# BurnhamG/PyTorch-ScalableFHVAE

Measured on AMD Instinct MI355X. Metric: segments/sec + ELBO (nats/frame), (B,20,80) fbank, higher is better.
Workload: dtype bf16; 1 GPU; c3: fhvae.FHVAE 2x256 LSTM enc/dec, z1=z2=32, 28k-seq mu2 table, batch 2048; per-GPU batch 2048, T=20, F=80, full train step (fwd+loss+bwd+Adam), intended objective, mu_idx uniform; global_batch=2048, parallelism=single

## Files before the change

include/fhvae_hip.h:

```cpp
#ifndef FHVAE_HIP_H
#define FHVAE_HIP_H

#include <stdint.h>

#ifdef __cplusplus
extern "C" {
#endif

#define FHVAE_ABI_VERSION 11

enum { FHVAE_F32 = 0, FHVAE_BF16 = 1 };

enum {
  FHVAE_OK = 0,
  FHVAE_ERR_NULL = -1,
  FHVAE_ERR_SHAPE = -2,
  FHVAE_ERR_DTYPE = -3,
  FHVAE_ERR_ALIGN = -4,
  FHVAE_ERR_LIMIT = -5
};

#define FHVAE_MAX_LAYERS 4
#define FHVAE_LSTM_SYNC_BYTES 16384

int fhvae_abi_version(void);
const char* fhvae_strerror(int code);

int fhvae_linear_fwd(const void* x, int64_t ldx, const void* w, int64_t ldw, const float* b,
                     float* y, int64_t ldy, void* y_lp, int64_t M, int64_t K, int64_t N, int relu,
                     int dtype, void* stream);

int fhvae_linear_bwd(const float* x, int64_t ldx, const float* w, int64_t ldw, const float* y,
                     int64_t ldy, const float* dy, int64_t lddy, float* dy_masked, float* dx,
                     int64_t lddx, float* dw, int64_t lddw, float* db, int64_t M, int64_t K,
                     int64_t N, int relu, int dx_accumulate, void* stream);

int fhvae_gauss_head_reparam_fwd(const void* h, int64_t ldh, const void* w_mu, const void* w_lv,
                                 const float* b_mu, const float* b_lv, const float* eps, float* mu,
                                 float* logvar, float* sample, int64_t M, int64_t K, int64_t D,
                                 int dtype, void* stream);
int fhvae_gauss_head_pair_fwd(const void* h_lp, int64_t ldh, const void* w_pair_lp, const float* b_mu, const float* b_lv,
                              float* out, int64_t ldo, int64_t M, int64_t K, int64_t D, void* stream);
int fhvae_head_pair_weights(const float* w_mu, const float* w_lv, void* wl_pair, void* wt_pair, int64_t ldt,
                            int64_t D, int64_t K, void* stream);
int fhvae_gauss_reparam_pair_fwd(const float* out, int64_t ldo, const float* eps, float* sample, float* mu, float* logvar,
                                 int64_t M, int64_t D, void* stream);
int fhvae_gauss_reparam_bwd_pair(const float* d_mu, const float* d_logvar, const float* d_sample, int64_t ld_s, const float* eps,
                                 const float* logvar, int64_t ld_lv, void* g_lp, int64_t ldg, float* db_mu, float* db_lv,
                                 int64_t M, int64_t D, void* stream);
int fhvae_gauss_head_bwd_pair(const void* h_lp, int64_t ldh, const void* wt_pair, int64_t ldt, const void* g_lp, int64_t ldg,
                              const float* col_sum, int64_t col_sum_rows, float* dh, int64_t lddh, float* dw_mu, float* dw_lv, float* db_mu,
                              float* db_lv, int64_t M, int64_t K, int64_t D, void* stream);

int fhvae_gauss_reparam_bwd(const float* d_mu, const float* d_logvar, const float* d_sample,
                            const float* eps, const float* logvar, float* g_mu, float* g_lv,
                            int64_t n, void* stream);
int fhvae_gauss_head_bwd(const float* h, int64_t ldh, const float* w_mu, const float* w_lv,
                         const float* d_mu, const float* d_logvar, const float* d_sample,
                         const float* eps, const float* logvar, float* g_ws, float* dh, int64_t lddh,
                         float* dw_mu, float* dw_lv, float* db_mu, float* db_lv, int64_t M, int64_t K,
                         int64_t D, void* stream);
typedef struct fhvae_lstm_desc {
  int32_t dtype;
  int32_t L;
  int64_t B, T, I, Ic, H;
  const float* x;
  const void* x_lp;
  const float* xc;
  const float* w_ih[FHVAE_MAX_LAYERS];
  const float* w_hh[FHVAE_MAX_LAYERS];
  const float* b_ih[FHVAE_MAX_LAYERS];
  const float* b_hh[FHVAE_MAX_LAYERS];
  void* hs;
  float* cs;
  void* gates;
  float* hn;
  float* hs_top_f32;
  float* pre;
  void* lp;
  void* hn_lp;
  const float* head_w_mu;
  const float* head_w_lv;
  void* head_wl;
  void* head_wt;
  int64_t head_D, head_K, head_ldt;
  int32_t* sticky_status;
} fhvae_lstm_desc;

int64_t fhvae_lstm_lp_bytes(const fhvae_lstm_desc* d);
int64_t fhvae_lstm_pre_elems(const fhvae_lstm_desc* d);
int fhvae_lstm_layout_id(const fhvae_lstm_desc* d);

int64_t fhvae_lstm_ws_below_elems(const fhvae_lstm_desc* d);
int fhvae_lstm_form(const fhvae_lstm_desc* d);
int fhvae_lstm_seq_fwd(const fhvae_lstm_desc* d, void* stream);
int64_t fhvae_lstm_infer_cs_elems(const fhvae_lstm_desc* d);
int fhvae_lstm_seq_infer(const fhvae_lstm_desc* d, void* stream);

typedef struct fhvae_lstm_bwd_desc {
  fhvae_lstm_desc f;
  const float* d_hs_top;
  const float* d_hn;
  void* dgates;
  float* dgsum;
  float* dc;
  float* dw_ih[FHVAE_MAX_LAYERS];
  float* dw_hh[FHVAE_MAX_LAYERS];
  float* db_ih[FHVAE_MAX_LAYERS];
  float* db_hh[FHVAE_MAX_LAYERS];
  float* d_xc;
  int32_t phase;
  float* ws_below;
} fhvae_lstm_bwd_desc;

int fhvae_lstm_seq_bwd(const fhvae_lstm_bwd_desc* d, void* stream);
typedef struct fhvae_wgrad_desc {
  const void* a; int64_t lda;
  int64_t a_col0;
  const void* b; int64_t ldb;
  float* c; int64_t ldc;
  int64_t M, N, K;
} fhvae_wgrad_desc;
int fhvae_wgrad_desc_ok(const fhvae_wgrad_desc* p);
int fhvae_lstm_param_grads_multi(const fhvae_lstm_bwd_desc* const* descs, int n, const fhvae_wgrad_desc* extra, int n_extra,
                                 void* stream);
int fhvae_wgrad_bf16(const void* a, int64_t lda, const void* b, int64_t ldb, float* c, int64_t ldc, int64_t M,
                     int64_t N, int64_t K, void* stream);
int fhvae_wgrad_f32(const float* a, int64_t lda, const float* b, int64_t ldb, float* c, int64_t ldc, int64_t M, int64_t N,
                    int64_t K, void* stream);

int fhvae_proj_bf16(const void* a, int64_t lda, const void* b, int64_t ldb, const float* bias, float* c, int64_t ldc,
                    int64_t M, int64_t N, int64_t K, void* stream);

int fhvae_mu2_gather_fwd(const float* table, const int64_t* idx, int64_t idx_offset, float* mu2,
                         int64_t B, int64_t S, int64_t D, int32_t* oob_flag, void* stream);
int fhvae_mu2_gather_bwd(const float* dmu2, const int64_t* idx, int64_t idx_offset, float* dtable,
                         int64_t B, int64_t S, int64_t D, float scale, void* stream);

typedef struct fhvae_elbo_desc {
  int64_t B, T, F, D1, D2;
  const float* x;    int64_t x_sb, x_st;
  const float* x_mu; const float* x_lv; int64_t xo_sb, xo_st;
  const float* z1_mu; const float* z1_lv;
  const float* z2_mu; const float* z2_lv;
  const float* mu2;
  const int64_t* num_segs; double nsegs_scalar;
  float* lower_bound; float* log_px_z; float* neg_kld_z1; float* neg_kld_z2; float* log_pmu2;
} fhvae_elbo_desc;

int fhvae_elbo_fwd(const fhvae_elbo_desc* d, void* stream);

typedef struct fhvae_elbo_bwd_desc {
  fhvae_elbo_desc f;
  const float* g_lower_bound; const float* g_log_px_z; const float* g_neg_kld_z1;
  const float* g_neg_kld_z2; const float* g_log_pmu2;
  int32_t reference_detach;
  float* d_x_mu; float* d_x_lv;
  float* d_z1_mu; float* d_z1_lv; float* d_z2_mu; float* d_z2_lv; float* d_mu2;
  void* d_x_pair_lp; int64_t ld_pair; float* d_x_colsum;
} fhvae_elbo_bwd_desc;

int fhvae_elbo_bwd(const fhvae_elbo_bwd_desc* d, void* stream);
int64_t fhvae_elbo_colsum_rows(int64_t B);

int64_t fhvae_disc_lse_ws_bytes(int64_t B, int64_t S);
int fhvae_disc_lse_fwd(const float* q, const float* table, const int64_t* idx, int64_t row0,
                       float inv_two_var, float* row_max, float* row_sumexp, float* tgt_logit,
                       float* ce_mean, float ce_scale, void* ws, int64_t B, int64_t S, int64_t D, int dtype, void* stream);
int fhvae_shard_pack(const float* q, const int64_t* idx, float* out, int64_t B, int64_t D, void* stream);
int fhvae_shard_unpack(const float* packed, float* q, int64_t* idx, int64_t N, int64_t D, void* stream);
int fhvae_disc_merge_partials(const float* parts, float* row_max, float* row_sumexp, float* tgt_logit, int64_t W, int64_t N,
                              void* stream);
int fhvae_shard_bwd_pack(const float* dq_all, float dq_scale, const float* dmu2_local, int64_t own0, int64_t n_own, float* out,
                         int64_t N, int64_t D, void* stream);
int fhvae_shard_bwd_unpack(const float* buf, int64_t own0, int64_t n_own, float* dq_local, float* dmu2_all, int64_t N, int64_t D,
                           void* stream);
int fhvae_disc_ce_mean(const float* row_max, const float* row_sumexp, const float* tgt_logit,
                       float* ce_mean, float ce_scale, int64_t B, void* stream);

int64_t fhvae_disc_lse_bwd_ws_bytes(int64_t B, int64_t S, int64_t D);
int fhvae_disc_lse_bwd(const float* q, const float* table, const int64_t* idx, int64_t row0,
                       float inv_two_var, const float* row_max, const float* row_sumexp,
                       const float* g_scale, float g_mul, float* dq, float* dtable, void* ws, int64_t ws_bytes,
                       int64_t B, int64_t S, int64_t D, int dtype, void* stream);

int fhvae_loss_fwd(const float* lower_bound, const float* log_qy, float alpha, float* loss, int64_t B,
                   int32_t* nan_flag, void* stream);
int fhvae_loss_bwd(const float* g_loss, float alpha, float* d_lower_bound, float* d_log_qy, int64_t B,
                   void* stream);

int fhvae_adam_step(float* p, float* g, float* m, float* v, void* p_lp, int64_t n, float lr,
                    float beta1, float beta2, float eps, float grad_scale, int flags, int32_t* step_count,
                    void* stream);
#define FHVAE_ADAM_ZERO_GRAD 1
#define FHVAE_ADAM_ADVANCE 2
#define FHVAE_ADAM_STEP_WORDS (65 * 32)

int fhvae_trace_enable(int on);
int64_t fhvae_trace_collect(float* ms, int32_t* kind, double* flops, int64_t cap);

int fhvae_segment_gather(const float* pool, int64_t pool_frames, const int64_t* start, const float* mean,
                         const float* inv_std, float* out_btf, float* out_tbf, int64_t B, int64_t T,
                         int64_t F, int32_t* oob_flag, void* stream);

int fhvae_mu2_accumulate(const float* z2_mu, const int64_t* idx, float* zsum, float* count, int64_t N,
                         int64_t S, int64_t D, void* stream);
int fhvae_mu2_finalize(const float* zsum, const float* count, float* mu2, int64_t S, int64_t D,
                       float ratio, void* stream);

#define FHVAE_HS_BAD_SEQ 1
#define FHVAE_HS_CAP 2
#define FHVAE_HS_BAD_IDX 4
#define FHVAE_HS_UNSORTED 8
int fhvae_hs_select(const int64_t* seq_ptr, int64_t S, const int64_t* block_seqs, int64_t K, int64_t* seg_ids,
                    int64_t* local_idx, int64_t* n_out, int64_t cap, int32_t* status, void* stream);
int fhvae_mu2_accumulate_sorted(const float* z2_mu, const int64_t* local_idx, float* zsum, float* count, int64_t N,
                                int64_t K, int64_t D, int32_t* status, void* stream);
int fhvae_mu2_load_table(float* zsum, float* count, float* table, float* m_rows, float* v_rows, int64_t K, int64_t D,
                         float ratio, void* stream);
int fhvae_hs_pack_partials(float* zsum, float* count, float* out, int64_t K, int64_t D, void* stream);
int fhvae_mu2_merge_load_shard(const float* parts, int64_t W, int64_t K, int64_t row0, int64_t row1, float* shard,
                               float* m_rows, float* v_rows, int64_t D, float ratio, void* stream);

#define FHVAE_FEATS_FBANK 0
#define FHVAE_FEATS_SPEC 1
#define FHVAE_FEATS_MAX_NFFT 2048
#define FHVAE_FEATS_MAX_NFFT_FBANK 1664
#define FHVAE_FEATS_MAX_NMELS 256
#define FHVAE_FEATS_BAD_PTR 1
int fhvae_feats_tile_rows(int64_t n_fft, int ftype);
int fhvae_feats_fwd(const float* wave, int64_t n_samples, const int64_t* wave_ptr, const int64_t* frame_ptr, int64_t U,
                    int64_t n_frames, const float* dft_basis, const float* mel_basis, int64_t n_fft, int64_t hop, int64_t n_mels,
                    int ftype, float* out, int32_t* status, void* stream);

#define FHVAE_SYNTH_BAD_PTR 1
int fhvae_synth_tile_rows(int64_t n_fft);
int fhvae_synth_istft(const float* spec, int64_t n_frames, const int64_t* wave_ptr, const int64_t* frame_ptr, int64_t U,
                      int64_t n_samples, const float* synth_basis, const float* win_sq, int64_t n_fft, int64_t hop,
                      float* frames_ws, float* wave_out, int32_t* status, void* stream);
int fhvae_synth_project(const float* wave, int64_t n_samples, const int64_t* wave_ptr, const int64_t* frame_ptr, int64_t U,
                        int64_t n_frames, const float* dft_basis, const float* mag, const float* tprev, float coef, int64_t n_fft,
                        int64_t hop, float* rebuilt, float* next, int32_t* status, void* stream);
int fhvae_synth_deemph(const float* wave, const int64_t* wave_ptr, int64_t U, int64_t n_samples, float coef, float* out,
                       int32_t* status, void* stream);

#define FHVAE_RESAMPLE_MAX_L 4096
#define FHVAE_RESAMPLE_MAX_BANK (1 << 24)
#define FHVAE_RESAMPLE_LDS_FLOATS 40128
#define FHVAE_RESAMPLE_BAD_PTR 1
int fhvae_resample_tile_rows(int64_t KP);
int fhvae_resample_fwd(const float* wave_in, int64_t n_in, const int64_t* in_ptr, const int64_t* out_ptr,
                       const int64_t* row_ptr, int64_t U, int64_t n_rows, const float* bank, const int32_t* chunks, int64_t L,
                       int64_t M, int64_t P, int64_t KP, int64_t WL, double ratio, const uint8_t* exc, int64_t n_exc,
                       const float* alt, int64_t alt_taps, int64_t alt_wl, float* wave_out, int64_t n_out, int32_t* status,
                       void* stream);

int fhvae_to_time_major(const float* x_btf, void* x_tbf, float* x_tbf_f32, int64_t B, int64_t T,
                        int64_t F, int dtype, void* stream);
int fhvae_cast_bf16(const float* src, void* dst, void* dst_t, int64_t R, int64_t C, void* stream);

#ifdef __cplusplus
}
#endif
#endif
```

pytorch-scalablefhvae_amd/csrc/disc_mfma.h:

```cpp
#pragma once
#include "common.h"

namespace fh {

struct DiscMfmaArgs {
  const float* X;
  const float* Y;
  int NX, NY;
  float c;
  int x_is_query;
  const int64_t* idx;
  int64_t row0;
  const float* rmax;
  const float* rsum;
  const float* gsc;
  float gmul;
  float2* part;
  float* G;
  float* G2;
  float* WY;
  int chunk;
};

int mfma_chunk(int64_t nx, int64_t ny, int target = 1024);

bool disc_mfma_supported(int64_t B, int64_t S, int64_t D);
int64_t disc_mfma_ws_bytes(int64_t B, int64_t S);
int disc_mfma_fwd(const float* q, const float* table, const int64_t* idx, int64_t row0, float c, float2* part, int* nchunks,
                  int64_t B, int64_t S, int64_t D, int lp, hipStream_t st);
constexpr int64_t kOnePassWsCap = 3LL << 29;
int64_t disc_onepass_ws_bytes(int64_t B, int64_t S, int64_t D);
int disc_mfma_bwd(const float* q, const float* table, const int64_t* idx, int64_t row0, float c, const float* rmax,
                  const float* rsum, const float* gsc, float gmul, float* dq, float* dtable, float* ws, int64_t ws_bytes,
                  int64_t B, int64_t S, int64_t D, int lp, hipStream_t st);
void disc_lp_launch(const DiscMfmaArgs& a, int mode, dim3 grid, hipStream_t st);

}
```

pytorch-scalablefhvae_amd/csrc/disc_mfma.hip:

```cpp
#include <algorithm>

#include "disc_mfma.h"

#include <cstdlib>
#include <type_traits>

namespace fh {


template <int D>
__device__ __forceinline__ int yoff(int row, int ch) {
  constexpr int CHN = D / 4;
  return row * (D * 4) + ((ch ^ (row & (CHN >= 8 ? 7 : CHN - 1))) << 4);
}

template <int D, int MODE>
__global__ __launch_bounds__(256, 2) void disc_mfma_kernel(DiscMfmaArgs a) {
  constexpr int CHN = D / 4;
  constexpr int NJ = D / 16;
  constexpr int YT = 64;
  __shared__ __attribute__((aligned(16))) char ytile[YT * D * 4];
  __shared__ __attribute__((aligned(16))) float yn[YT];
  __shared__ float ymax[YT], yinv[YT];
  __shared__ int ytgt[YT];
  __shared__ int yown[YT / 16];
  constexpr bool BW = MODE >= 1, BOTH = MODE == 2;
  constexpr int kWLd = 68;
  constexpr int kDtLd = D + 4;
  __shared__ __attribute__((aligned(16))) float wimg[BOTH ? 4 : 1][BOTH ? 16 * kWLd : 4];
  __shared__ float wy_lds[BOTH ? 4 : 1][BOTH ? YT : 1];
  constexpr int kRed = !BW ? 1 : (BOTH && 4 * YT * kDtLd > 256 * (D + 1) ? 4 * YT * kDtLd : 256 * (D + 1));
  __shared__ __attribute__((aligned(16))) float red[kRed];
  float (*tr)[D + 1] = (float (*)[D + 1]) red;

  const int tid = threadIdx.x, lane = tid & 63, wave = tid >> 6;
  const int g = lane >> 4, i = lane & 15;
  const int x0 = blockIdx.y * 256 + wave * 64;
  const int y_begin = blockIdx.x * a.chunk;
  const int y_end = min(a.NY, y_begin + a.chunk);
  const float gscale = BW ? (*a.gsc) * a.gmul : 0.f;

  uint4 xf[4][NJ];
  float xn[4], xmax[4], xinv[4];
  int xtgt[4];
#pragma unroll
  for (int t = 0; t < 4; ++t) {
    const int x = x0 + t * 16 + i;
    const bool ok = x < a.NX;
    float nrm = 0.f;
#pragma unroll
    for (int jj = 0; jj < NJ; ++jj) {
      uint4 u = make_uint4(0, 0, 0, 0);
      if (ok) u = *(const uint4*)(a.X + (int64_t)x * D + 4 * g + 16 * jj);
      xf[t][jj] = u;
      const float f0 = __uint_as_float(u.x), f1 = __uint_as_float(u.y), f2 = __uint_as_float(u.z), f3 = __uint_as_float(u.w);
      nrm += f0 * f0 + f1 * f1 + f2 * f2 + f3 * f3;
    }
    nrm += __shfl_xor(nrm, 16, 64);
    nrm += __shfl_xor(nrm, 32, 64);
    xn[t] = nrm;
    xmax[t] = 0.f;
    xinv[t] = 0.f;
    xtgt[t] = -1;
    if (a.x_is_query) {
      if (ok) {
        const int64_t tg = a.idx[x] - a.row0;
        xtgt[t] = (tg >= 0 && tg < a.NY) ? (int)tg : -1;
        if (BW) {
          xmax[t] = a.rmax[x];
          xinv[t] = gscale / a.rsum[x];
        }
      }
    } else {
      xtgt[t] = ok ? x : -2;
    }
  }
  float m[4], ssum[4], wsum[4];
  f32x4 gacc[4][NJ];
#pragma unroll
  for (int t = 0; t < 4; ++t) {
    m[t] = -INFINITY;
    ssum[t] = 0.f;
    wsum[t] = 0.f;
#pragma unroll
    for (int j = 0; j < NJ; ++j) gacc[t][j] = f32x4{0.f, 0.f, 0.f, 0.f};
  }

  constexpr int LOADS = YT * CHN / 256;
  uint4 st[LOADS];
  auto issue = [&](int y0) {
#pragma unroll
    for (int p = 0; p < LOADS; ++p) {
      const int id = tid + p * 256;
      const int row = id / CHN, ch = id % CHN;
      const int y = y0 + row;
      st[p] = (y < y_end) ? *(const uint4*)(a.Y + (int64_t)y * D + ch * 4) : make_uint4(0, 0, 0, 0);
    }
  };
  if (y_begin < y_end) issue(y_begin);
  for (int y0 = y_begin; y0 < y_end; y0 += YT) {
#pragma unroll
    for (int p = 0; p < LOADS; ++p) {
      const int id = tid + p * 256;
      *(uint4*)(ytile + yoff<D>(id / CHN, id % CHN)) = st[p];
    }
    __syncthreads();
    if (y0 + YT < y_end) issue(y0 + YT);
    {
      const int row = tid >> 2, part = tid & 3;
      float nrm = 0.f;
#pragma unroll
      for (int c4 = part; c4 < CHN; c4 += 4) {
        const uint4 u = *(const uint4*)(ytile + yoff<D>(row, c4));
        const float f0 = __uint_as_float(u.x), f1 = __uint_as_float(u.y), f2 = __uint_as_float(u.z), f3 = __uint_as_float(u.w);
        nrm += f0 * f0 + f1 * f1 + f2 * f2 + f3 * f3;
      }
      nrm += __shfl_xor(nrm, 1, 64);
      nrm += __shfl_xor(nrm, 2, 64);
      bool mine = false;
      if (part == 0) {
        yn[row] = nrm;
        const int y = y0 + row;
        if (!a.x_is_query) {
          const bool ok = y < y_end;
          ymax[row] = ok && MODE == 1 ? a.rmax[y] : 0.f;
          yinv[row] = ok && MODE == 1 ? gscale / a.rsum[y] : 0.f;
          int tg = -3;
          if (ok) {
            const int64_t v = a.idx[y] - a.row0;
            tg = (v >= 0 && v < a.NX) ? (int)v : -3;
          }
          ytgt[row] = tg;
          mine = tg >= (int)blockIdx.y * 256 && tg < (int)blockIdx.y * 256 + 256;
        }
      }
      {
        const bool any = __any(mine);
        if (lane == 0) yown[wave] = any ? 1 : 0;
      }
    }
    __syncthreads();

#pragma unroll 1
    for (int yb = 0; yb < YT / 16; ++yb) {
      if (y0 + yb * 16 >= y_end) break;
      uint4 af[NJ];
#pragma unroll
      for (int jj = 0; jj < NJ; ++jj) af[jj] = *(const uint4*)(ytile + yoff<D>(yb * 16 + i, g + 4 * jj));
      const float4 ynv = *(const float4*)(yn + yb * 16 + 4 * g);
      const float ynr[4] = {ynv.x, ynv.y, ynv.z, ynv.w};
      float ymx[4], yiv[4];
      int ytg[4];
      if (MODE == 1 && !a.x_is_query) {
#pragma unroll
        for (int r = 0; r < 4; ++r) {
          ymx[r] = ymax[yb * 16 + 4 * g + r];
          yiv[r] = yinv[yb * 16 + 4 * g + r];
          ytg[r] = ytgt[yb * 16 + 4 * g + r];
        }
      }
      const int ybase = y0 + yb * 16;
      const bool whole = ybase + 16 <= y_end && x0 + 64 <= a.NX;
      const bool own_blk = !a.x_is_query && yown[yb] != 0;
      const float c2 = 2.f * a.c;
      f32x4 oacc[BOTH ? NJ : 1];
      float wyp = 0.f;
      if constexpr (BOTH) {
#pragma unroll
        for (int dj = 0; dj < NJ; ++dj) oacc[dj] = f32x4{0.f, 0.f, 0.f, 0.f};
      }
      auto logits = [&](int t) __attribute__((always_inline)) -> f32x4 {
        f32x4 acc = {0.f, 0.f, 0.f, 0.f};
#pragma unroll
        for (int jj = 0; jj < NJ; ++jj) {
          const uint4 ua = af[jj], ub = xf[t][jj];
          acc = __builtin_amdgcn_mfma_f32_16x16x4f32(__uint_as_float(ua.x), __uint_as_float(ub.x), acc, 0, 0, 0);
          acc = __builtin_amdgcn_mfma_f32_16x16x4f32(__uint_as_float(ua.y), __uint_as_float(ub.y), acc, 0, 0, 0);
          acc = __builtin_amdgcn_mfma_f32_16x16x4f32(__uint_as_float(ua.z), __uint_as_float(ub.z), acc, 0, 0, 0);
          acc = __builtin_amdgcn_mfma_f32_16x16x4f32(__uint_as_float(ua.w), __uint_as_float(ub.w), acc, 0, 0, 0);
        }
        return acc;
      };
      auto tile = [&](int t, auto masked_c, const f32x4& acc) __attribute__((always_inline)) {
        constexpr bool MASKED = decltype(masked_c)::value;
        const bool xok = x0 + t * 16 + i < a.NX;
        const float cxn = a.c * xn[t];
        float lg[4];
#pragma unroll
        for (int r = 0; r < 4; ++r) {
          lg[r] = c2 * acc[r] - (a.c * ynr[r] + cxn);
          if constexpr (MASKED) {
            const int y = ybase + 4 * g + r;
            if (!(xok && y < y_end)) lg[r] = -INFINITY;
            const bool own = (MODE == 1 && !a.x_is_query) ? ytg[r] == xtgt[t] : xtgt[t] == y;
            if (own) lg[r] = -INFINITY;
          }
        }
        if constexpr (MODE == 0) {
          const float gm = fmaxf(fmaxf(lg[0], lg[1]), fmaxf(lg[2], lg[3]));
          if (gm > m[t]) {
            ssum[t] *= __expf(m[t] - gm);
            m[t] = gm;
          }
          if (!MASKED || m[t] > -INFINITY) {
#pragma unroll
            for (int r = 0; r < 4; ++r) ssum[t] += __expf(lg[r] - m[t]);
          }
        } else {
          float w[4];
#pragma unroll
          for (int r = 0; r < 4; ++r) {
            float p;
            if (a.x_is_query)
              p = __expf(lg[r] - xmax[t]) * xinv[t];
            else
              p = __expf(lg[r] - ymx[r]) * yiv[r];
            w[r] = (!MASKED || lg[r] > -INFINITY) ? p : 0.f;
            wsum[t] += w[r];
          }
          float xb[BOTH ? 4 : 1][NJ];
          if constexpr (BOTH) {
#pragma unroll
            for (int q = 0; q < 4; ++q) {
              const int x = min(x0 + 16 * t + 4 * g + q, a.NX - 1);
#pragma unroll
              for (int dj = 0; dj < NJ; ++dj) xb[q][dj] = a.X[(int64_t)x * D + 16 * dj + i];
            }
          }
#pragma unroll
          for (int dj = 0; dj < NJ; ++dj) {
#pragma unroll
            for (int r = 0; r < 4; ++r) {
              const int row = yb * 16 + 4 * g + r, d = dj * 16 + i;
              const float av = *(const float*)(ytile + yoff<D>(row, d >> 2) + (d & 3) * 4);
              gacc[t][dj] = __builtin_amdgcn_mfma_f32_16x16x4f32(av, w[r], gacc[t][dj], 0, 0, 0);
            }
          }
          if constexpr (BOTH) {
            float* wi = wimg[wave];
#pragma unroll
            for (int r = 0; r < 4; ++r) wi[(4 * g + r) * kWLd + 16 * t + i] = w[r];
            asm volatile("" ::: "memory");
            const float4 wt = *(const float4*)(wi + i * kWLd + 16 * t + 4 * g);
            asm volatile("" ::: "memory");
            const float wq[4] = {wt.x, wt.y, wt.z, wt.w};
            wyp += (wq[0] + wq[1]) + (wq[2] + wq[3]);
#pragma unroll
            for (int q = 0; q < 4; ++q)
#pragma unroll
              for (int dj = 0; dj < NJ; ++dj) oacc[dj] = __builtin_amdgcn_mfma_f32_16x16x4f32(wq[q], xb[q][dj], oacc[dj], 0, 0, 0);
          }
        }
      };
      bool any_masked = !whole || own_blk;
      if (a.x_is_query) {
#pragma unroll
        for (int t = 0; t < 4; ++t) any_masked = any_masked || __any((unsigned)(xtgt[t] - ybase) < 16u);
      }
      if (!BOTH && !any_masked) {
        f32x4 nxt = logits(0);
#pragma unroll
        for (int t = 0; t < 4; ++t) {
          const f32x4 cur = nxt;
          if (t + 1 < 4) nxt = logits(t + 1);
          tile(t, std::false_type{}, cur);
        }
      } else {
#pragma unroll
        for (int t = 0; t < 4; ++t) {
          bool masked = !whole || own_blk;
          if (a.x_is_query) masked = masked || __any((unsigned)(xtgt[t] - ybase) < 16u);
          const f32x4 acc = logits(t);
          if (masked)
            tile(t, std::true_type{}, acc);
          else
            tile(t, std::false_type{}, acc);
        }
      }
      if constexpr (BOTH) {
        float* slot = red + wave * (YT * kDtLd);
#pragma unroll
        for (int dj = 0; dj < NJ; ++dj)
#pragma unroll
          for (int r = 0; r < 4; ++r) slot[(yb * 16 + 4 * g + r) * kDtLd + 16 * dj + i] = oacc[dj][r];
        wyp += __shfl_xor(wyp, 16, 64);
        wyp += __shfl_xor(wyp, 32, 64);
        if (g == 0) wy_lds[wave][yb * 16 + i] = wyp;
      }
    }
    __syncthreads();
    if constexpr (BOTH) {
      for (int e = tid; e < YT * D; e += 256) {
        const int row = e / D, d = e % D, o = row * kDtLd + d;
        if (y0 + row < y_end)
          a.G2[((int64_t)blockIdx.y * a.NY + y0 + row) * D + d] =
              (red[o] + red[YT * kDtLd + o]) + (red[2 * YT * kDtLd + o] + red[3 * YT * kDtLd + o]);
      }
      if (tid < YT && y0 + tid < y_end)
        a.WY[(int64_t)blockIdx.y * a.NY + y0 + tid] = (wy_lds[0][tid] + wy_lds[1][tid]) + (wy_lds[2][tid] + wy_lds[3][tid]);
    }
  }

  if constexpr (MODE == 0) {
#pragma unroll
    for (int t = 0; t < 4; ++t) {
      float mm = m[t], ss = ssum[t];
#pragma unroll
      for (int o = 16; o <= 32; o <<= 1) {
        const float om = __shfl_xor(mm, o, 64), os = __shfl_xor(ss, o, 64);
        const float nm = fmaxf(mm, om);
        ss = (nm == -INFINITY) ? 0.f : ss * __expf(mm - nm) + os * __expf(om - nm);
        mm = nm;
      }
      const int x = x0 + t * 16 + i;
      if (g == 0 && x < a.NX) a.part[(int64_t)blockIdx.x * a.NX + x] = make_float2(mm, ss);
    }
  } else {
    if constexpr (BOTH) __syncthreads();
#pragma unroll
    for (int t = 0; t < 4; ++t) {
      float ws = wsum[t];
      ws += __shfl_xor(ws, 16, 64);
      ws += __shfl_xor(ws, 32, 64);
#pragma unroll
      for (int dj = 0; dj < NJ; ++dj) {
        const int x = x0 + t * 16 + i;
        float4 xv = make_float4(0.f, 0.f, 0.f, 0.f);
        if (x < a.NX) xv = *(const float4*)(a.X + (int64_t)x * D + dj * 16 + 4 * g);
        const float xr[4] = {xv.x, xv.y, xv.z, xv.w};
#pragma unroll
        for (int r = 0; r < 4; ++r)
          tr[wave * 64 + t * 16 + i][dj * 16 + 4 * g + r] = 2.f * a.c * (gacc[t][dj][r] - xr[r] * ws);
      }
    }
    __syncthreads();
    for (int e = tid; e < 256 * D; e += 256) {
      const int rr = e / D, d = e % D;
      const int x = blockIdx.y * 256 + rr;
      if (x < a.NX) {
        if constexpr (BOTH)
          a.G[((int64_t)blockIdx.x * a.NX + x) * D + d] = tr[rr][d];
        else
          atomicAdd(a.G + (int64_t)x * D + d, tr[rr][d]);
      }
    }
  }
}

__global__ void disc_dt_finish_kernel(float* __restrict__ dy, const float* __restrict__ y, const float* __restrict__ g2,
                                      const float* __restrict__ wy, int nxt, float c2, int64_t NY, int D) {
  const int64_t i = (int64_t)blockIdx.x * blockDim.x + threadIdx.x;
  if (i >= NY * D) return;
  const int64_t row = i / D;
  float sg = 0.f, sw = 0.f;
  for (int t = 0; t < nxt; ++t) {
    sg += g2[(int64_t)t * NY * D + i];
    sw += wy[(int64_t)t * NY + row];
  }
  dy[i] += c2 * (sg - y[i] * sw);
}
__global__ void disc_dq_reduce_kernel(float* __restrict__ dx, const float* __restrict__ g, int nchunks, int64_t n) {
  const int64_t i = (int64_t)blockIdx.x * blockDim.x + threadIdx.x;
  if (i >= n) return;
  float a0 = 0.f, a1 = 0.f, a2 = 0.f, a3 = 0.f;
  int c = 0;
  for (; c + 4 <= nchunks; c += 4) {
    a0 += g[(int64_t)c * n + i], a1 += g[(int64_t)(c + 1) * n + i], a2 += g[(int64_t)(c + 2) * n + i], a3 += g[(int64_t)(c + 3) * n + i];
  }
  for (; c < nchunks; ++c) a0 += g[(int64_t)c * n + i];
  dx[i] = (a0 + a1) + (a2 + a3);
}

int mfma_chunk(int64_t nx, int64_t ny, int target) {
  const int64_t xt = fh_cdiv(nx, 256);
  int64_t want = fh_cdiv(target, xt);
  int64_t chunk = fh_cdiv(fh_cdiv(ny, want), 64) * 64;
  if (chunk < 64) chunk = 64;
  return (int)chunk;
}

bool disc_mfma_supported(int64_t B, int64_t S, int64_t D) { return (D == 32 || D == 16) && B * S >= (int64_t)1 << 16; }

int64_t disc_mfma_ws_bytes(int64_t B, int64_t S) {
  const int chunk = mfma_chunk(B, S);
  return fh_cdiv(S, chunk) * B * (int64_t)sizeof(float2);
}

static int64_t onepass_group_bytes(int64_t tiles, int64_t B, int64_t S, int64_t D) {
  const int64_t rows = std::min<int64_t>(B, tiles * 256);
  const int64_t nchunks = fh_cdiv(S, mfma_chunk(rows, S, 512));
  return (nchunks * rows * D + tiles * S * (D + 1)) * (int64_t)sizeof(float);
}
static int64_t onepass_group_tiles(int64_t bytes, int64_t B, int64_t S, int64_t D) {
  const int64_t nxt = fh_cdiv(B, 256);
  int64_t lo = 0, hi = nxt;
  while (lo < hi) {
    const int64_t mid = (lo + hi + 1) / 2;
    if (onepass_group_bytes(mid, B, S, D) <= bytes) lo = mid;
    else hi = mid - 1;
  }
  return lo;
}
int64_t disc_onepass_ws_bytes(int64_t B, int64_t S, int64_t D) {
  const int64_t t = onepass_group_tiles(kOnePassWsCap, B, S, D);
  return t > 0 ? onepass_group_bytes(t, B, S, D) : 0;
}

int disc_mfma_fwd(const float* q, const float* table, const int64_t* idx, int64_t row0, float c, float2* part, int* nchunks,
                  int64_t B, int64_t S, int64_t D, int lp, hipStream_t st) {
  DiscMfmaArgs a = {};
  a.X = q;
  a.Y = table;
  a.NX = (int)B;
  a.NY = (int)S;
  a.c = c;
  a.x_is_query = 1;
  a.idx = idx;
  a.row0 = row0;
  a.part = part;
  a.chunk = mfma_chunk(B, S);
  *nchunks = (int)fh_cdiv(S, a.chunk);
  dim3 grid((unsigned)*nchunks, (unsigned)fh_cdiv(B, 256));
  if (lp && D == 32)
    disc_lp_launch(a, 0, grid, st);
  else if (D == 32)
    hipLaunchKernelGGL((disc_mfma_kernel<32, 0>), grid, dim3(256), 0, st, a);
  else
    hipLaunchKernelGGL((disc_mfma_kernel<16, 0>), grid, dim3(256), 0, st, a);
  return fh_launch_status();
}

int disc_mfma_bwd(const float* q, const float* table, const int64_t* idx, int64_t row0, float c, const float* rmax,
                  const float* rsum, const float* gsc, float gmul, float* dq, float* dtable, float* ws, int64_t ws_bytes, int64_t B,
                  int64_t S, int64_t D, int lp, hipStream_t st) {
  DiscMfmaArgs a = {};
  a.c = c;
  a.idx = idx;
  a.row0 = row0;
  a.rmax = rmax;
  a.rsum = rsum;
  a.gsc = gsc;
  a.gmul = gmul;
  const int64_t gtiles = (dq && dtable && ws) ? onepass_group_tiles(ws_bytes, B, S, D) : 0;
  if (gtiles > 0) {
    for (int64_t x0 = 0; x0 < B; x0 += gtiles * 256) {
      const int64_t nb = std::min<int64_t>(B - x0, gtiles * 256), nxt = fh_cdiv(nb, 256);
      a.X = q + x0 * D;
      a.Y = table;
      a.NX = (int)nb;
      a.NY = (int)S;
      a.x_is_query = 1;
      a.idx = idx + x0;
      a.rmax = rmax + x0;
      a.rsum = rsum + x0;
      a.chunk = mfma_chunk(nb, S, 512);
      const int64_t nchunks = fh_cdiv(S, a.chunk);
      a.G = ws;
      a.G2 = a.G + nchunks * nb * D;
      a.WY = a.G2 + nxt * S * D;
      dim3 grid((unsigned)nchunks, (unsigned)nxt);
      if (lp && D == 32)
        disc_lp_launch(a, 2, grid, st);
      else if (D == 32)
        hipLaunchKernelGGL((disc_mfma_kernel<32, 2>), grid, dim3(256), 0, st, a);
      else
        hipLaunchKernelGGL((disc_mfma_kernel<16, 2>), grid, dim3(256), 0, st, a);
      int e = fh_launch_status();
      if (e) return e;
      hipLaunchKernelGGL(disc_dq_reduce_kernel, dim3((unsigned)fh_cdiv(nb * D, 256)), dim3(256), 0, st, dq + x0 * D, a.G, (int)nchunks, nb * D);
      hipLaunchKernelGGL(disc_dt_finish_kernel, dim3((unsigned)fh_cdiv(S * D, 256)), dim3(256), 0, st, dtable, table, a.G2, a.WY, (int)nxt,
                         2.f * c, S, (int)D);
      e = fh_launch_status();
      if (e) return e;
    }
    return FHVAE_OK;
  }
  if (dq) {
    hipError_t he = hipMemsetAsync(dq, 0, (size_t)(B * D) * sizeof(float), st);
    if (he != hipSuccess) return (int)he;
    a.X = q;
    a.Y = table;
    a.NX = (int)B;
    a.NY = (int)S;
    a.x_is_query = 1;
    a.G = dq;
    a.chunk = mfma_chunk(B, S, 512);
    dim3 grid((unsigned)fh_cdiv(S, a.chunk), (unsigned)fh_cdiv(B, 256));
    if (lp && D == 32)
      disc_lp_launch(a, 1, grid, st);
    else if (D == 32)
      hipLaunchKernelGGL((disc_mfma_kernel<32, 1>), grid, dim3(256), 0, st, a);
    else
      hipLaunchKernelGGL((disc_mfma_kernel<16, 1>), grid, dim3(256), 0, st, a);
    int e = fh_launch_status();
    if (e) return e;
  }
  if (dtable) {
    a.X = table;
    a.Y = q;
    a.NX = (int)S;
    a.NY = (int)B;
    a.x_is_query = 0;
    a.G = dtable;
    a.chunk = mfma_chunk(S, B, 512);
    dim3 grid((unsigned)fh_cdiv(B, a.chunk), (unsigned)fh_cdiv(S, 256));
    if (lp && D == 32)
      disc_lp_launch(a, 1, grid, st);
    else if (D == 32)
      hipLaunchKernelGGL((disc_mfma_kernel<32, 1>), grid, dim3(256), 0, st, a);
    else
      hipLaunchKernelGGL((disc_mfma_kernel<16, 1>), grid, dim3(256), 0, st, a);
    int e = fh_launch_status();
    if (e) return e;
  }
  return FHVAE_OK;
}

}
```

pytorch-scalablefhvae_amd/csrc/loss.hip:

```cpp
#include "common.h"
#include "disc_mfma.h"
#include <cstdlib>

namespace fh {

__device__ constexpr float kPz2Logvar = -1.3862943649291992f;
__device__ constexpr float kLog2Pi = 1.8378770664093453f;

template <typename T>
__global__ void to_time_major_kernel(const float* __restrict__ x, T* __restrict__ o, float* __restrict__ of, int64_t B,
                                     int64_t T_, int64_t F) {
  int64_t i = (int64_t)blockIdx.x * blockDim.x + threadIdx.x;
  if (i >= B * T_ * F) return;
  int64_t f = i % F, b = (i / F) % B, t = i / (F * B);
  float v = x[(b * T_ + t) * F + f];
  if constexpr (sizeof(T) == 4)
    o[i] = v;
  else
    o[i] = f2bf(v);
  if (of) of[i] = v;
}

template <typename T>
__global__ void to_time_major4_kernel(const float* __restrict__ x, T* __restrict__ o, float* __restrict__ of, int B, int T_, int F4) {
  const int64_t i = (int64_t)blockIdx.x * blockDim.x + threadIdx.x;
  if (i >= (int64_t)B * T_ * F4) return;
  const int f = (int)(i % F4);
  const int64_t tb = i / F4;
  const int b = (int)(tb % B), t = (int)(tb / B);
  const float4 v = ((const float4*)x)[((int64_t)b * T_ + t) * F4 + f];
  if constexpr (sizeof(T) == 4) {
    ((float4*)o)[i] = v;
  } else {
    ((uint2*)o)[i] = uint2{(uint32_t)f2bf(v.x) | ((uint32_t)f2bf(v.y) << 16), (uint32_t)f2bf(v.z) | ((uint32_t)f2bf(v.w) << 16)};
  }
  if (of) ((float4*)of)[i] = v;
}

__global__ void cast_bf16_kernel(const float* __restrict__ s, u16* __restrict__ d, u16* __restrict__ dt, int64_t R,
                                 int64_t C) {
  int64_t i = (int64_t)blockIdx.x * blockDim.x + threadIdx.x;
  if (i >= R * C) return;
  u16 v = f2bf(s[i]);
  if (d) d[i] = v;
  if (dt) dt[(i % C) * R + i / C] = v;
}

__global__ void gather_fwd_kernel(const float* __restrict__ table, const int64_t* __restrict__ idx, int64_t off,
                                  float* __restrict__ out, int64_t B, int64_t S, int64_t D, int32_t* oob) {
  int64_t i = (int64_t)blockIdx.x * blockDim.x + threadIdx.x;
  if (i >= B * D) return;
  int64_t b = i / D, d = i % D;
  int64_t s = idx[b] - off;
  if (s < 0 || s >= S) {
    out[i] = 0.f;
    if (oob && d == 0) atomicOr(oob, 1);
    return;
  }
  out[i] = table[s * D + d];
}

__global__ void gather_bwd_kernel(const float* __restrict__ dmu2, const int64_t* __restrict__ idx, int64_t off,
                                  float* __restrict__ dtable, int64_t B, int64_t S, int64_t D, float scale) {
  int64_t i = (int64_t)blockIdx.x * blockDim.x + threadIdx.x;
  if (i >= B * D) return;
  int64_t b = i / D, d = i % D;
  int64_t s = idx[b] - off;
  if (s < 0 || s >= S) return;
  atomicAdd(dtable + s * D + d, scale * dmu2[i]);
}


__device__ __forceinline__ float nll_term(float x, float mu, float lv) {
  const float df = x - mu;
  return lv + df * df / expf(lv);
}

__global__ __launch_bounds__(256) void elbo_fwd_kernel(fhvae_elbo_desc d) {
  const int lane = threadIdx.x & 63;
  const int64_t b = (int64_t)blockIdx.x * 4 + (threadIdx.x >> 6);
  if (b >= d.B) return;
  const float* x = d.x + b * d.x_sb;
  const float* xm = d.x_mu + b * d.xo_sb;
  const float* xl = d.x_lv + b * d.xo_sb;
  float s = 0.f;
  const bool vec = (d.F % 4 == 0) && (d.x_sb % 4 == 0) && (d.x_st % 4 == 0) && (d.xo_sb % 4 == 0) &&
                   (d.xo_st % 4 == 0) && ((((uintptr_t)d.x | (uintptr_t)d.x_mu | (uintptr_t)d.x_lv) & 15) == 0);
  if (vec) {
    const int F4 = (int)(d.F / 4);
    const int n4 = (int)d.T * F4;
    for (int i = lane; i < n4; i += 64) {
      const int t = i / F4, f = (i % F4) * 4;
      const float4 a = *(const float4*)(x + t * d.x_st + f);
      const float4 m = *(const float4*)(xm + t * d.xo_st + f);
      const float4 l = *(const float4*)(xl + t * d.xo_st + f);
      s += nll_term(a.x, m.x, l.x) + nll_term(a.y, m.y, l.y) + nll_term(a.z, m.z, l.z) + nll_term(a.w, m.w, l.w);
    }
  } else {
    const int n = (int)(d.T * d.F);
    for (int i = lane; i < n; i += 64) {
      const int t = i / (int)d.F, f = i % (int)d.F;
      s += nll_term(x[t * d.x_st + f], xm[t * d.xo_st + f], xl[t * d.xo_st + f]);
    }
  }
  s = wave_sum(s);
  const float log_px_z = -0.5f * ((float)(d.T * d.F) * kLog2Pi + s);

  const float v2 = expf(kPz2Logvar);
  float k1 = 0.f, k2 = 0.f, pm = 0.f;
  for (int j = lane; j < d.D1; j += 64) {
    const float mu = d.z1_mu[b * d.D1 + j], lv = d.z1_lv[b * d.D1 + j];
    k1 += 1.f + lv - 0.f - (mu * mu + expf(lv)) / 1.f;
  }
  for (int j = lane; j < d.D2; j += 64) {
    const float mu = d.z2_mu[b * d.D2 + j], lv = d.z2_lv[b * d.D2 + j], m2 = d.mu2[b * d.D2 + j];
    const float df = mu - m2;
    k2 += 1.f + lv - kPz2Logvar - (df * df + expf(lv)) / v2;
    pm += kLog2Pi + m2 * m2;
  }
  k1 = 0.5f * wave_sum(k1);
  k2 = 0.5f * wave_sum(k2);
  pm = -0.5f * wave_sum(pm);
  if (lane == 0) {
    const float ns = d.num_segs ? (float)d.num_segs[b] : (float)d.nsegs_scalar;
    d.log_px_z[b] = log_px_z;
    d.neg_kld_z1[b] = k1;
    d.neg_kld_z2[b] = k2;
    d.log_pmu2[b] = pm;
    d.lower_bound[b] = log_px_z + k1 + k2 + pm / ns;
  }
}

__device__ __forceinline__ void elbo_dx4(const float4& a, const float4& mu, const float4& lv, float gpx, float4& gm, float4& gl) {
  const float av[4] = {a.x, a.y, a.z, a.w}, mv[4] = {mu.x, mu.y, mu.z, mu.w}, lvv[4] = {lv.x, lv.y, lv.z, lv.w};
  float m[4], l[4];
#pragma unroll
  for (int k = 0; k < 4; ++k) {
    const float df = av[k] - mv[k], iv = 1.f / expf(lvv[k]);
    m[k] = gpx * df * iv;
    l[k] = gpx * -0.5f * (1.f - df * df * iv);
  }
  gm = make_float4(m[0], m[1], m[2], m[3]);
  gl = make_float4(l[0], l[1], l[2], l[3]);
}

struct ElboG {
  float gpx, gk1, gk2, gpm;
};
__device__ __forceinline__ ElboG elbo_upstream(const fhvae_elbo_bwd_desc& bd, int64_t b) {
  const fhvae_elbo_desc& d = bd.f;
  const float glb = bd.g_lower_bound ? bd.g_lower_bound[b] : 0.f;
  ElboG g;
  g.gpx = glb + (bd.g_log_px_z ? bd.g_log_px_z[b] : 0.f);
  g.gk1 = glb + (bd.g_neg_kld_z1 ? bd.g_neg_kld_z1[b] : 0.f);
  g.gk2 = glb + (bd.g_neg_kld_z2 ? bd.g_neg_kld_z2[b] : 0.f);
  const float ns = d.num_segs ? (float)d.num_segs[b] : (float)d.nsegs_scalar;
  g.gpm = glb / ns + (bd.g_log_pmu2 ? bd.g_log_pmu2[b] : 0.f);
  return g;
}
__device__ __forceinline__ void elbo_dz(const fhvae_elbo_bwd_desc& bd, int64_t b, int lane, const ElboG& g) {
  const fhvae_elbo_desc& d = bd.f;
  const float v2 = expf(kPz2Logvar);
  for (int j = lane; j < d.D1; j += 64) {
    const int64_t o = b * d.D1 + j;
    const float mu = d.z1_mu[o], lv = d.z1_lv[o];
    bd.d_z1_mu[o] = -mu * g.gk1;
    bd.d_z1_lv[o] = 0.5f * (1.f - expf(lv)) * g.gk1;
  }
  for (int j = lane; j < d.D2; j += 64) {
    const int64_t o = b * d.D2 + j;
    const float mu = d.z2_mu[o], lv = d.z2_lv[o], m2 = d.mu2[o];
    const float df = (mu - m2) / v2;
    bd.d_z2_mu[o] = -df * g.gk2;
    bd.d_z2_lv[o] = 0.5f * (1.f - expf(lv) / v2) * g.gk2;
    bd.d_mu2[o] = df * g.gk2 + (bd.reference_detach ? 0.f : -m2 * g.gpm);
  }
}

__global__ __launch_bounds__(256) void elbo_bwd_kernel(fhvae_elbo_bwd_desc bd) {
  const fhvae_elbo_desc& d = bd.f;
  const int lane = threadIdx.x & 63;
  const int64_t b = (int64_t)blockIdx.x * 4 + (threadIdx.x >> 6);
  if (b >= d.B) return;
  const ElboG g = elbo_upstream(bd, b);
  if (bd.d_x_mu && bd.d_x_lv && !bd.reference_detach) {
    const float* x = d.x + b * d.x_sb;
    const float* xm = d.x_mu + b * d.xo_sb;
    const float* xl = d.x_lv + b * d.xo_sb;
    float* dm = bd.d_x_mu + b * d.xo_sb;
    float* dl = bd.d_x_lv + b * d.xo_sb;
    const bool vec = (d.F % 4 == 0) && (d.x_sb % 4 == 0) && (d.x_st % 4 == 0) && (d.xo_sb % 4 == 0) && (d.xo_st % 4 == 0) &&
                     ((((uintptr_t)d.x | (uintptr_t)d.x_mu | (uintptr_t)d.x_lv | (uintptr_t)bd.d_x_mu | (uintptr_t)bd.d_x_lv) & 15) == 0);
    if (vec) {
      const int F4 = (int)(d.F / 4), n4 = (int)d.T * F4;
      for (int i = lane; i < n4; i += 64) {
        const int t = i / F4, f = (i % F4) * 4;
        const int64_t o = t * d.xo_st + f;
        float4 gm, gl;
        elbo_dx4(*(const float4*)(x + t * d.x_st + f), *(const float4*)(xm + o), *(const float4*)(xl + o), g.gpx, gm, gl);
        *(float4*)(dm + o) = gm;
        *(float4*)(dl + o) = gl;
      }
    } else {
      const int n = (int)(d.T * d.F);
      for (int i = lane; i < n; i += 64) {
        const int t = i / (int)d.F, f = i % (int)d.F;
        const int64_t o = t * d.xo_st + f;
        const float df = x[t * d.x_st + f] - xm[o];
        const float iv = 1.f / expf(xl[o]);
        dm[o] = g.gpx * df * iv;
        dl[o] = g.gpx * -0.5f * (1.f - df * df * iv);
      }
    }
  }
  elbo_dz(bd, b, lane, g);
}

__global__ __launch_bounds__(256) void elbo_bwd_pair_kernel(fhvae_elbo_bwd_desc bd) {
  const fhvae_elbo_desc& d = bd.f;
  __shared__ float cs[4][512];
  const int lane = threadIdx.x & 63, wave = threadIdx.x >> 6;
  const int64_t b = (int64_t)blockIdx.x * 2 + (wave >> 1);
  const int half = wave & 1;
  const int F = (int)d.F, F4 = F / 4, RP = 64 / F4, T = (int)d.T;
  const int rsub = lane / F4, f = (lane % F4) * 4;
  const bool act = lane < RP * F4 && b < d.B;
  float4 sm = make_float4(0.f, 0.f, 0.f, 0.f), sl = sm;
  if (b < d.B) {
    const ElboG g = elbo_upstream(bd, b);
    const float* x = d.x + b * d.x_sb;
    const float* xm = d.x_mu + b * d.xo_sb;
    const float* xl = d.x_lv + b * d.xo_sb;
    float* dm = bd.d_x_mu + b * d.xo_sb;
    float* dl = bd.d_x_lv + b * d.xo_sb;
    u16* gp = (u16*)bd.d_x_pair_lp;
    const int npass = (T + RP - 1) / RP;
    for (int p0 = half; p0 < npass; p0 += 8) {
      float4 a[4], mu[4], lv[4];
#pragma unroll
      for (int k = 0; k < 4; ++k) {
        const int t = (p0 + 2 * k) * RP + rsub;
        if (act && t < T) {
          const int64_t o = t * d.xo_st + f;
          a[k] = *(const float4*)(x + t * d.x_st + f);
          mu[k] = *(const float4*)(xm + o);
          lv[k] = *(const float4*)(xl + o);
        }
      }
#pragma unroll
      for (int k = 0; k < 4; ++k) {
        const int t = (p0 + 2 * k) * RP + rsub;
        if (act && t < T) {
          const int64_t o = t * d.xo_st + f;
          float4 gm, gl;
          elbo_dx4(a[k], mu[k], lv[k], g.gpx, gm, gl);
          *(float4*)(dm + o) = gm;
          *(float4*)(dl + o) = gl;
          u16* row = gp + ((int64_t)t * d.B + b) * bd.ld_pair;
          *(uint2*)(row + f) = uint2{(uint32_t)f2bf(gm.x) | ((uint32_t)f2bf(gm.y) << 16), (uint32_t)f2bf(gm.z) | ((uint32_t)f2bf(gm.w) << 16)};
          *(uint2*)(row + F + f) = uint2{(uint32_t)f2bf(gl.x) | ((uint32_t)f2bf(gl.y) << 16), (uint32_t)f2bf(gl.z) | ((uint32_t)f2bf(gl.w) << 16)};
          sm.x += gm.x, sm.y += gm.y, sm.z += gm.z, sm.w += gm.w;
          sl.x += gl.x, sl.y += gl.y, sl.z += gl.z, sl.w += gl.w;
        }
      }
    }
    const int padc = (int)(bd.ld_pair - 2 * F) / 8;
    for (int i = lane + 64 * half; i < T * padc; i += 128) {
      const int t = i / padc, c = i % padc;
      *(uint4*)(gp + ((int64_t)t * d.B + b) * bd.ld_pair + 2 * F + c * 8) = make_uint4(0u, 0u, 0u, 0u);
    }
    if (half == 0) elbo_dz(bd, b, lane, g);
  }
  for (int j = lane; j < 2 * F; j += 64) cs[wave][j] = 0.f;
  __syncthreads();
  if (lane < RP * F4) {
    atomicAdd(&cs[wave][f + 0], sm.x), atomicAdd(&cs[wave][f + 1], sm.y), atomicAdd(&cs[wave][f + 2], sm.z), atomicAdd(&cs[wave][f + 3], sm.w);
    atomicAdd(&cs[wave][F + f + 0], sl.x), atomicAdd(&cs[wave][F + f + 1], sl.y), atomicAdd(&cs[wave][F + f + 2], sl.z),
        atomicAdd(&cs[wave][F + f + 3], sl.w);
  }
  __syncthreads();
  for (int j = threadIdx.x; j < 2 * F; j += 256)
    bd.d_x_colsum[(int64_t)blockIdx.x * 2 * F + j] = (cs[0][j] + cs[1][j]) + (cs[2][j] + cs[3][j]);
}

struct DiscPlan {
  int chunk;
  int nchunks;
  int btiles;
};
static inline DiscPlan disc_plan(int64_t B, int64_t S) {
  DiscPlan p;
  p.btiles = (int)fh_cdiv(B, 256);
  int64_t want = fh_cdiv(1024, p.btiles);
  int64_t chunk = fh_cdiv(S, want);
  chunk = fh_cdiv(chunk, 8) * 8;
  if (chunk < 8) chunk = 8;
  p.chunk = (int)chunk;
  p.nchunks = (int)fh_cdiv(S, chunk);
  return p;
}

template <int D>
__device__ __forceinline__ float sqdist(const float (&q)[D], const float* __restrict__ trow) {
  float a0 = 0.f, a1 = 0.f;
#pragma unroll
  for (int d = 0; d < D; d += 2) {
    const float d0 = q[d] - trow[d], d1 = q[d + 1] - trow[d + 1];
    a0 = fmaf(d0, d0, a0);
    a1 = fmaf(d1, d1, a1);
  }
  return a0 + a1;
}

template <int D>
__global__ __launch_bounds__(256) void disc_fwd_kernel(const float* __restrict__ q, const float* __restrict__ table,
                                                       float c, float2* __restrict__ part, int B, int S, int chunk) {
  const int b = blockIdx.x * 256 + threadIdx.x;
  const int bb = b < B ? b : B - 1;
  float qr[D];
#pragma unroll
  for (int d = 0; d < D; ++d) qr[d] = q[(int64_t)bb * D + d];
  const int s0 = blockIdx.y * chunk;
  const int s1 = min(S, s0 + chunk);
  float m = -INFINITY, sum = 0.f;
  for (int s = s0; s < s1; s += 8) {
    float l[8];
    float gm = -INFINITY;
#pragma unroll
    for (int u = 0; u < 8; ++u) {
      const int su = s + u;
      const float* trow = table + (int64_t)(su < s1 ? su : s1 - 1) * D;
      l[u] = su < s1 ? -c * sqdist<D>(qr, trow) : -INFINITY;
      gm = fmaxf(gm, l[u]);
    }
    if (gm > m) {
      sum *= __expf(m - gm);
      m = gm;
    }
#pragma unroll
    for (int u = 0; u < 8; ++u) sum += __expf(l[u] - m);
  }
  if (b < B) part[(int64_t)blockIdx.y * B + b] = make_float2(m, sum);
}

template <int D>
__global__ __launch_bounds__(256) void disc_combine_kernel(const float* __restrict__ q, const float* __restrict__ table,
                                                           const int64_t* __restrict__ idx, int64_t row0, float c,
                                                           const float2* __restrict__ part, int nchunks,
                                                           float* __restrict__ row_max, float* __restrict__ row_sum,
                                                           float* __restrict__ tgt, int B, int S, int own_excluded) {
  const int lane = threadIdx.x & 63;
  const int b = blockIdx.x * 4 + (threadIdx.x >> 6);
  if (b >= B) return;
  float m = -INFINITY, sum = 0.f;
  for (int k = lane; k < nchunks; k += 64) {
    const float2 p = part[(int64_t)k * B + b];
    if (p.x > m) {
      sum = sum * __expf(m - p.x) + p.y;
      m = p.x;
    } else {
      sum += p.y * __expf(p.x - m);
    }
  }
  const float gm = wave_max(m);
  sum = m == -INFINITY ? 0.f : sum * __expf(m - gm);
  sum = wave_sum(sum);
  const int64_t s = idx[b] - row0;
  if (lane == 0) {
    float t = 0.f;
    if (s >= 0 && s < S) {
      float qr[D];
#pragma unroll
      for (int d = 0; d < D; ++d) qr[d] = q[(int64_t)b * D + d];
      t = -c * sqdist<D>(qr, table + s * D);
      if (own_excluded) {
        const float nm = fmaxf(gm, t);
        sum = (gm == -INFINITY ? 0.f : sum * __expf(gm - nm)) + __expf(t - nm);
        row_max[b] = nm;
        row_sum[b] = sum;
        tgt[b] = t;
        return;
      }
    }
    row_max[b] = gm;
    row_sum[b] = sum;
    tgt[b] = t;
  }
}

template <int D>
__global__ __launch_bounds__(256) void disc_own_bwd_kernel(const float* __restrict__ q, const float* __restrict__ table,
                                                           const int64_t* __restrict__ idx, int64_t row0, float c,
                                                           const float* __restrict__ rmax, const float* __restrict__ rsum,
                                                           const float* __restrict__ gsc, float gmul, float* __restrict__ dq,
                                                           float* __restrict__ dtable, int B, int S) {
  constexpr int PER = D / 4;
  const int tid = blockIdx.x * 256 + threadIdx.x;
  const int b = tid / PER, part = tid % PER;
  if (b >= B) return;
  const int64_t s = idx[b] - row0;
  if (s < 0 || s >= S) return;
  float qr[D];
#pragma unroll
  for (int d = 0; d < D; ++d) qr[d] = q[(int64_t)b * D + d];
  const float t = -c * sqdist<D>(qr, table + s * D);
  const float w = (*gsc) * gmul * (__expf(t - rmax[b]) / rsum[b] - 1.f);
#pragma unroll
  for (int k = 0; k < 4; ++k) {
    const int d = part * 4 + k;
    const float diff = qr[d] - table[s * D + d];
    if (dq) atomicAdd(dq + (int64_t)b * D + d, -2.f * c * w * diff);
    if (dtable) atomicAdd(dtable + s * D + d, 2.f * c * w * diff);
  }
}

__global__ __launch_bounds__(256) void ce_mean_kernel(const float* __restrict__ row_max, const float* __restrict__ row_sum,
                                                      const float* __restrict__ tgt, float* __restrict__ out, int B, float scale) {
  __shared__ float red[4];
  float s = 0.f;
  for (int b = threadIdx.x; b < B; b += 256) s += (row_max[b] - tgt[b]) + logf(row_sum[b]);
  s = wave_sum(s);
  if ((threadIdx.x & 63) == 0) red[threadIdx.x >> 6] = s;
  __syncthreads();
  if (threadIdx.x == 0) *out = scale * ((red[0] + red[1] + red[2] + red[3]) / (float)B);
}

__global__ __launch_bounds__(256) void loss_fwd_kernel(const float* __restrict__ lb, const float* __restrict__ log_qy, float alpha,
                                                       float* __restrict__ out, int B, int* __restrict__ nan_flag) {
  __shared__ float red[4];
  float s = 0.f;
  for (int b = threadIdx.x; b < B; b += 256) s += lb[b];
  s = wave_sum(s);
  if ((threadIdx.x & 63) == 0) red[threadIdx.x >> 6] = s;
  __syncthreads();
  if (threadIdx.x == 0) {
    const float mean_lb = (red[0] + red[1] + red[2] + red[3]) / (float)B;
    *out = -(mean_lb + alpha * log_qy[0]);
    if (nan_flag && mean_lb != mean_lb) atomicOr(nan_flag, 1);
  }
}
__global__ void loss_bwd_kernel(const float* __restrict__ g, float alpha, float* __restrict__ d_lb, float* __restrict__ d_qy,
                                int64_t B) {
  const int64_t i = (int64_t)blockIdx.x * blockDim.x + threadIdx.x;
  const float gv = g ? g[0] : 1.f;
  if (i < B) d_lb[i] = -gv / (float)B;
  if (i == 0 && d_qy) d_qy[0] = -alpha * gv;
}

__global__ void shard_pack_kernel(const float* __restrict__ q, const int64_t* __restrict__ idx, float* __restrict__ out, int64_t B, int D) {
  const int64_t i = (int64_t)blockIdx.x * blockDim.x + threadIdx.x;
  if (i >= B * (D + 1)) return;
  const int64_t b = i / (D + 1);
  const int d = (int)(i - b * (D + 1));
  out[i] = d < D ? q[b * D + d] : __int_as_float((int)idx[b]);
}
__global__ void shard_unpack_kernel(const float* __restrict__ pk, float* __restrict__ q, int64_t* __restrict__ idx, int64_t N, int D) {
  const int64_t i = (int64_t)blockIdx.x * blockDim.x + threadIdx.x;
  if (i >= N * (D + 1)) return;
  const int64_t b = i / (D + 1);
  const int d = (int)(i - b * (D + 1));
  if (d < D)
    q[b * D + d] = pk[i];
  else
    idx[b] = (int64_t)__float_as_int(pk[i]);
}
__global__ void disc_merge_kernel(const float* __restrict__ parts, float* __restrict__ m, float* __restrict__ s, float* __restrict__ t,
                                  int W, int64_t N) {
  const int64_t i = (int64_t)blockIdx.x * blockDim.x + threadIdx.x;
  if (i >= N) return;
  float mx = -INFINITY;
  for (int w = 0; w < W; ++w) mx = fmaxf(mx, parts[((int64_t)w * 3 + 0) * N + i]);
  float ss = 0.f, tt = 0.f;
  for (int w = 0; w < W; ++w) {
    const float rm = parts[((int64_t)w * 3 + 0) * N + i], rs = parts[((int64_t)w * 3 + 1) * N + i];
    ss += rs > 0.f ? rs * __expf(rm - mx) : 0.f;
    tt += parts[((int64_t)w * 3 + 2) * N + i];
  }
  m[i] = mx, s[i] = ss, t[i] = tt;
}
__global__ void shard_bwd_pack_kernel(const float* __restrict__ dq, float scale, const float* __restrict__ dmu2, int64_t own0, int64_t nown,
                                      float* __restrict__ out, int64_t N, int D) {
  const int64_t i = (int64_t)blockIdx.x * blockDim.x + threadIdx.x;
  if (i >= N * 2 * D) return;
  const int64_t b = i / (2 * D);
  const int d = (int)(i - b * 2 * D);
  float v = 0.f;
  if (d < D) {
    if (dq) v = dq[b * D + d] * scale;
  } else if (dmu2 && b >= own0 && b < own0 + nown) {
    v = dmu2[(b - own0) * D + (d - D)];
  }
  out[i] = v;
}
__global__ void shard_bwd_unpack_kernel(const float* __restrict__ buf, int64_t own0, int64_t nown, float* __restrict__ dq_local,
                                        float* __restrict__ dmu2_all, int64_t N, int D) {
  const int64_t i = (int64_t)blockIdx.x * blockDim.x + threadIdx.x;
  if (i >= N * 2 * D) return;
  const int64_t b = i / (2 * D);
  const int d = (int)(i - b * 2 * D);
  if (d < D) {
    if (dq_local && b >= own0 && b < own0 + nown) dq_local[(b - own0) * D + d] = buf[i];
  } else if (dmu2_all) {
    dmu2_all[b * D + (d - D)] = buf[i];
  }
}

template <int D>
__global__ __launch_bounds__(256) void disc_bwd_dq_kernel(const float* __restrict__ q, const float* __restrict__ table,
                                                          const int64_t* __restrict__ idx, int64_t row0, float c,
                                                          const float* __restrict__ rmax, const float* __restrict__ rsum,
                                                          const float* __restrict__ gsc, float gmul,
                                                          float* __restrict__ dq, int B, int S, int chunk) {
  __shared__ float tr[256][D + 1];
  const int b = blockIdx.x * 256 + threadIdx.x;
  const int bb = b < B ? b : B - 1;
  float qr[D], V[D];
#pragma unroll
  for (int d = 0; d < D; ++d) {
    qr[d] = q[(int64_t)bb * D + d];
    V[d] = 0.f;
  }
  const float g = *gsc * gmul;
  const float mb = rmax[bb], inv_s = 1.f / rsum[bb];
  const int64_t tg = idx[bb] - row0;
  const int s0 = blockIdx.y * chunk, s1 = min(S, s0 + chunk);
  for (int s = s0; s < s1; ++s) {
    const float* trow = table + (int64_t)s * D;
    float df[D];
    float a0 = 0.f, a1 = 0.f;
#pragma unroll
    for (int d = 0; d < D; d += 2) {
      df[d] = qr[d] - trow[d];
      df[d + 1] = qr[d + 1] - trow[d + 1];
      a0 = fmaf(df[d], df[d], a0);
      a1 = fmaf(df[d + 1], df[d + 1], a1);
    }
    const float lg = -c * (a0 + a1);
    const float w = g * (__expf(lg - mb) * inv_s - (s == tg ? 1.f : 0.f));
#pragma unroll
    for (int d = 0; d < D; ++d) V[d] = fmaf(w, df[d], V[d]);
  }
#pragma unroll
  for (int d = 0; d < D; ++d) tr[threadIdx.x][d] = -2.f * c * V[d];
  __syncthreads();
  for (int i = threadIdx.x; i < 256 * D; i += 256) {
    const int r = i / D, d = i % D;
    const int br = blockIdx.x * 256 + r;
    if (br < B) atomicAdd(dq + (int64_t)br * D + d, tr[r][d]);
  }
}

template <int D>
__global__ __launch_bounds__(256) void disc_bwd_dt_kernel(const float* __restrict__ q, const float* __restrict__ table,
                                                          const int64_t* __restrict__ idx, int64_t row0, float c,
                                                          const float* __restrict__ rmax, const float* __restrict__ rsum,
                                                          const float* __restrict__ gsc, float gmul,
                                                          float* __restrict__ dtable, int B, int S, int bchunk) {
  __shared__ float tr[256][D + 1];
  const int s = blockIdx.x * 256 + threadIdx.x;
  const int ss = s < S ? s : S - 1;
  float t[D], U[D];
#pragma unroll
  for (int d = 0; d < D; ++d) {
    t[d] = table[(int64_t)ss * D + d];
    U[d] = 0.f;
  }
  const float g = *gsc * gmul;
  const int b0 = blockIdx.y * bchunk, b1 = min(B, b0 + bchunk);
  for (int b = b0; b < b1; ++b) {
    const float* qrow = q + (int64_t)b * D;
    float df[D];
    float a0 = 0.f, a1 = 0.f;
#pragma unroll
    for (int d = 0; d < D; d += 2) {
      df[d] = qrow[d] - t[d];
      df[d + 1] = qrow[d + 1] - t[d + 1];
      a0 = fmaf(df[d], df[d], a0);
      a1 = fmaf(df[d + 1], df[d + 1], a1);
    }
    const float lg = -c * (a0 + a1);
    const float w = g * (__expf(lg - rmax[b]) / rsum[b] - ((int64_t)s == idx[b] - row0 ? 1.f : 0.f));
#pragma unroll
    for (int d = 0; d < D; ++d) U[d] = fmaf(w, df[d], U[d]);
  }
#pragma unroll
  for (int d = 0; d < D; ++d) tr[threadIdx.x][d] = 2.f * c * U[d];
  __syncthreads();
  for (int i = threadIdx.x; i < 256 * D; i += 256) {
    const int r = i / D, d = i % D;
    const int sr = blockIdx.x * 256 + r;
    if (sr < S) atomicAdd(dtable + (int64_t)sr * D + d, tr[r][d]);
  }
}

__device__ __forceinline__ float adam_one(float& p, float g, float& m, float& v, float lr_bc1, float rs_bc2, float b1,
                                          float b2, float eps, float gscale) {
  const float gi = g * gscale;
  m = b1 * m + (1.f - b1) * gi;
  v = b2 * v + (1.f - b2) * gi * gi;
  const float denom = sqrtf(v) * rs_bc2 + eps;
  p = p - lr_bc1 * (m / denom);
  return p;
}

__global__ void adam_kernel(float* __restrict__ p, float* __restrict__ g, float* __restrict__ m,
                            float* __restrict__ v, u16* __restrict__ plp, int64_t n, float lr, float b1, float b2,
                            float eps, float gscale, int flags, int32_t* __restrict__ step) {
  const int t_i = *(volatile int32_t*)step + ((flags & FHVAE_ADAM_ADVANCE) ? 1 : 0);
  const float t = (float)t_i;
  const bool zg = (flags & FHVAE_ADAM_ZERO_GRAD) != 0;
  const float lr_bc1 = lr / (1.f - powf(b1, t)), rs_bc2 = 1.f / sqrtf(1.f - powf(b2, t));
  const int64_t n4 = n / 4;
  const bool vec = ((((uintptr_t)p | (uintptr_t)g | (uintptr_t)m | (uintptr_t)v) & 15) == 0);
  const int64_t stride = (int64_t)gridDim.x * blockDim.x;
  int64_t i = (int64_t)blockIdx.x * blockDim.x + threadIdx.x;
  if (vec) {
    for (int64_t k = i; k < n4; k += stride) {
      float4 pp = ((float4*)p)[k], mm = ((float4*)m)[k], vv = ((float4*)v)[k];
      const float4 gg = ((const float4*)g)[k];
      adam_one(pp.x, gg.x, mm.x, vv.x, lr_bc1, rs_bc2, b1, b2, eps, gscale);
      adam_one(pp.y, gg.y, mm.y, vv.y, lr_bc1, rs_bc2, b1, b2, eps, gscale);
      adam_one(pp.z, gg.z, mm.z, vv.z, lr_bc1, rs_bc2, b1, b2, eps, gscale);
      adam_one(pp.w, gg.w, mm.w, vv.w, lr_bc1, rs_bc2, b1, b2, eps, gscale);
      ((float4*)p)[k] = pp;
      ((float4*)m)[k] = mm;
      ((float4*)v)[k] = vv;
      if (zg) ((float4*)g)[k] = make_float4(0.f, 0.f, 0.f, 0.f);
      if (plp) {
        plp[4 * k] = f2bf(pp.x);
        plp[4 * k + 1] = f2bf(pp.y);
        plp[4 * k + 2] = f2bf(pp.z);
        plp[4 * k + 3] = f2bf(pp.w);
      }
    }
    i += n4 * 4;
    for (int64_t k = i; k < n; k += stride) {
      const float r = adam_one(p[k], g[k], m[k], v[k], lr_bc1, rs_bc2, b1, b2, eps, gscale);
      if (zg) g[k] = 0.f;
      if (plp) plp[k] = f2bf(r);
    }
  } else {
    for (int64_t k = i; k < n; k += stride) {
      const float r = adam_one(p[k], g[k], m[k], v[k], lr_bc1, rs_bc2, b1, b2, eps, gscale);
      if (zg) g[k] = 0.f;
      if (plp) plp[k] = f2bf(r);
    }
  }
  if (flags & FHVAE_ADAM_ADVANCE) {
    __syncthreads();
    if (threadIdx.x == 0) {
      const unsigned grp = blockIdx.x & 63u, ngrp = gridDim.x < 64u ? gridDim.x : 64u;
      const unsigned members = (gridDim.x - grp + 63u) / 64u;
      if (atomicAdd((unsigned*)(step + 32 * (1 + grp)), 1u) == members - 1) {
        step[32 * (1 + grp)] = 0;
        if (atomicAdd((unsigned*)(step + 1), 1u) == ngrp - 1) {
          step[1] = 0;
          step[0] = t_i;
        }
      }
    }
  }
}

}

using namespace fh;

extern "C" int fhvae_abi_version(void) { return FHVAE_ABI_VERSION; }

extern "C" const char* fhvae_strerror(int code) {
  switch (code) {
    case FHVAE_OK: return "ok";
    case FHVAE_ERR_NULL: return "required pointer is NULL";
    case FHVAE_ERR_SHAPE: return "bad or inconsistent dimension";
    case FHVAE_ERR_DTYPE: return "unsupported dtype for this entry point";
    case FHVAE_ERR_ALIGN: return "pointer or leading dimension not aligned";
    case FHVAE_ERR_LIMIT: return "dimension exceeds kernel index range";
    default: return code > 0 ? hipGetErrorString((hipError_t)code) : "unknown error";
  }
}

extern "C" int fhvae_to_time_major(const float* x_btf, void* x_tbf, float* x_tbf_f32, int64_t B, int64_t T, int64_t F,
                                   int dtype, void* stream) {
  FH_CHECK_PTR(x_btf);
  FH_CHECK_PTR(x_tbf);
  FH_CHECK_POS(B);
  FH_CHECK_POS(T);
  FH_CHECK_POS(F);
  const int64_t n = B * T * F;
  if (dtype != FHVAE_F32 && dtype != FHVAE_BF16) return FHVAE_ERR_DTYPE;
  if (F % 4 == 0 && B <= INT32_MAX && T <= INT32_MAX && ((((uintptr_t)x_btf) | ((uintptr_t)x_tbf) | ((uintptr_t)x_tbf_f32)) & 15) == 0) {
    dim3 grid4((unsigned)fh_cdiv(n / 4, 256));
    if (dtype == FHVAE_F32)
      hipLaunchKernelGGL((to_time_major4_kernel<float>), grid4, dim3(256), 0, (hipStream_t)stream, x_btf, (float*)x_tbf, x_tbf_f32, (int)B,
                         (int)T, (int)(F / 4));
    else
      hipLaunchKernelGGL((to_time_major4_kernel<u16>), grid4, dim3(256), 0, (hipStream_t)stream, x_btf, (u16*)x_tbf, x_tbf_f32, (int)B, (int)T,
                         (int)(F / 4));
    return fh_launch_status();
  }
  dim3 grid((unsigned)fh_cdiv(n, 256));
  if (dtype == FHVAE_F32)
    hipLaunchKernelGGL((to_time_major_kernel<float>), grid, dim3(256), 0, (hipStream_t)stream, x_btf, (float*)x_tbf,
                       x_tbf_f32, B, T, F);
  else if (dtype == FHVAE_BF16)
    hipLaunchKernelGGL((to_time_major_kernel<u16>), grid, dim3(256), 0, (hipStream_t)stream, x_btf, (u16*)x_tbf, x_tbf_f32,
                       B, T, F);
  else
    return FHVAE_ERR_DTYPE;
  return fh_launch_status();
}

extern "C" int fhvae_cast_bf16(const float* src, void* dst, void* dst_t, int64_t R, int64_t C, void* stream) {
  FH_CHECK_PTR(src);
  if (!dst && !dst_t) return FHVAE_ERR_NULL;
  FH_CHECK_POS(R);
  FH_CHECK_POS(C);
  hipLaunchKernelGGL(cast_bf16_kernel, dim3((unsigned)fh_cdiv(R * C, 256)), dim3(256), 0, (hipStream_t)stream, src,
                     (u16*)dst, (u16*)dst_t, R, C);
  return fh_launch_status();
}

extern "C" int fhvae_mu2_gather_fwd(const float* table, const int64_t* idx, int64_t idx_offset, float* mu2, int64_t B,
                                    int64_t S, int64_t D, int32_t* oob_flag, void* stream) {
  FH_CHECK_PTR(table);
  FH_CHECK_PTR(idx);
  FH_CHECK_PTR(mu2);
  FH_CHECK_POS(B);
  FH_CHECK_POS(S);
  FH_CHECK_POS(D);
  hipLaunchKernelGGL(gather_fwd_kernel, dim3((unsigned)fh_cdiv(B * D, 256)), dim3(256), 0, (hipStream_t)stream, table, idx,
                     idx_offset, mu2, B, S, D, oob_flag);
  return fh_launch_status();
}

extern "C" int fhvae_mu2_gather_bwd(const float* dmu2, const int64_t* idx, int64_t idx_offset, float* dtable, int64_t B,
                                    int64_t S, int64_t D, float scale, void* stream) {
  FH_CHECK_PTR(dmu2);
  FH_CHECK_PTR(idx);
  FH_CHECK_PTR(dtable);
  FH_CHECK_POS(B);
  FH_CHECK_POS(S);
  FH_CHECK_POS(D);
  hipLaunchKernelGGL(gather_bwd_kernel, dim3((unsigned)fh_cdiv(B * D, 256)), dim3(256), 0, (hipStream_t)stream, dmu2, idx,
                     idx_offset, dtable, B, S, D, scale);
  return fh_launch_status();
}

static int check_elbo(const fhvae_elbo_desc* d) {
  FH_CHECK_PTR(d);
  FH_CHECK_POS(d->B);
  FH_CHECK_POS(d->T);
  FH_CHECK_POS(d->F);
  FH_CHECK_POS(d->D1);
  FH_CHECK_POS(d->D2);
  FH_CHECK_I32(d->T * d->F);
  FH_CHECK_PTR(d->x);
  FH_CHECK_PTR(d->x_mu);
  FH_CHECK_PTR(d->x_lv);
  FH_CHECK_PTR(d->z1_mu);
  FH_CHECK_PTR(d->z1_lv);
  FH_CHECK_PTR(d->z2_mu);
  FH_CHECK_PTR(d->z2_lv);
  FH_CHECK_PTR(d->mu2);
  if (!d->num_segs && !(d->nsegs_scalar > 0)) return FHVAE_ERR_SHAPE;
  return FHVAE_OK;
}

extern "C" int fhvae_elbo_fwd(const fhvae_elbo_desc* d, void* stream) {
  int e = check_elbo(d);
  if (e) return e;
  FH_CHECK_PTR(d->lower_bound);
  FH_CHECK_PTR(d->log_px_z);
  FH_CHECK_PTR(d->neg_kld_z1);
  FH_CHECK_PTR(d->neg_kld_z2);
  FH_CHECK_PTR(d->log_pmu2);
  hipLaunchKernelGGL(elbo_fwd_kernel, dim3((unsigned)fh_cdiv(d->B, 4)), dim3(256), 0, (hipStream_t)stream, *d);
  return fh_launch_status();
}

extern "C" int fhvae_elbo_bwd(const fhvae_elbo_bwd_desc* d, void* stream) {
  FH_CHECK_PTR(d);
  int e = check_elbo(&d->f);
  if (e) return e;
  FH_CHECK_PTR(d->d_z1_mu);
  FH_CHECK_PTR(d->d_z1_lv);
  FH_CHECK_PTR(d->d_z2_mu);
  FH_CHECK_PTR(d->d_z2_lv);
  FH_CHECK_PTR(d->d_mu2);
  if (!d->reference_detach && (!d->d_x_mu || !d->d_x_lv)) return FHVAE_ERR_NULL;
  if (d->d_x_pair_lp) {
    const fhvae_elbo_desc& f = d->f;
    FH_CHECK_PTR(d->d_x_colsum);
    if (d->reference_detach || !d->d_x_mu) return FHVAE_ERR_NULL;
    if (f.F % 4 || f.F > 256 || d->ld_pair < 2 * f.F || (d->ld_pair - 2 * f.F) % 8 || d->ld_pair % 8) return FHVAE_ERR_SHAPE;
    if ((f.x_sb % 4) || (f.x_st % 4) || (f.xo_sb % 4) || (f.xo_st % 4)) return FHVAE_ERR_ALIGN;
    if ((((uintptr_t)f.x | (uintptr_t)f.x_mu | (uintptr_t)f.x_lv | (uintptr_t)d->d_x_mu | (uintptr_t)d->d_x_lv | (uintptr_t)d->d_x_pair_lp) & 15))
      return FHVAE_ERR_ALIGN;
  }
  if (d->d_x_pair_lp)
    hipLaunchKernelGGL(elbo_bwd_pair_kernel, dim3((unsigned)fh_cdiv(d->f.B, 2)), dim3(256), 0, (hipStream_t)stream, *d);
  else
    hipLaunchKernelGGL(elbo_bwd_kernel, dim3((unsigned)fh_cdiv(d->f.B, 4)), dim3(256), 0, (hipStream_t)stream, *d);
  return fh_launch_status();
}


extern "C" int64_t fhvae_disc_lse_bwd_ws_bytes(int64_t B, int64_t S, int64_t D) {
  return (B > 0 && S > 0 && D > 0 && disc_mfma_supported(B, S, D)) ? disc_onepass_ws_bytes(B, S, D) : 0;
}

extern "C" int64_t fhvae_elbo_colsum_rows(int64_t B) { return B > 0 ? fh_cdiv(B, 2) : 0; }

extern "C" int64_t fhvae_disc_lse_ws_bytes(int64_t B, int64_t S) {
  if (B <= 0 || S <= 0) return 0;
  DiscPlan p = disc_plan(B, S);
  const int64_t a = (int64_t)p.nchunks * B * (int64_t)sizeof(float2), b = disc_mfma_ws_bytes(B, S);
  return a > b ? a : b;
}

#define DISC_DISPATCH(D_, CALL) \
  switch (D_) {                 \
    case 4: { constexpr int DD = 4; CALL; } break;   \
    case 8: { constexpr int DD = 8; CALL; } break;   \
    case 16: { constexpr int DD = 16; CALL; } break; \
    case 32: { constexpr int DD = 32; CALL; } break; \
    case 64: { constexpr int DD = 64; CALL; } break; \
    default: return FHVAE_ERR_SHAPE;                 \
  }

extern "C" int fhvae_disc_lse_fwd(const float* q, const float* table, const int64_t* idx, int64_t row0, float inv_two_var,
                                  float* row_max, float* row_sumexp, float* tgt_logit, float* ce_mean, float ce_scale, void* ws,
                                  int64_t B, int64_t S, int64_t D, int dtype, void* stream) {
  if (dtype != FHVAE_F32 && dtype != FHVAE_BF16) return FHVAE_ERR_DTYPE;
  FH_CHECK_PTR(q);
  FH_CHECK_PTR(table);
  FH_CHECK_PTR(idx);
  FH_CHECK_PTR(row_max);
  FH_CHECK_PTR(row_sumexp);
  FH_CHECK_PTR(tgt_logit);
  FH_CHECK_PTR(ws);
  FH_CHECK_POS(B);
  FH_CHECK_POS(S);
  FH_CHECK_I32(B);
  FH_CHECK_I32(S);
  hipStream_t st = (hipStream_t)stream;
  DiscPlan p = disc_plan(B, S);
  float2* part = (float2*)ws;
  int e, own_excluded = 0;
  if (disc_mfma_supported(B, S, D) && !getenv("FHVAE_DISC_VALU")) {
    e = disc_mfma_fwd(q, table, idx, row0, inv_two_var, part, &p.nchunks, B, S, D, dtype == FHVAE_BF16, st);
    own_excluded = 1;
  } else {
    dim3 grid((unsigned)p.btiles, (unsigned)p.nchunks);
    DISC_DISPATCH(D, hipLaunchKernelGGL((disc_fwd_kernel<DD>), grid, dim3(256), 0, st, q, table, inv_two_var, part, (int)B,
                                        (int)S, p.chunk));
    e = fh_launch_status();
  }
  if (e) return e;
  DISC_DISPATCH(D, hipLaunchKernelGGL((disc_combine_kernel<DD>), dim3((unsigned)fh_cdiv(B, 4)), dim3(256), 0, st, q, table, idx,
                                      row0, inv_two_var, part, p.nchunks, row_max, row_sumexp, tgt_logit, (int)B, (int)S,
                                      own_excluded));
  e = fh_launch_status();
  if (e) return e;
  if (ce_mean) {
    hipLaunchKernelGGL(ce_mean_kernel, dim3(1), dim3(256), 0, st, row_max, row_sumexp, tgt_logit, ce_mean, (int)B, ce_scale);
    e = fh_launch_status();
  }
  return e;
}

extern "C" int fhvae_shard_pack(const float* q, const int64_t* idx, float* out, int64_t B, int64_t D, void* stream) {
  FH_CHECK_PTR(q);
  FH_CHECK_PTR(idx);
  FH_CHECK_PTR(out);
  FH_CHECK_POS(B);
  FH_CHECK_POS(D);
  hipLaunchKernelGGL(shard_pack_kernel, dim3((unsigned)fh_cdiv(B * (D + 1), 256)), dim3(256), 0, (hipStream_t)stream, q, idx, out, B, (int)D);
  return fh_launch_status();
}
extern "C" int fhvae_shard_unpack(const float* packed, float* q, int64_t* idx, int64_t N, int64_t D, void* stream) {
  FH_CHECK_PTR(packed);
  FH_CHECK_PTR(q);
  FH_CHECK_PTR(idx);
  FH_CHECK_POS(N);
  FH_CHECK_POS(D);
  hipLaunchKernelGGL(shard_unpack_kernel, dim3((unsigned)fh_cdiv(N * (D + 1), 256)), dim3(256), 0, (hipStream_t)stream, packed, q, idx, N, (int)D);
  return fh_launch_status();
}
extern "C" int fhvae_disc_merge_partials(const float* parts, float* row_max, float* row_sumexp, float* tgt_logit, int64_t W, int64_t N,
                                         void* stream) {
  FH_CHECK_PTR(parts);
  FH_CHECK_PTR(row_max);
  FH_CHECK_PTR(row_sumexp);
  FH_CHECK_PTR(tgt_logit);
  FH_CHECK_POS(W);
  FH_CHECK_POS(N);
  FH_CHECK_I32(W);
  hipLaunchKernelGGL(disc_merge_kernel, dim3((unsigned)fh_cdiv(N, 256)), dim3(256), 0, (hipStream_t)stream, parts, row_max, row_sumexp,
                     tgt_logit, (int)W, N);
  return fh_launch_status();
}
extern "C" int fhvae_shard_bwd_pack(const float* dq_all, float dq_scale, const float* dmu2_local, int64_t own0, int64_t n_own, float* out,
                                    int64_t N, int64_t D, void* stream) {
  FH_CHECK_PTR(out);
  FH_CHECK_POS(N);
  FH_CHECK_POS(D);
  hipLaunchKernelGGL(shard_bwd_pack_kernel, dim3((unsigned)fh_cdiv(N * 2 * D, 256)), dim3(256), 0, (hipStream_t)stream, dq_all, dq_scale,
                     dmu2_local, own0, n_own, out, N, (int)D);
  return fh_launch_status();
}
extern "C" int fhvae_shard_bwd_unpack(const float* buf, int64_t own0, int64_t n_own, float* dq_local, float* dmu2_all, int64_t N, int64_t D,
                                      void* stream) {
  FH_CHECK_PTR(buf);
  FH_CHECK_POS(N);
  FH_CHECK_POS(D);
  hipLaunchKernelGGL(shard_bwd_unpack_kernel, dim3((unsigned)fh_cdiv(N * 2 * D, 256)), dim3(256), 0, (hipStream_t)stream, buf, own0, n_own,
                     dq_local, dmu2_all, N, (int)D);
  return fh_launch_status();
}

extern "C" int fhvae_disc_ce_mean(const float* row_max, const float* row_sumexp, const float* tgt_logit, float* ce_mean,
                                  float ce_scale, int64_t B, void* stream) {
  FH_CHECK_PTR(row_max);
  FH_CHECK_PTR(row_sumexp);
  FH_CHECK_PTR(tgt_logit);
  FH_CHECK_PTR(ce_mean);
  FH_CHECK_POS(B);
  FH_CHECK_I32(B);
  hipLaunchKernelGGL(ce_mean_kernel, dim3(1), dim3(256), 0, (hipStream_t)stream, row_max, row_sumexp, tgt_logit, ce_mean,
                     (int)B, ce_scale);
  return fh_launch_status();
}

extern "C" int fhvae_disc_lse_bwd(const float* q, const float* table, const int64_t* idx, int64_t row0, float inv_two_var,
                                  const float* row_max, const float* row_sumexp, const float* g_scale, float g_mul,
                                  float* dq, float* dtable, void* ws, int64_t ws_bytes, int64_t B, int64_t S, int64_t D, int dtype,
                                  void* stream) {
  if (dtype != FHVAE_F32 && dtype != FHVAE_BF16) return FHVAE_ERR_DTYPE;
  FH_CHECK_PTR(q);
  FH_CHECK_PTR(table);
  FH_CHECK_PTR(idx);
  FH_CHECK_PTR(row_max);
  FH_CHECK_PTR(row_sumexp);
  FH_CHECK_PTR(g_scale);
  FH_CHECK_POS(B);
  FH_CHECK_POS(S);
  FH_CHECK_I32(B);
  FH_CHECK_I32(S);
  hipStream_t st = (hipStream_t)stream;
  if (disc_mfma_supported(B, S, D) && !getenv("FHVAE_DISC_VALU")) {
    if (ws && (((uintptr_t)ws) & 15)) return FHVAE_ERR_ALIGN;
    int e = disc_mfma_bwd(q, table, idx, row0, inv_two_var, row_max, row_sumexp, g_scale, g_mul, dq, dtable, (float*)ws,
                          ws ? ws_bytes : 0, B, S, D, dtype == FHVAE_BF16, st);
    if (e) return e;
    if (dq || dtable) {
      DISC_DISPATCH(D, hipLaunchKernelGGL((disc_own_bwd_kernel<DD>), dim3((unsigned)fh_cdiv(B * (DD / 4), 256)), dim3(256), 0, st, q,
                                          table, idx, row0, inv_two_var, row_max, row_sumexp, g_scale, g_mul, dq, dtable, (int)B,
                                          (int)S));
      e = fh_launch_status();
    }
    return e;
  }
  if (dq) {
    hipError_t he = hipMemsetAsync(dq, 0, (size_t)(B * D) * sizeof(float), st);
    if (he != hipSuccess) return (int)he;
    DiscPlan p = disc_plan(B, S);
    dim3 grid((unsigned)p.btiles, (unsigned)p.nchunks);
    DISC_DISPATCH(D, hipLaunchKernelGGL((disc_bwd_dq_kernel<DD>), grid, dim3(256), 0, st, q, table, idx, row0, inv_two_var,
                                        row_max, row_sumexp, g_scale, g_mul, dq, (int)B, (int)S, p.chunk));
    int e = fh_launch_status();
    if (e) return e;
  }
  if (dtable) {
    DiscPlan p = disc_plan(S, B);
    dim3 grid((unsigned)p.btiles, (unsigned)p.nchunks);
    DISC_DISPATCH(D, hipLaunchKernelGGL((disc_bwd_dt_kernel<DD>), grid, dim3(256), 0, st, q, table, idx, row0, inv_two_var,
                                        row_max, row_sumexp, g_scale, g_mul, dtable, (int)B, (int)S, p.chunk));
    int e = fh_launch_status();
    if (e) return e;
  }
  return FHVAE_OK;
}

extern "C" int fhvae_adam_step(float* p, float* g, float* m, float* v, void* p_lp, int64_t n, float lr, float beta1,
                               float beta2, float eps, float grad_scale, int flags, int32_t* step_count, void* stream) {
  if (flags & ~(FHVAE_ADAM_ZERO_GRAD | FHVAE_ADAM_ADVANCE)) return FHVAE_ERR_SHAPE;
  FH_CHECK_PTR(p);
  FH_CHECK_PTR(g);
  FH_CHECK_PTR(m);
  FH_CHECK_PTR(v);
  FH_CHECK_PTR(step_count);
  FH_CHECK_POS(n);
  int64_t blocks = fh_cdiv(fh_cdiv(n, 4), 256);
  if (blocks > 8192) blocks = 8192;
  if (blocks < 1) blocks = 1;
  hipLaunchKernelGGL(adam_kernel, dim3((unsigned)blocks), dim3(256), 0, (hipStream_t)stream, p, g, m, v, (u16*)p_lp, n, lr,
                     beta1, beta2, eps, grad_scale, flags, step_count);
  return fh_launch_status();
}

extern "C" int fhvae_loss_fwd(const float* lower_bound, const float* log_qy, float alpha, float* loss, int64_t B, int32_t* nan_flag,
                              void* stream) {
  FH_CHECK_PTR(lower_bound);
  FH_CHECK_PTR(log_qy);
  FH_CHECK_PTR(loss);
  FH_CHECK_POS(B);
  FH_CHECK_I32(B);
  hipLaunchKernelGGL(loss_fwd_kernel, dim3(1), dim3(256), 0, (hipStream_t)stream, lower_bound, log_qy, alpha, loss, (int)B, nan_flag);
  return fh_launch_status();
}

extern "C" int fhvae_loss_bwd(const float* g_loss, float alpha, float* d_lower_bound, float* d_log_qy, int64_t B, void* stream) {
  FH_CHECK_PTR(d_lower_bound);
  FH_CHECK_POS(B);
  hipLaunchKernelGGL(loss_bwd_kernel, dim3((unsigned)fh_cdiv(B, 256)), dim3(256), 0, (hipStream_t)stream, g_loss, alpha, d_lower_bound,
                     d_log_qy, B);
  return fh_launch_status();
}
```

pytorch-scalablefhvae_amd/fhvae.py:

```python
from __future__ import annotations

import math

import torch
import torch.nn as nn

import hip_binding as hb
from fhvae_core import FHVAEBase
from simple_fhvae import GaussianLayer


class LSTMParams(nn.Module):

    def __init__(self, input_size: int, hidden_size: int, num_layers: int):
        super().__init__()
        self.input_size, self.hidden_size, self.num_layers = input_size, hidden_size, num_layers
        k = 1.0 / math.sqrt(hidden_size)
        for l in range(num_layers):
            i = input_size if l == 0 else hidden_size
            for name, shape in (("weight_ih", (4 * hidden_size, i)), ("weight_hh", (4 * hidden_size, hidden_size)),
                                ("bias_ih", (4 * hidden_size,)), ("bias_hh", (4 * hidden_size,))):
                self.register_parameter("%s_l%d" % (name, l), nn.Parameter(torch.empty(shape).uniform_(-k, k)))

    def flat(self):
        out = []
        for l in range(self.num_layers):
            out += [getattr(self, "%s_l%d" % (n, l)) for n in ("weight_ih", "weight_hh", "bias_ih", "bias_hh")]
        return out


class LSTMNet(nn.Module):
    def __init__(self, input_size: int, hus):
        super().__init__()
        if len(set(hus)) != 1:
            raise ValueError("all layers of one LSTM net must share the hidden size (got %s)" % (hus,))
        self.lstm = LSTMParams(input_size, hus[0], len(hus))

    def forward(self, x_tm, xc, T, dtype=hb.F32, top=2, head=None):
        return hb.lstm_seq(x_tm, xc, T, self.lstm.flat(), dtype, top, head.head_weights() if (head is not None and dtype == hb.BF16) else None)


class FHVAE(FHVAEBase):
    def __init__(self, input_size: int, z1_hus: list, z2_hus: list, z1_dim: int, z2_dim: int, x_hus: list, *,
                 seg_len: int = 20, num_seqs=None, reference_compat=True, compute_dtype: str = "f32"):
        super().__init__()
        self.model = "fhvae"
        self._init_common(z1_hus, z2_hus, z1_dim, z2_dim, x_hus, num_seqs, reference_compat)
        input_size = int(input_size)
        if input_size % seg_len:
            raise ValueError("input_size=%d is not a multiple of seg_len=%d" % (input_size, seg_len))
        if compute_dtype not in ("f32", "bf16"):
            raise ValueError("compute_dtype must be 'f32' (exact-f32 MFMA, parity mode) or 'bf16'")
        self.compute_dtype = compute_dtype
        self.seg_len = int(seg_len)
        self.n_feat = input_size // seg_len
        F_ = self.n_feat
        self.z1_pre_encoder = LSTMNet(F_ + self.z2_dim, self.z1_hus)
        self.z2_pre_encoder = LSTMNet(F_, self.z2_hus)
        self.z1_gauss_layer = GaussianLayer(sum(self.z1_hus), self.z1_dim)
        self.z2_gauss_layer = GaussianLayer(sum(self.z2_hus), self.z2_dim)
        self.pre_decoder = LSTMNet(self.z1_dim + self.z2_dim, self.x_hus)
        self.dec_gauss_layer = GaussianLayer(self.x_hus[-1], F_)
        self._maybe_create_table()

    def mu2_lookup(self, mu_idx: torch.Tensor, z2_dim: int, num_seqs: int, init_std: float = 1.0, mu2_table=None):
        return self.table_ops.lookup(mu_idx, num_seqs, mu2_table)

    @torch.no_grad()
    def encode(self, x: torch.Tensor):
        x, _, _ = self._prep_inputs(x, torch.zeros(x.shape[0], dtype=torch.int64), 1)
        T = x.shape[1]
        dt = self._dt()
        x_tm = hb.to_time_major(x, with_bf16=dt == hb.BF16)
        _, hn2 = hb.lstm_seq_eval(x_tm, None, T, self.z2_pre_encoder.lstm.flat(), dt, top=0)
        z2_mu, z2_logvar, _ = self.z2_gauss_layer(hn2, sample=False)
        _, hn1 = hb.lstm_seq_eval(x_tm, z2_mu, T, self.z1_pre_encoder.lstm.flat(), dt, top=0)
        z1_mu, z1_logvar, _ = self.z1_gauss_layer(hn1, sample=False)
        self.qz2_x = [z2_mu, z2_logvar]
        return z1_mu, z2_mu

    @torch.no_grad()
    def encode_z2(self, x: torch.Tensor):
        x, _, _ = self._prep_inputs(x, torch.zeros(x.shape[0], dtype=torch.int64), 1)
        T = x.shape[1]
        dt = self._dt()
        x_tm = hb.to_time_major(x, with_bf16=dt == hb.BF16)
        _, hn2 = hb.lstm_seq_eval(x_tm, None, T, self.z2_pre_encoder.lstm.flat(), dt, top=0)
        z2_mu, z2_logvar, _ = self.z2_gauss_layer(hn2, sample=False)
        self.qz2_x = [z2_mu, z2_logvar]
        return z2_mu

    def _dt(self):
        return hb.BF16 if self.compute_dtype == "bf16" else hb.F32

    @torch.no_grad()
    def decode(self, z1: torch.Tensor, z2: torch.Tensor):
        z1, z2 = self._prep_latents(z1, z2)
        B, T, F_ = z1.shape[0], self.seg_len, self.n_feat
        dt = self._dt()
        lp_head = dt == hb.BF16 and self.x_hus[-1] % 8 == 0 and F_ % 8 == 0
        head = self.dec_gauss_layer.head_weights() if dt == hb.BF16 else None
        hs_top, _ = hb.lstm_seq_eval(None, torch.cat([z1, z2], dim=-1), T, self.pre_decoder.lstm.flat(), dt,
                                     top=1 if lp_head else 2, head=head)
        H = hs_top.shape[-1]
        hs_lp = getattr(hs_top, "_fh_lp", None) if lp_head else None
        x_mu, x_logvar, _ = self.dec_gauss_layer(hs_top.reshape(T * B, H), sample=False,
                                                 input_lp=hs_lp.reshape(T * B, H) if hs_lp is not None else None,
                                                 shadows=getattr(hs_top, "_fh_head", None))
        return (x_mu.reshape(T, B, F_).transpose(0, 1).contiguous(), x_logvar.reshape(T, B, F_).transpose(0, 1).contiguous())

    def forward(self, x: torch.Tensor, mu_idx: torch.Tensor, num_seqs: int, num_segs, *, mu2_table=None, eps=None):
        self._check_idx(mu_idx, num_seqs)
        x, mu_idx, num_segs = self._prep_inputs(x, mu_idx, num_segs)
        B, T, F_ = x.shape
        if F_ != self.n_feat:
            raise ValueError("x has %d features per frame, model was built for %d" % (F_, self.n_feat))
        mu2_table, mu2 = self.mu2_lookup(mu_idx, self.z2_dim, num_seqs, mu2_table=mu2_table)
        e2, e1 = self._draw(eps, B, x.device)

        dt = hb.BF16 if self.compute_dtype == "bf16" else hb.F32
        x_tm = hb.to_time_major(x, with_bf16=dt == hb.BF16)
        lp = (lambda h, dim: (getattr(h, "_fh_lp", None) if getattr(h, "_fh_lp", None) is not None else hb.cast_bf16(h))
              if (dt == hb.BF16 and h.shape[1] % 8 == 0 and dim % 8 == 0) else None)
        _, hn2 = self.z2_pre_encoder(x_tm, None, T, dt, top=0, head=self.z2_gauss_layer)
        z2_mu, z2_logvar, z2_sample = self.z2_gauss_layer(hn2, e2, input_lp=lp(hn2, self.z2_dim), shadows=getattr(hn2, "_fh_head", None))
        _, hn1 = self.z1_pre_encoder(x_tm, z2_sample, T, dt, top=0, head=self.z1_gauss_layer)
        z1_mu, z1_logvar, z1_sample = self.z1_gauss_layer(hn1, e1, input_lp=lp(hn1, self.z1_dim), shadows=getattr(hn1, "_fh_head", None))
        lp_head = dt == hb.BF16 and self.x_hus[-1] % 8 == 0 and F_ % 8 == 0
        hs_top, _ = self.pre_decoder(None, torch.cat([z1_sample, z2_sample], dim=-1), T, dt, top=1 if lp_head else 2,
                                     head=self.dec_gauss_layer)
        H = hs_top.shape[-1]
        hs_lp = getattr(hs_top, "_fh_lp", None)
        x_mu, x_logvar, _ = self.dec_gauss_layer(hs_top.reshape(T * B, H), sample=False,
                                                 input_lp=hs_lp.reshape(T * B, H) if hs_lp is not None else None,
                                                 shadows=getattr(hs_top, "_fh_head", None))

        layout = (B, T, F_, (F_, B * F_), (F_, B * F_))
        return self._tail(x_tm, layout, x_mu, x_logvar, (z1_mu, z1_logvar), (z2_mu, z2_logvar), mu2, mu2_table, mu_idx,
                          num_segs)
```

pytorch-scalablefhvae_amd/fhvae_core.py:

```python
from __future__ import annotations

import warnings
from typing import Optional, Tuple

import numpy as np
import torch
import torch.nn as nn

import hip_binding as hb

PZ1_LOGVAR = np.log(1.0 ** 2).astype(np.float32)
PMU2_LOGVAR = np.log(1.0 ** 2).astype(np.float32)
PZ2_LOGVAR = np.log(0.5 ** 2).astype(np.float32)


class LocalTableOps:

    def __init__(self, model):
        self.model = model

    def lookup(self, mu_idx, num_seqs, mu2_table=None):
        table = mu2_table if mu2_table is not None else self.model._table(num_seqs, mu_idx.device)
        return table, hb.mu2_gather(table, mu_idx)

    def disc(self, z2_mu, table, mu_idx, sign=1.0):
        return hb.disc_lse(z2_mu, table, mu_idx, lp=getattr(self.model, "compute_dtype", "f32") == "bf16", sign=sign)

    def resolve(self, z2_mu, table, mu_idx, mu2, sign=1.0):
        return mu2, self.disc(z2_mu, table, mu_idx, sign)


class FHVAEBase(nn.Module):

    def _init_common(self, z1_hus, z2_hus, z1_dim, z2_dim, x_hus, num_seqs, reference_compat):
        self.z1_hus = [int(h) for h in z1_hus]
        self.z2_hus = [int(h) for h in z2_hus]
        self.x_hus = [int(h) for h in x_hus]
        self.z1_dim = int(z1_dim)
        self.z2_dim = int(z2_dim)
        self.pz1 = [0.0, PZ1_LOGVAR]
        self.pmu2 = [0.0, PMU2_LOGVAR]
        self.pz2 = [None, PZ2_LOGVAR]
        self.reference_compat = bool(reference_compat)
        self._init_num_seqs = num_seqs
        self.table_ops = LocalTableOps(self)

    def _maybe_create_table(self):
        if self._init_num_seqs is not None:
            self.mu2_table = nn.Parameter(torch.empty(int(self._init_num_seqs), self.z2_dim).normal_(0.0, 1.0))
        else:
            self.register_parameter("mu2_table", None)

    def _table(self, num_seqs: int, device) -> torch.Tensor:
        if self.mu2_table is None:
            warnings.warn(
                "mu2_table created lazily at the first forward; optimizers built before this call do not "
                "contain it (pass num_seqs= to the constructor)")
            self.mu2_table = nn.Parameter(torch.empty(int(num_seqs), self.z2_dim, device=device).normal_(0.0, 1.0))
        if self.mu2_table.shape[0] != int(num_seqs):
            raise ValueError("num_seqs=%d does not match the mu2 table (%d rows)" % (num_seqs, self.mu2_table.shape[0]))
        return self.mu2_table

    @staticmethod
    def _check_idx(mu_idx, num_seqs):
        t = torch.as_tensor(mu_idx)
        if not t.is_cuda and t.numel() > 0:
            lo, hi = int(t.min()), int(t.max())
            if lo < 0 or hi >= int(num_seqs):
                raise IndexError("mu_idx out of range: [%d, %d] for a mu2 table of %d rows" % (lo, hi, num_seqs))

    @staticmethod
    def _prep_inputs(x, mu_idx, num_segs):
        if not x.is_cuda:
            raise RuntimeError("FHVAE (HIP path) needs the model and inputs on a MI355X device; no CPU fallback")
        if x.dtype != torch.float32:
            raise RuntimeError("the HIP path computes in float32/bf16; got input dtype %s "
                               "(the reference's model.double() at train_model.py:438 is not supported)" % x.dtype)
        dev = x.device
        mu_idx = torch.as_tensor(mu_idx).to(device=dev, dtype=torch.int64).contiguous()
        if isinstance(num_segs, torch.Tensor):
            num_segs = num_segs.to(device=dev, dtype=torch.int64).contiguous()
        return x.contiguous(), mu_idx, num_segs

    def _prep_latents(self, z1, z2):
        if not z1.is_cuda or not z2.is_cuda:
            raise RuntimeError("decode (HIP path) needs the latents on a MI355X device; no CPU fallback")
        if z1.dtype != torch.float32 or z2.dtype != torch.float32:
            raise RuntimeError("decode takes float32 latents; got %s / %s" % (z1.dtype, z2.dtype))
        if z1.dim() != 2 or z1.shape[1] != self.z1_dim:
            raise ValueError("z1 must be (B, %d); got %s" % (self.z1_dim, tuple(z1.shape)))
        if z2.dim() == 1:
            z2 = z2.unsqueeze(0).expand(z1.shape[0], -1)
        if z2.dim() != 2 or z2.shape[1] != self.z2_dim or z2.shape[0] != z1.shape[0]:
            raise ValueError("z2 must be (%d, %d) or (%d,); got %s" % (z1.shape[0], self.z2_dim, self.z2_dim, tuple(z2.shape)))
        return z1.contiguous(), z2.contiguous()

    @torch.no_grad()
    def reconstruct(self, x: torch.Tensor):
        x_mu, x_lv = self.decode(*self.encode(x))
        return x_mu.reshape(x.shape), x_lv.reshape(x.shape)

    @torch.no_grad()
    def convert(self, x: torch.Tensor, z2: torch.Tensor):
        z1, _ = self.encode(x)
        x_mu, x_lv = self.decode(z1, z2)
        return x_mu.reshape(x.shape), x_lv.reshape(x.shape)

    def _draw(self, eps, B, device):
        if eps is not None:
            return eps[0].to(device), eps[1].to(device)
        if self.z1_dim == self.z2_dim:
            e = torch.randn(2, B, self.z2_dim, device=device)
            return e[0], e[1]
        e2 = torch.randn(B, self.z2_dim, device=device)
        e1 = torch.randn(B, self.z1_dim, device=device)
        return e2, e1

    def _tail(self, x_like, layout, x_mu, x_lv, z1, z2, mu2, table, mu_idx, num_segs):
        rc = self.reference_compat
        mu2, log_qy = self.table_ops.resolve(z2[0], table, mu_idx, mu2, 1.0 if rc else -1.0)
        lb, lpx, nk1, nk2, lpm = hb.elbo(x_like, x_mu, x_lv, z1[0], z1[1], z2[0], z2[1], mu2, num_segs, layout, rc)
        self.qz2_x = [z2[0], z2[1]]
        self.pz2 = [mu2, PZ2_LOGVAR]
        return lb, log_qy, lpx, nk1, nk2, lpm
```

pytorch-scalablefhvae_amd/hip_binding.py:

```python
from __future__ import annotations

import ctypes as C
import os
from typing import List, Optional, Sequence

import numpy as np
import torch

_HERE = os.path.dirname(os.path.abspath(__file__))
LIB_PATH = os.path.join(_HERE, "libfhvae_hip.so")

F32, BF16 = 0, 1
MAX_LAYERS = 4
ABI_VERSION = 11
PZ2_LOGVAR = np.log(0.5 ** 2).astype(np.float32)
INV_TWO_VAR = float(np.float32(1.0) / (np.float32(2.0) * np.exp(PZ2_LOGVAR)))

_vp, _i64, _i32, _f32, _f64 = C.c_void_p, C.c_int64, C.c_int32, C.c_float, C.c_double


class LstmDesc(C.Structure):
    _fields_ = [
        ("dtype", _i32), ("L", _i32),
        ("B", _i64), ("T", _i64), ("I", _i64), ("Ic", _i64), ("H", _i64),
        ("x", _vp), ("x_lp", _vp), ("xc", _vp),
        ("w_ih", _vp * MAX_LAYERS), ("w_hh", _vp * MAX_LAYERS),
        ("b_ih", _vp * MAX_LAYERS), ("b_hh", _vp * MAX_LAYERS),
        ("hs", _vp), ("cs", _vp), ("gates", _vp), ("hn", _vp), ("hs_top_f32", _vp), ("pre", _vp), ("lp", _vp),
        ("hn_lp", _vp),
        ("head_w_mu", _vp), ("head_w_lv", _vp), ("head_wl", _vp), ("head_wt", _vp), ("head_D", _i64), ("head_K", _i64), ("head_ldt", _i64),
        ("sticky_status", _vp),
    ]


class LstmBwdDesc(C.Structure):
    _fields_ = [
        ("f", LstmDesc),
        ("d_hs_top", _vp), ("d_hn", _vp),
        ("dgates", _vp), ("dgsum", _vp), ("dc", _vp),
        ("dw_ih", _vp * MAX_LAYERS), ("dw_hh", _vp * MAX_LAYERS),
        ("db_ih", _vp * MAX_LAYERS), ("db_hh", _vp * MAX_LAYERS),
        ("d_xc", _vp), ("phase", _i32), ("ws_below", _vp),
    ]


class ElboDesc(C.Structure):
    _fields_ = [
        ("B", _i64), ("T", _i64), ("F", _i64), ("D1", _i64), ("D2", _i64),
        ("x", _vp), ("x_sb", _i64), ("x_st", _i64),
        ("x_mu", _vp), ("x_lv", _vp), ("xo_sb", _i64), ("xo_st", _i64),
        ("z1_mu", _vp), ("z1_lv", _vp), ("z2_mu", _vp), ("z2_lv", _vp), ("mu2", _vp),
        ("num_segs", _vp), ("nsegs_scalar", _f64),
        ("lower_bound", _vp), ("log_px_z", _vp), ("neg_kld_z1", _vp), ("neg_kld_z2", _vp), ("log_pmu2", _vp),
    ]


class ElboBwdDesc(C.Structure):
    _fields_ = [
        ("f", ElboDesc),
        ("g_lower_bound", _vp), ("g_log_px_z", _vp), ("g_neg_kld_z1", _vp), ("g_neg_kld_z2", _vp), ("g_log_pmu2", _vp),
        ("reference_detach", _i32),
        ("d_x_mu", _vp), ("d_x_lv", _vp), ("d_z1_mu", _vp), ("d_z1_lv", _vp), ("d_z2_mu", _vp), ("d_z2_lv", _vp),
        ("d_mu2", _vp),
        ("d_x_pair_lp", _vp), ("ld_pair", _i64), ("d_x_colsum", _vp),
    ]


class WgradDesc(C.Structure):
    _fields_ = [("a", _vp), ("lda", _i64), ("a_col0", _i64), ("b", _vp), ("ldb", _i64), ("c", _vp), ("ldc", _i64),
                ("M", _i64), ("N", _i64), ("K", _i64)]


SIGNATURES = {
    "fhvae_abi_version": (C.c_int, []),
    "fhvae_strerror": (C.c_char_p, [C.c_int]),
    "fhvae_linear_fwd": (C.c_int, [_vp, _i64, _vp, _i64, _vp, _vp, _i64, _vp, _i64, _i64, _i64, C.c_int, C.c_int, _vp]),
    "fhvae_linear_bwd": (C.c_int, [_vp, _i64, _vp, _i64, _vp, _i64, _vp, _i64, _vp, _vp, _i64, _vp, _i64, _vp, _i64, _i64,
                                   _i64, C.c_int, C.c_int, _vp]),
    "fhvae_gauss_head_reparam_fwd": (C.c_int, [_vp, _i64, _vp, _vp, _vp, _vp, _vp, _vp, _vp, _vp, _i64, _i64, _i64, C.c_int,
                                               _vp]),
    "fhvae_gauss_head_pair_fwd": (C.c_int, [_vp, _i64, _vp, _vp, _vp, _vp, _i64, _i64, _i64, _i64, _vp]),
    "fhvae_gauss_reparam_bwd": (C.c_int, [_vp, _vp, _vp, _vp, _vp, _vp, _vp, _i64, _vp]),
    "fhvae_gauss_head_bwd": (C.c_int, [_vp, _i64, _vp, _vp, _vp, _vp, _vp, _vp, _vp, _vp, _vp, _i64, _vp, _vp, _vp, _vp, _i64, _i64, _i64, _vp]),
    "fhvae_head_pair_weights": (C.c_int, [_vp, _vp, _vp, _vp, _i64, _i64, _i64, _vp]),
    "fhvae_gauss_reparam_pair_fwd": (C.c_int, [_vp, _i64, _vp, _vp, _vp, _vp, _i64, _i64, _vp]),
    "fhvae_gauss_reparam_bwd_pair": (C.c_int, [_vp, _vp, _vp, _i64, _vp, _vp, _i64, _vp, _i64, _vp, _vp, _i64, _i64, _vp]),
    "fhvae_elbo_colsum_rows": (_i64, [_i64]),
    "fhvae_gauss_head_bwd_pair": (C.c_int, [_vp, _i64, _vp, _i64, _vp, _i64, _vp, _i64, _vp, _i64, _vp, _vp, _vp, _vp, _i64, _i64, _i64, _vp]),
    "fhvae_loss_fwd": (C.c_int, [_vp, _vp, _f32, _vp, _i64, _vp, _vp]),
    "fhvae_loss_bwd": (C.c_int, [_vp, _f32, _vp, _vp, _i64, _vp]),
    "fhvae_lstm_lp_bytes": (_i64, [C.POINTER(LstmDesc)]),
    "fhvae_lstm_form": (C.c_int, [C.POINTER(LstmDesc)]),
    "fhvae_lstm_layout_id": (C.c_int, [C.POINTER(LstmDesc)]),
    "fhvae_lstm_pre_elems": (_i64, [C.POINTER(LstmDesc)]),
    "fhvae_lstm_ws_below_elems": (_i64, [C.POINTER(LstmDesc)]),
    "fhvae_lstm_seq_fwd": (C.c_int, [C.POINTER(LstmDesc), _vp]),
    "fhvae_lstm_infer_cs_elems": (_i64, [C.POINTER(LstmDesc)]),
    "fhvae_lstm_seq_infer": (C.c_int, [C.POINTER(LstmDesc), _vp]),
    "fhvae_lstm_seq_bwd": (C.c_int, [C.POINTER(LstmBwdDesc), _vp]),
    "fhvae_lstm_param_grads_multi": (C.c_int, [_vp, C.c_int, _vp, C.c_int, _vp]),
    "fhvae_wgrad_desc_ok": (C.c_int, [_vp]),
    "fhvae_wgrad_bf16": (C.c_int, [_vp, _i64, _vp, _i64, _vp, _i64, _i64, _i64, _i64, _vp]),
    "fhvae_wgrad_f32": (C.c_int, [_vp, _i64, _vp, _i64, _vp, _i64, _i64, _i64, _i64, _vp]),
    "fhvae_proj_bf16": (C.c_int, [_vp, _i64, _vp, _i64, _vp, _vp, _i64, _i64, _i64, _i64, _vp]),
    "fhvae_mu2_gather_fwd": (C.c_int, [_vp, _vp, _i64, _vp, _i64, _i64, _i64, _vp, _vp]),
    "fhvae_mu2_gather_bwd": (C.c_int, [_vp, _vp, _i64, _vp, _i64, _i64, _i64, _f32, _vp]),
    "fhvae_shard_pack": (C.c_int, [_vp, _vp, _vp, _i64, _i64, _vp]),
    "fhvae_shard_unpack": (C.c_int, [_vp, _vp, _vp, _i64, _i64, _vp]),
    "fhvae_disc_merge_partials": (C.c_int, [_vp, _vp, _vp, _vp, _i64, _i64, _vp]),
    "fhvae_shard_bwd_pack": (C.c_int, [_vp, _f32, _vp, _i64, _i64, _vp, _i64, _i64, _vp]),
    "fhvae_shard_bwd_unpack": (C.c_int, [_vp, _i64, _i64, _vp, _vp, _i64, _i64, _vp]),
    "fhvae_disc_ce_mean": (C.c_int, [_vp, _vp, _vp, _vp, _f32, _i64, _vp]),
    "fhvae_elbo_fwd": (C.c_int, [C.POINTER(ElboDesc), _vp]),
    "fhvae_elbo_bwd": (C.c_int, [C.POINTER(ElboBwdDesc), _vp]),
    "fhvae_disc_lse_ws_bytes": (_i64, [_i64, _i64]),
    "fhvae_disc_lse_bwd_ws_bytes": (_i64, [_i64, _i64, _i64]),
    "fhvae_disc_lse_fwd": (C.c_int, [_vp, _vp, _vp, _i64, _f32, _vp, _vp, _vp, _vp, _f32, _vp, _i64, _i64, _i64, C.c_int, _vp]),
    "fhvae_disc_lse_bwd": (C.c_int, [_vp, _vp, _vp, _i64, _f32, _vp, _vp, _vp, _f32, _vp, _vp, _vp, _i64, _i64, _i64, _i64, C.c_int, _vp]),
    "fhvae_adam_step": (C.c_int, [_vp, _vp, _vp, _vp, _vp, _i64, _f32, _f32, _f32, _f32, _f32, C.c_int, _vp, _vp]),
    "fhvae_segment_gather": (C.c_int, [_vp, _i64, _vp, _vp, _vp, _vp, _vp, _i64, _i64, _i64, _vp, _vp]),
    "fhvae_mu2_accumulate": (C.c_int, [_vp, _vp, _vp, _vp, _i64, _i64, _i64, _vp]),
    "fhvae_mu2_finalize": (C.c_int, [_vp, _vp, _vp, _i64, _i64, _f32, _vp]),
    "fhvae_hs_select": (C.c_int, [_vp, _i64, _vp, _i64, _vp, _vp, _vp, _i64, _vp, _vp]),
    "fhvae_mu2_accumulate_sorted": (C.c_int, [_vp, _vp, _vp, _vp, _i64, _i64, _i64, _vp, _vp]),
    "fhvae_mu2_load_table": (C.c_int, [_vp, _vp, _vp, _vp, _vp, _i64, _i64, _f32, _vp]),
    "fhvae_hs_pack_partials": (C.c_int, [_vp, _vp, _vp, _i64, _i64, _vp]),
    "fhvae_mu2_merge_load_shard": (C.c_int, [_vp, _i64, _i64, _i64, _i64, _vp, _vp, _vp, _i64, _f32, _vp]),
    "fhvae_feats_tile_rows": (C.c_int, [_i64, C.c_int]),
    "fhvae_feats_fwd": (C.c_int, [_vp, _i64, _vp, _vp, _i64, _i64, _vp, _vp, _i64, _i64, _i64, C.c_int, _vp, _vp, _vp]),
    "fhvae_synth_tile_rows": (C.c_int, [_i64]),
    "fhvae_synth_istft": (C.c_int, [_vp, _i64, _vp, _vp, _i64, _i64, _vp, _vp, _i64, _i64, _vp, _vp, _vp, _vp]),
    "fhvae_synth_project": (C.c_int, [_vp, _i64, _vp, _vp, _i64, _i64, _vp, _vp, _vp, C.c_float, _i64, _i64, _vp, _vp, _vp, _vp]),
    "fhvae_synth_deemph": (C.c_int, [_vp, _vp, _i64, _i64, C.c_float, _vp, _vp, _vp]),
    "fhvae_resample_tile_rows": (C.c_int, [_i64]),
    "fhvae_resample_fwd": (C.c_int, [_vp, _i64, _vp, _vp, _vp, _i64, _i64, _vp, _vp, _i64, _i64, _i64, _i64, _i64, C.c_double, _vp, _i64, _vp,
                                     _i64, _i64, _vp, _i64, _vp, _vp]),
    "fhvae_trace_enable": (C.c_int, [C.c_int]),
    "fhvae_trace_collect": (_i64, [_vp, _vp, _vp, _i64]),
    "fhvae_to_time_major": (C.c_int, [_vp, _vp, _vp, _i64, _i64, _i64, C.c_int, _vp]),
    "fhvae_cast_bf16": (C.c_int, [_vp, _vp, _vp, _i64, _i64, _vp]),
}

_lib = None


def load_library(path: str = LIB_PATH):
    global _lib
    if _lib is not None:
        return _lib
    if not os.path.exists(path):
        raise RuntimeError(
            "libfhvae_hip.so is not built (%s). Run `python pytorch-scalablefhvae_amd/build_ext.py` "
            "(or __graft_entry__.build()). There is no CPU fallback." % path
        )
    lib = C.CDLL(path)
    for name, (res, args) in SIGNATURES.items():
        fn = getattr(lib, name)
        fn.restype = res
        fn.argtypes = args
    if lib.fhvae_abi_version() != ABI_VERSION:
        raise RuntimeError("libfhvae_hip.so ABI version mismatch")
    _lib = lib
    return lib


_SIDE = {"stream": None, "pending": False, "keep": [], "enabled": False}


LSTM_BWD_REC_HOOK = {"fn": None}


_DEFER = {"enabled": not os.environ.get("FHVAE_NO_DEFER"), "pending": [], "extra": []}


def flush_param_grads():
    pend, extra = _DEFER["pending"], _DEFER["extra"]
    if not pend and not extra:
        return
    lib = load_library()
    n, nx = len(pend), len(extra)
    arr = (C.POINTER(LstmBwdDesc) * n)(*[C.pointer(bd) for bd, _ in pend]) if n else None
    xs = (WgradDesc * nx)(*[x for x, _ in extra]) if nx else None
    with _Timed("fhvae_lstm_param_grads_multi"):
        _check(lib.fhvae_lstm_param_grads_multi(arr, n, xs, nx, _stream()), "fhvae_lstm_param_grads_multi")
    pend.clear()
    extra.clear()


def flush_param_grads_except_last():
    pend = _DEFER["pending"]
    if len(pend) <= 1:
        return
    last = pend.pop()
    flush_param_grads()
    pend.append(last)


def set_defer_param_grads(on: bool):
    flush_param_grads()
    _DEFER["enabled"] = bool(on)


def side_stream():
    if _SIDE["stream"] is None:
        _SIDE["stream"] = torch.cuda.Stream()
    return _SIDE["stream"]


def join_side_stream():
    if _SIDE["pending"]:
        torch.cuda.current_stream().wait_stream(_SIDE["stream"])
        _SIDE["pending"] = False
        _SIDE["keep"].clear()


def set_side_stream_enabled(on: bool):
    join_side_stream()
    _SIDE["enabled"] = bool(on)


class _OpTimer:

    def __init__(self):
        self.on = False
        self.pairs = []

    def enable(self):
        self.on, self.pairs = True, []

    def disable(self):
        self.on = False

    def start(self):
        e = torch.cuda.Event(enable_timing=True)
        e.record()
        return e

    def stop(self, name, e0):
        e1 = torch.cuda.Event(enable_timing=True)
        e1.record()
        self.pairs.append((name, e0, e1))

    def summary(self):
        torch.cuda.synchronize()
        out = {}
        for name, e0, e1 in self.pairs:
            n, t = out.get(name, (0, 0.0))
            out[name] = (n + 1, t + e0.elapsed_time(e1))
        return out


OP_TIMER = _OpTimer()


def cell_trace(enable: bool):
    _check(load_library().fhvae_trace_enable(int(enable)), "fhvae_trace_enable")


def cell_trace_collect(cap: int = 65536):
    lib = load_library()
    ms = (C.c_float * cap)()
    kind = (C.c_int32 * cap)()
    fl = (C.c_double * cap)()
    n = int(lib.fhvae_trace_collect(ms, kind, fl, cap))
    out = {}
    for i in range(n):
        c, t, f = out.get(kind[i], (0, 0.0, 0.0))
        out[kind[i]] = (c + 1, t + ms[i], f + fl[i])
    return out


class _Timed:

    def __init__(self, name):
        self.name = name

    def __enter__(self):
        self.e0 = OP_TIMER.start() if OP_TIMER.on else None

    def __exit__(self, *exc):
        if self.e0 is not None:
            OP_TIMER.stop(self.name, self.e0)


def _check(code: int, what: str):
    if code != 0:
        msg = load_library().fhvae_strerror(code).decode()
        raise RuntimeError("%s failed: %s (code %d)" % (what, msg, code))


def _p(t: Optional[torch.Tensor]):
    if t is None:
        return None
    return t.data_ptr()


def _stream():
    return torch.cuda.current_stream().cuda_stream


def _need_gpu(*ts):
    for t in ts:
        if t is not None and not t.is_cuda:
            raise RuntimeError(
                "fhvae HIP op called with a CPU tensor: the hot path has no CPU fallback "
                "(move the model and inputs to a MI355X device)"
            )


def _sink(t):
    return getattr(t, "_fh_grad", None) if t is not None else None


def _f32c(t: torch.Tensor) -> torch.Tensor:
    if t.dtype != torch.float32:
        raise RuntimeError("fhvae HIP ops take float32 tensors (got %s)" % t.dtype)
    return t if t.is_contiguous() else t.contiguous()


def raw_linear_fwd(x, w, b, relu=False):
    lib = load_library()
    M, K = x.shape
    N = w.shape[0]
    y = torch.empty(M, N, device=x.device, dtype=torch.float32)
    with _Timed("fhvae_linear_fwd"):
        _check(lib.fhvae_linear_fwd(_p(x), x.stride(0), _p(w), w.stride(0), _p(b), _p(y), N, None, M, K, N, int(relu), F32,
                                    _stream()), "fhvae_linear_fwd")
    return y


def raw_linear_bwd(x, w, y, dy, relu, need_dx=True, need_dw=True, need_db=True, dx_out=None, dw_sink=None, db_sink=None):
    lib = load_library()
    M, K = x.shape
    N = w.shape[0]
    dev = x.device
    masked = torch.empty(M, N, device=dev, dtype=torch.float32) if relu else None
    acc = dx_out is not None
    dx = dx_out if acc else (torch.empty(M, K, device=dev, dtype=torch.float32) if need_dx else None)
    dw = dw_sink if dw_sink is not None else (torch.zeros(N, K, device=dev, dtype=torch.float32) if need_dw else None)
    db = db_sink if db_sink is not None else (torch.zeros(N, device=dev, dtype=torch.float32) if need_db else None)
    with _Timed("fhvae_linear_bwd"):
        _check(lib.fhvae_linear_bwd(_p(x), x.stride(0), _p(w), w.stride(0), _p(y), N if y is not None else 0, _p(dy),
                                    dy.stride(0), _p(masked), _p(dx), K, _p(dw), K, _p(db), M, K, N, int(relu), int(acc),
                                    _stream()), "fhvae_linear_bwd")
    return dx, dw, db


class _Linear(torch.autograd.Function):

    @staticmethod
    def forward(ctx, x, w, b, relu):
        _need_gpu(x, w, b)
        ctx.sinks = (_sink(w), _sink(b))
        x, w, b = _f32c(x), _f32c(w), _f32c(b)
        y = raw_linear_fwd(x, w, b, relu)
        ctx.relu = relu
        ctx.save_for_backward(x, w, y if relu else None)
        return y

    @staticmethod
    def backward(ctx, dy):
        x, w, y = ctx.saved_tensors
        dy = _f32c(dy)
        dx, dw, db = raw_linear_bwd(x, w, y, dy, ctx.relu, need_dx=ctx.needs_input_grad[0],
                                    need_dw=ctx.needs_input_grad[1], need_db=ctx.needs_input_grad[2],
                                    dw_sink=ctx.sinks[0], db_sink=ctx.sinks[1])
        return dx, (None if ctx.sinks[0] is not None else dw), (None if ctx.sinks[1] is not None else db), None


def linear(x, w, b, relu=False):
    return _Linear.apply(x, w, b, bool(relu))


class _GaussHead(torch.autograd.Function):

    @staticmethod
    def forward(ctx, h, w_mu, b_mu, w_lv, b_lv, eps):
        _need_gpu(h, w_mu, b_mu, w_lv, b_lv, eps)
        ctx.set_materialize_grads(False)
        lib = load_library()
        ctx.sinks = tuple(_sink(t) for t in (w_mu, b_mu, w_lv, b_lv))
        h, w_mu, b_mu, w_lv, b_lv = _f32c(h), _f32c(w_mu), _f32c(b_mu), _f32c(w_lv), _f32c(b_lv)
        M, K = h.shape
        D = w_mu.shape[0]
        mu = torch.empty(M, D, device=h.device, dtype=torch.float32)
        lv = torch.empty_like(mu)
        if eps is not None:
            eps = _f32c(eps)
            smp = torch.empty_like(mu)
        else:
            smp = None
        with _Timed("fhvae_gauss_head_reparam_fwd"):
            _check(lib.fhvae_gauss_head_reparam_fwd(_p(h), h.stride(0), _p(w_mu), _p(w_lv), _p(b_mu), _p(b_lv), _p(eps), _p(mu),
                                                    _p(lv), _p(smp), M, K, D, F32, _stream()), "fhvae_gauss_head_reparam_fwd")
        ctx.save_for_backward(h, w_mu, w_lv, eps, lv)
        if smp is None:
            smp = mu.new_empty(())
            ctx.mark_non_differentiable(smp)
        return mu, lv, smp

    @staticmethod
    def backward(ctx, d_mu, d_lv, d_s):
        lib = load_library()
        h, w_mu, w_lv, eps, lv = ctx.saved_tensors
        if eps is None:
            d_s = None
        M, D = lv.shape
        K = h.shape[1]
        d_mu = _f32c(d_mu) if d_mu is not None else None
        d_lv = _f32c(d_lv) if d_lv is not None else None
        d_s = _f32c(d_s) if d_s is not None else None
        need_dh = ctx.needs_input_grad[0]
        sk = ctx.sinks
        outs = [k if k is not None else torch.zeros(shape, device=h.device, dtype=torch.float32)
                for k, shape in zip(sk, ((D, K), (D,), (D, K), (D,)))]
        dw_mu, db_mu, dw_lv, db_lv = outs
        g_ws = torch.empty(M, 2 * D, device=h.device, dtype=torch.float32)
        dh = torch.empty(M, K, device=h.device, dtype=torch.float32) if need_dh else None
        with _Timed("fhvae_gauss_head_bwd"):
            _check(lib.fhvae_gauss_head_bwd(_p(h), h.stride(0), _p(w_mu), _p(w_lv), _p(d_mu), _p(d_lv), _p(d_s), _p(eps), _p(lv),
                                            _p(g_ws), _p(dh), K, _p(dw_mu), _p(dw_lv), _p(db_mu), _p(db_lv), M, K, D, _stream()),
                   "fhvae_gauss_head_bwd")
        dw_mu, db_mu, dw_lv, db_lv = (None if k is not None else o for k, o in zip(sk, outs))
        return dh, dw_mu, db_mu, dw_lv, db_lv, None


_PAIR_GRAD: dict = {}
PAIR_SIDE = {"enabled": True, "used": 0}


def _pair_ld(D: int) -> int:
    return (2 * D + 63) // 64 * 64


class _GaussHeadLp(torch.autograd.Function):

    @staticmethod
    def forward(ctx, h, h_lp, w_mu, b_mu, w_lv, b_lv, eps, shadows=None):
        _need_gpu(h, h_lp, w_mu, b_mu, w_lv, b_lv, eps)
        lib = load_library()
        ctx.set_materialize_grads(False)
        ctx.sinks = tuple(_sink(t) for t in (w_mu, b_mu, w_lv, b_lv))
        w_mu, b_mu, w_lv, b_lv = _f32c(w_mu), _f32c(b_mu), _f32c(w_lv), _f32c(b_lv)
        M, K = h_lp.shape
        D = w_mu.shape[0]
        assert h_lp.dtype == torch.bfloat16 and h_lp.is_contiguous() and h.shape == h_lp.shape
        dev = h_lp.device
        ldg = _pair_ld(D)
        if shadows is not None and tuple(shadows[0].shape) == (2 * D, K) and tuple(shadows[1].shape) == (K, ldg):
            wl, wt = shadows
        else:
            wl = torch.empty(2 * D, K, device=dev, dtype=torch.bfloat16)
            wt = torch.empty(K, ldg, device=dev, dtype=torch.bfloat16)
            _check(lib.fhvae_head_pair_weights(_p(w_mu), _p(w_lv), _p(wl), _p(wt), ldg, D, K, _stream()), "fhvae_head_pair_weights")
        out = torch.empty(M, 2 * D, device=dev, dtype=torch.float32)
        with _Timed("fhvae_gauss_head_reparam_fwd"):
            _check(lib.fhvae_gauss_head_pair_fwd(_p(h_lp), K, _p(wl), _p(b_mu), _p(b_lv), _p(out), 2 * D, M, K, D, _stream()),
                   "fhvae_gauss_head_pair_fwd")
            if eps is not None:
                eps = _f32c(eps)
                mu, lv, smp = (torch.empty(M, D, device=dev, dtype=torch.float32) for _ in range(3))
                _check(lib.fhvae_gauss_reparam_pair_fwd(_p(out), 2 * D, _p(eps), _p(smp), _p(mu), _p(lv), M, D, _stream()),
                       "fhvae_gauss_reparam_pair_fwd")
            else:
                mu, lv = out[:, :D], out[:, D:]
                smp = mu.new_empty(())
                ctx.mark_non_differentiable(smp)
        ctx.save_for_backward(h_lp, wt, eps, lv)
        return mu, lv, smp

    @staticmethod
    def backward(ctx, d_mu, d_lv, d_s):
        lib = load_library()
        h_lp, wt, eps, lv = ctx.saved_tensors
        if eps is None:
            d_s = None
        M, D = lv.shape
        K = h_lp.shape[1]
        ldg = wt.shape[1]
        need_dh = ctx.needs_input_grad[0]
        sk = ctx.sinks
        dev = h_lp.device
        outs = [k if k is not None else torch.zeros(shape, device=dev, dtype=torch.float32)
                for k, shape in zip(sk, ((D, K), (D,), (D, K), (D,)))]
        dh = torch.empty(M, K, device=dev, dtype=torch.float32) if need_dh else None
        g_lp = colsum = None
        db_done = False
        ready = _PAIR_GRAD.get("latest")
        if (ready is not None and d_s is None and d_mu is not None and d_lv is not None and ready[0].data_ptr() == d_mu.data_ptr()
                and d_mu._base is ready[0] and d_lv._base is ready[0] and ready[0]._version == ready[3]
                and d_lv.data_ptr() == d_mu.data_ptr() + 4 * D and d_mu.shape == (M, D) and d_lv.shape == (M, D)
                and d_mu.stride() == (2 * D, 1) and d_lv.stride() == (2 * D, 1) and ready[1].shape == (M, ldg)):
            g_lp, colsum = ready[1], ready[2]
            _PAIR_GRAD.clear()
            PAIR_SIDE["used"] += 1
        with _Timed("fhvae_gauss_head_bwd"):
            if g_lp is None:
                d_mu = _f32c(d_mu) if d_mu is not None else None
                d_lv = _f32c(d_lv) if d_lv is not None else None
                if d_s is not None and not (d_s.dtype == torch.float32 and d_s.dim() == 2 and d_s.stride(1) == 1 and d_s.stride(0) >= D):
                    d_s = _f32c(d_s)
                g_lp = torch.empty(M, ldg, device=dev, dtype=torch.bfloat16)
                _check(lib.fhvae_gauss_reparam_bwd_pair(_p(d_mu), _p(d_lv), _p(d_s), d_s.stride(0) if d_s is not None else D, _p(eps), _p(lv), lv.stride(0), _p(g_lp), ldg,
                                                        _p(outs[1]), _p(outs[3]), M, D, _stream()), "fhvae_gauss_reparam_bwd_pair")
                db_done = True
            xs = None
            if _DEFER["enabled"] and not _SIDE["enabled"] and all(k is not None for k in sk):
                xs = [WgradDesc(_p(g_lp) + 2 * i * D, ldg, i * D, _p(h_lp), K, _p(outs[2 * i]), K, D, K, M) for i in range(2)]
                if not all(lib.fhvae_wgrad_desc_ok(C.byref(x)) for x in xs):
                    xs = None
            dws = (None, None) if xs is not None else (outs[0], outs[2])
            _check(lib.fhvae_gauss_head_bwd_pair(_p(h_lp), K, _p(wt), ldg, _p(g_lp), ldg, _p(colsum), colsum.shape[0] if colsum is not None else 0, _p(dh), K,
                                                 _p(dws[0]), _p(dws[1]),
                                                 None if db_done else _p(outs[1]), None if db_done else _p(outs[3]), M, K, D, _stream()),
                   "fhvae_gauss_head_bwd_pair")
            if xs is not None:
                _DEFER["extra"].extend((x, (g_lp, h_lp, outs[0], outs[2])) for x in xs)
        dw_mu, db_mu, dw_lv, db_lv = (None if k is not None else o for k, o in zip(sk, outs))
        return dh, None, dw_mu, db_mu, dw_lv, db_lv, None, None


def head_shadow_shapes(w_mu):
    D, K = w_mu.shape
    if K % 8 or D % 8:
        return None
    return (2 * D, K), (K, _pair_ld(D))


def gauss_head(h, w_mu, b_mu, w_lv, b_lv, eps, h_lp=None, shadows=None):
    if h_lp is not None and h.shape[1] % 8 == 0 and w_mu.shape[0] % 8 == 0:
        mu, lv, smp = _GaussHeadLp.apply(h, h_lp, w_mu, b_mu, w_lv, b_lv, eps, shadows)
    else:
        mu, lv, smp = _GaussHead.apply(h, w_mu, b_mu, w_lv, b_lv, eps)
    return mu, lv, (smp if eps is not None else None)


def cast_bf16(t: torch.Tensor) -> torch.Tensor:
    _need_gpu(t)
    t = _f32c(t.detach())
    out = torch.empty(t.shape, device=t.device, dtype=torch.bfloat16)
    R = t.shape[0]
    _check(load_library().fhvae_cast_bf16(_p(t), _p(out), None, R, t.numel() // R, _stream()), "fhvae_cast_bf16")
    return out


def to_time_major(x: torch.Tensor, with_bf16: bool = False):
    _need_gpu(x)
    lib = load_library()
    x = _f32c(x.detach())
    B, T, F_ = x.shape
    out = torch.empty(T, B, F_, device=x.device, dtype=torch.float32)
    if with_bf16:
        lp = torch.empty(T, B, F_, device=x.device, dtype=torch.bfloat16)
        with _Timed("fhvae_to_time_major"):
            _check(lib.fhvae_to_time_major(_p(x), _p(lp), _p(out), B, T, F_, BF16, _stream()), "fhvae_to_time_major")
        out._fh_lp = lp
        return out
    with _Timed("fhvae_to_time_major"):
        _check(lib.fhvae_to_time_major(_p(x), _p(out), None, B, T, F_, F32, _stream()), "fhvae_to_time_major")
    return out


def _fill_lstm_desc(d, dtype, dims, x_tm, xc, params, x_lp=None):
    L, B, T, I, Ic, H = dims
    d.dtype, d.L, d.B, d.T, d.I, d.Ic, d.H = dtype, L, B, T, I, Ic, H
    d.x, d.xc = _p(x_tm), _p(xc)
    d.x_lp = _p(x_lp) if dtype == BF16 else None
    for l in range(L):
        d.w_ih[l], d.w_hh[l], d.b_ih[l], d.b_hh[l] = (_p(params[4 * l + k]) for k in range(4))
    d.sticky_status = _p(_device_words(params[0].device)) if dtype == BF16 else None


_DEVICE_WORDS: dict = {}


def _device_words(device) -> torch.Tensor:
    key = torch.device(device).index if torch.device(device).index is not None else torch.cuda.current_device()
    w = _DEVICE_WORDS.get(key)
    if w is None:
        w = _DEVICE_WORDS[key] = torch.zeros(4, device=torch.device("cuda", key), dtype=torch.int32)
    return w


def diverged(device=None) -> bool:
    w = _device_words(device if device is not None else torch.cuda.current_device())
    return bool(w[1].item() != 0)


def reset_device_words(device=None):
    _device_words(device if device is not None else torch.cuda.current_device()).zero_()


LSTM_WORKSPACES: list = []


LSTM_FORMS = {0: "one launch per wavefront step", 1: "persistent cluster kernel (waves split rows)",
              2: "persistent cluster kernel (waves split the contraction)"}
LAST_LSTM_FORM = {"form": 0, "layout": 0}


def lstm_kernel_names(form: int, H: int) -> dict:
    kn = {0: "lstm_%s_step_kernel", 1: "lstm_%s_cluster_kernel", 2: "lstm_%s_ksplit_kernel"}[form]
    names = {0: kn % "fwd", 1: kn % "bwd"}
    if form == 1:
        names[1] = "lstm_bwd_layer_rs_kernel" if H == 256 and not os.environ.get("FHVAE_NO_RS") else "lstm_bwd_layer_kernel"
        if H == 256 and not os.environ.get("FHVAE_NO_RS") and not os.environ.get("FHVAE_NO_FWD_WR"):
            names[0] = "lstm_fwd_wr_kernel"
    return names


def lstm_sync_status() -> int:
    st = 0
    for w in _DEVICE_WORDS.values():
        st |= int(w[0].item())
    for lp in LSTM_WORKSPACES:
        st |= int(lp[:4].view(torch.int32).item())
    return st


class _LstmSeq(torch.autograd.Function):

    @staticmethod
    def forward(ctx, x_tm, xc, T, dtype, top, head, *params):
        lib = load_library()
        ctx.set_materialize_grads(False)
        _need_gpu(x_tm, xc, *params)
        L = len(params) // 4
        assert len(params) == 4 * L and 1 <= L <= MAX_LAYERS
        ctx.sinks = [_sink(p) for p in params]
        params = [_f32c(p) for p in params]
        H = params[1].shape[1]
        x_lp = getattr(x_tm, "_fh_lp", None) if x_tm is not None else None
        x_tm = _f32c(x_tm) if x_tm is not None else None
        xc = _f32c(xc) if xc is not None else None
        I = x_tm.shape[2] if x_tm is not None else 0
        Ic = xc.shape[1] if xc is not None else 0
        B = x_tm.shape[1] if x_tm is not None else xc.shape[0]
        if x_tm is not None:
            assert x_tm.shape[0] == T
        assert params[0].shape == (4 * H, I + Ic), (params[0].shape, H, I, Ic)
        dev = params[0].device
        f32 = dict(device=dev, dtype=torch.float32)
        bf = dtype == BF16
        hs = torch.empty(L, T, B, H, device=dev, dtype=torch.bfloat16 if bf else torch.float32)
        cs = torch.empty(L, T, B, H, **f32)
        gates = torch.empty(L, T, B, 4 * H, device=dev, dtype=hs.dtype)
        hn = torch.empty(B, L * H, **f32)
        hn_lp = torch.empty(B, L * H, device=dev, dtype=torch.bfloat16) if (bf and top == 0) else None
        if not bf:
            top = 2
        hs_top = torch.empty(T, B, H, **f32) if (bf and top != 0) else None
        d = LstmDesc()
        dims = (L, B, T, I, Ic, H)
        _fill_lstm_desc(d, dtype, dims, x_tm, xc, params, x_lp)
        lp = torch.empty(int(lib.fhvae_lstm_lp_bytes(C.byref(d))), device=dev, dtype=torch.uint8)
        if bf:
            LSTM_WORKSPACES.append(lp)
            del LSTM_WORKSPACES[:-16]
        d.lp = _p(lp)
        d.hs, d.cs, d.gates, d.hn, d.hs_top_f32, d.lp = _p(hs), _p(cs), _p(gates), _p(hn), _p(hs_top if top == 2 else None), _p(lp)
        d.hn_lp = _p(hn_lp)
        shadows = None
        if bf and head is not None and head_shadow_shapes(head[0]) is not None:
            hw_mu, hw_lv = _f32c(head[0].detach()), _f32c(head[1].detach())
            (sl, st_) = head_shadow_shapes(hw_mu)
            shadows = (torch.empty(sl, device=dev, dtype=torch.bfloat16), torch.empty(st_, device=dev, dtype=torch.bfloat16))
            d.head_w_mu, d.head_w_lv, d.head_wl, d.head_wt = _p(hw_mu), _p(hw_lv), _p(shadows[0]), _p(shadows[1])
            d.head_D, d.head_K, d.head_ldt = hw_mu.shape[0], hw_mu.shape[1], st_[1]
        pre = torch.empty(max(1, int(lib.fhvae_lstm_pre_elems(C.byref(d)))), **f32)
        d.pre = _p(pre)
        LAST_LSTM_FORM["form"] = int(lib.fhvae_lstm_form(C.byref(d)))
        with _Timed("fhvae_lstm_seq_fwd"):
            _check(lib.fhvae_lstm_seq_fwd(C.byref(d), _stream()), "fhvae_lstm_seq_fwd")
        ctx.dims, ctx.dtype = dims, dtype
        ctx.x_lp = x_lp
        ctx.layout_id = int(lib.fhvae_lstm_layout_id(C.byref(d)))
        LAST_LSTM_FORM["layout"] = ctx.layout_id
        ctx.save_for_backward(x_tm, xc, hs, cs, gates, lp, *params)
        if hn_lp is not None:
            hn._fh_lp = hn_lp
        hn._fh_head = shadows
        if top == 0:
            out = hn.new_empty(())
            ctx.mark_non_differentiable(out)
            return out, hn
        out = hs_top if bf else hs[L - 1]
        if bf:
            out._fh_lp = hs[L - 1]
        out._fh_head = shadows
        return out, hn

    @staticmethod
    def backward(ctx, d_hs_top, d_hn):
        lib = load_library()
        L, B, T, I, Ic, H = ctx.dims
        x_tm, xc, hs, cs, gates, lp = ctx.saved_tensors[:6]
        params = ctx.saved_tensors[6:]
        dev = hs.device
        f32 = dict(device=dev, dtype=torch.float32)
        if d_hs_top is None and d_hn is None:
            return (None,) * (6 + 4 * L)
        d_hs_top = _f32c(d_hs_top) if d_hs_top is not None else None
        d_hn = _f32c(d_hn) if d_hn is not None else None
        bd = LstmBwdDesc()
        d = bd.f
        _fill_lstm_desc(d, ctx.dtype, ctx.dims, x_tm, xc, params, ctx.x_lp)
        pre = torch.empty(1, **f32)
        d.hs, d.cs, d.gates, d.hn, d.hs_top_f32, d.pre, d.lp = _p(hs), _p(cs), _p(gates), None, None, _p(pre), _p(lp)
        dgates = torch.empty(L, T, B, 4 * H, device=dev, dtype=hs.dtype)
        dgsum = torch.empty(B, 4 * H, **f32) if Ic > 0 else None
        dc = torch.empty(L, B, H, **f32)
        grads = [sk if sk is not None else torch.zeros_like(p) for p, sk in zip(params, ctx.sinks)]
        d_xc = torch.empty(B, Ic, **f32) if (Ic > 0 and ctx.needs_input_grad[1]) else None
        bd.d_hs_top, bd.d_hn = _p(d_hs_top), _p(d_hn)
        bd.dgates, bd.dgsum, bd.dc = _p(dgates), _p(dgsum), _p(dc)
        for l in range(L):
            bd.dw_ih[l], bd.dw_hh[l], bd.db_ih[l], bd.db_hh[l] = (_p(grads[4 * l + k]) for k in range(4))
        bd.d_xc = _p(d_xc)
        if int(lib.fhvae_lstm_layout_id(C.byref(d))) != ctx.layout_id:
            raise RuntimeError("the LSTM schedule changed between this net's forward and its backward (an FHVAE_* switch was flipped "
                               "in between?): the saved gates / workspaces are in the forward's layout")
        n_below = int(lib.fhvae_lstm_ws_below_elems(C.byref(d)))
        ws_below = torch.empty(n_below, **f32) if n_below > 0 else None
        bd.ws_below = _p(ws_below)
        if (_DEFER["enabled"] and not _SIDE["enabled"] and all(sk is not None for sk in ctx.sinks)):
            bd.phase = 1
            with _Timed("fhvae_lstm_seq_bwd"):
                _check(lib.fhvae_lstm_seq_bwd(C.byref(bd), _stream()), "fhvae_lstm_seq_bwd")
            _DEFER["pending"].append((bd, (x_tm, xc, hs, cs, gates, lp, pre, dgates, dgsum, dc, d_hs_top, d_hn, params, ctx.x_lp)))
            if LSTM_BWD_REC_HOOK["fn"] is not None:
                LSTM_BWD_REC_HOOK["fn"](ctx.sinks)
            return (None, d_xc, None, None, None, None, *[None] * len(params))
        if _SIDE["enabled"] and all(sk is not None for sk in ctx.sinks):
            bd.phase = 1
            with _Timed("fhvae_lstm_seq_bwd"):
                _check(lib.fhvae_lstm_seq_bwd(C.byref(bd), _stream()), "fhvae_lstm_seq_bwd")
            main, side = torch.cuda.current_stream(), side_stream()
            side.wait_stream(main)
            bd.phase = 2
            with torch.cuda.stream(side):
                with _Timed("fhvae_lstm_seq_bwd(param grads, side stream)"):
                    _check(lib.fhvae_lstm_seq_bwd(C.byref(bd), _stream()), "fhvae_lstm_seq_bwd")
            _SIDE["pending"] = True
            _SIDE["keep"].append((x_tm, xc, hs, cs, gates, lp, dgates, dgsum, dc, d_hs_top, d_hn, params))
        elif LSTM_BWD_REC_HOOK["fn"] is not None:
            bd.phase = 1
            with _Timed("fhvae_lstm_seq_bwd"):
                _check(lib.fhvae_lstm_seq_bwd(C.byref(bd), _stream()), "fhvae_lstm_seq_bwd")
            LSTM_BWD_REC_HOOK["fn"](ctx.sinks)
            bd.phase = 2
            with _Timed("fhvae_lstm_seq_bwd(param grads)"):
                _check(lib.fhvae_lstm_seq_bwd(C.byref(bd), _stream()), "fhvae_lstm_seq_bwd")
        else:
            bd.phase = 0
            with _Timed("fhvae_lstm_seq_bwd"):
                _check(lib.fhvae_lstm_seq_bwd(C.byref(bd), _stream()), "fhvae_lstm_seq_bwd")
        return (None, d_xc, None, None, None, None, *[None if sk is not None else g for g, sk in zip(grads, ctx.sinks)])


def lstm_seq(x_tm, xc, T, params: Sequence[torch.Tensor], dtype: int = F32, top: int = 2, head=None):
    return _LstmSeq.apply(x_tm, xc, int(T), int(dtype), int(top), head, *params)


def lstm_seq_infer(x_tm, xc, T, params: Sequence[torch.Tensor], dtype: int = F32, top: int = 2, head=None):
    lib = load_library()
    _need_gpu(x_tm, xc, *params)
    L = len(params) // 4
    assert len(params) == 4 * L and 1 <= L <= MAX_LAYERS
    T, dtype, top = int(T), int(dtype), int(top)
    params = [_f32c(p.detach()) for p in params]
    H = params[1].shape[1]
    x_lp = getattr(x_tm, "_fh_lp", None) if x_tm is not None else None
    x_tm = _f32c(x_tm.detach()) if x_tm is not None else None
    xc = _f32c(xc.detach()) if xc is not None else None
    I = x_tm.shape[2] if x_tm is not None else 0
    Ic = xc.shape[1] if xc is not None else 0
    B = x_tm.shape[1] if x_tm is not None else xc.shape[0]
    if x_tm is not None:
        assert x_tm.shape[0] == T
    assert params[0].shape == (4 * H, I + Ic), (params[0].shape, H, I, Ic)
    dev = params[0].device
    f32 = dict(device=dev, dtype=torch.float32)
    bf = dtype == BF16
    hs = torch.empty(L, T, B, H, device=dev, dtype=torch.bfloat16 if bf else torch.float32)
    hn = torch.empty(B, L * H, **f32)
    hn_lp = torch.empty(B, L * H, device=dev, dtype=torch.bfloat16) if (bf and top == 0) else None
    if not bf:
        top = 2
    hs_top = torch.empty(T, B, H, **f32) if (bf and top == 2) else None
    d = LstmDesc()
    dims = (L, B, T, I, Ic, H)
    _fill_lstm_desc(d, dtype, dims, x_tm, xc, params, x_lp)
    lp = None
    if bf:
        lp = torch.empty(int(lib.fhvae_lstm_lp_bytes(C.byref(d))), device=dev, dtype=torch.uint8)
        LSTM_WORKSPACES.append(lp)
        del LSTM_WORKSPACES[:-16]
    d.lp = _p(lp)
    d.hs, d.gates, d.hn, d.hs_top_f32, d.hn_lp = _p(hs), None, _p(hn), _p(hs_top), _p(hn_lp)
    shadows = None
    if bf and head is not None and head_shadow_shapes(head[0]) is not None:
        hw_mu, hw_lv = _f32c(head[0].detach()), _f32c(head[1].detach())
        (sl, st_) = head_shadow_shapes(hw_mu)
        shadows = (torch.empty(sl, device=dev, dtype=torch.bfloat16), torch.empty(st_, device=dev, dtype=torch.bfloat16))
        d.head_w_mu, d.head_w_lv, d.head_wl, d.head_wt = _p(hw_mu), _p(hw_lv), _p(shadows[0]), _p(shadows[1])
        d.head_D, d.head_K, d.head_ldt = hw_mu.shape[0], hw_mu.shape[1], st_[1]
    pre = torch.empty(max(1, int(lib.fhvae_lstm_pre_elems(C.byref(d)))), **f32)
    d.pre = _p(pre)
    n_cs = int(lib.fhvae_lstm_infer_cs_elems(C.byref(d)))
    cs = torch.empty(n_cs, **f32) if n_cs > 0 else None
    d.cs = _p(cs)
    LAST_LSTM_FORM["form"] = int(lib.fhvae_lstm_form(C.byref(d)))
    with _Timed("fhvae_lstm_seq_infer"):
        _check(lib.fhvae_lstm_seq_infer(C.byref(d), _stream()), "fhvae_lstm_seq_infer")
    LAST_LSTM_FORM["layout"] = int(lib.fhvae_lstm_layout_id(C.byref(d)))
    if hn_lp is not None:
        hn._fh_lp = hn_lp
    hn._fh_head = shadows
    if top == 0:
        return None, hn
    out = hs_top if (bf and top == 2) else hs[L - 1]
    if bf:
        out._fh_lp = hs[L - 1]
    out._fh_head = shadows
    return out, hn


def infer_enabled() -> bool:
    return not os.environ.get("FHVAE_NO_INFER")


def lstm_seq_eval(x_tm, xc, T, params, dtype=F32, top=2, head=None):
    if infer_enabled():
        return lstm_seq_infer(x_tm, xc, T, params, dtype, top, head)
    out, hn = lstm_seq(x_tm, xc, T, params, dtype, top, head)
    return (None if (top == 0 and dtype == BF16) else out), hn


def raw_gather_rows(table, idx, idx_offset=0):
    lib = load_library()
    S, D = table.shape
    B = idx.shape[0]
    out = torch.empty(B, D, device=table.device, dtype=torch.float32)
    with _Timed("fhvae_mu2_gather_fwd"):
        _check(lib.fhvae_mu2_gather_fwd(_p(table), _p(idx), idx_offset, _p(out), B, S, D, None, _stream()),
               "fhvae_mu2_gather_fwd")
    return out


def raw_scatter_rows_(dtable, drows, idx, idx_offset=0, scale=1.0):
    lib = load_library()
    S, D = dtable.shape
    with _Timed("fhvae_mu2_gather_bwd"):
        _check(lib.fhvae_mu2_gather_bwd(_p(drows), _p(idx), idx_offset, _p(dtable), idx.shape[0], S, D, float(scale),
                                        _stream()), "fhvae_mu2_gather_bwd")


class _Mu2Gather(torch.autograd.Function):

    @staticmethod
    def forward(ctx, table, idx):
        _need_gpu(table, idx)
        ctx.sink = _sink(table)
        table = _f32c(table)
        out = raw_gather_rows(table, idx)
        ctx.save_for_backward(idx)
        ctx.shape = tuple(table.shape)
        return out

    @staticmethod
    def backward(ctx, dmu2):
        (idx,) = ctx.saved_tensors
        dmu2 = _f32c(dmu2)
        dt = ctx.sink if ctx.sink is not None else torch.zeros(ctx.shape, device=dmu2.device, dtype=torch.float32)
        raw_scatter_rows_(dt, dmu2, idx)
        return (None if ctx.sink is not None else dt), None


def mu2_gather(table, idx):
    return _Mu2Gather.apply(table, idx)


def _fill_elbo_desc(d: ElboDesc, x, x_strides, x_mu, x_lv, xo_strides, z1_mu, z1_lv, z2_mu, z2_lv, mu2, num_segs, B, T, F_):
    d.B, d.T, d.F, d.D1, d.D2 = B, T, F_, z1_mu.shape[1], z2_mu.shape[1]
    d.x, (d.x_sb, d.x_st) = _p(x), x_strides
    d.x_mu, d.x_lv, (d.xo_sb, d.xo_st) = _p(x_mu), _p(x_lv), xo_strides
    d.z1_mu, d.z1_lv, d.z2_mu, d.z2_lv, d.mu2 = _p(z1_mu), _p(z1_lv), _p(z2_mu), _p(z2_lv), _p(mu2)
    if isinstance(num_segs, torch.Tensor):
        d.num_segs, d.nsegs_scalar = _p(num_segs), 0.0
    else:
        d.num_segs, d.nsegs_scalar = None, float(num_segs)


class _Elbo(torch.autograd.Function):

    @staticmethod
    def forward(ctx, x, x_mu, x_lv, z1_mu, z1_lv, z2_mu, z2_lv, mu2, num_segs, layout, reference_detach):
        _need_gpu(x, x_mu, x_lv, z1_mu, z1_lv, z2_mu, z2_lv, mu2)
        ctx.set_materialize_grads(False)
        lib = load_library()
        B, T, F_, xs, xos = layout
        pair = (x_mu.dim() == 2 and x_lv.dim() == 2 and x_mu.dtype == torch.float32 and x_lv.dtype == torch.float32
                and x_mu.stride(1) == 1 and x_lv.stride(1) == 1 and x_mu.stride(0) == 2 * F_ and x_lv.stride(0) == 2 * F_
                and x_lv.data_ptr() - x_mu.data_ptr() == 4 * F_ and xos == (F_, B * F_))
        if pair:
            xos = (2 * F_, B * 2 * F_)
            layout = (B, T, F_, xs, xos)
        ts = [t if (pair and i in (1, 2)) else _f32c(t) for i, t in enumerate((x, x_mu, x_lv, z1_mu, z1_lv, z2_mu, z2_lv, mu2))]
        ctx.pair = pair
        if isinstance(num_segs, torch.Tensor):
            num_segs = num_segs.to(device=ts[0].device, dtype=torch.int64).contiguous()
        outs = [torch.empty(B, device=ts[0].device, dtype=torch.float32) for _ in range(5)]
        d = ElboDesc()
        _fill_elbo_desc(d, ts[0], xs, ts[1], ts[2], xos, *ts[3:], num_segs, B, T, F_)
        d.lower_bound, d.log_px_z, d.neg_kld_z1, d.neg_kld_z2, d.log_pmu2 = (_p(o) for o in outs)
        with _Timed("fhvae_elbo_fwd"):
            _check(lib.fhvae_elbo_fwd(C.byref(d), _stream()), "fhvae_elbo_fwd")
        ctx.layout, ctx.detach = layout, bool(reference_detach)
        ctx.nsegs = num_segs
        ctx.save_for_backward(*ts)
        if reference_detach:
            ctx.mark_non_differentiable(outs[1], outs[4])
        return tuple(outs)

    @staticmethod
    def backward(ctx, g_lb, g_px, g_k1, g_k2, g_pm):
        lib = load_library()
        ts = ctx.saved_tensors
        B, T, F_, xs, xos = ctx.layout
        _PAIR_GRAD.clear()
        bd = ElboBwdDesc()
        _fill_elbo_desc(bd.f, ts[0], xs, ts[1], ts[2], xos, *ts[3:], ctx.nsegs, B, T, F_)
        gs = [_f32c(g) if g is not None else None for g in (g_lb, g_px, g_k1, g_k2, g_pm)]
        if ctx.detach:
            gs[1] = gs[4] = None
        bd.g_lower_bound, bd.g_log_px_z, bd.g_neg_kld_z1, bd.g_neg_kld_z2, bd.g_log_pmu2 = (_p(g) for g in gs)
        bd.reference_detach = int(ctx.detach)
        need_x = not ctx.detach
        side = None
        if need_x and ctx.pair:
            dbuf = torch.empty(ts[1].shape[0], 2 * F_, device=ts[1].device, dtype=torch.float32)
            d_xmu, d_xlv = dbuf[:, :F_], dbuf[:, F_:]
            if PAIR_SIDE["enabled"] and xs == (F_, B * F_) and F_ % 4 == 0 and F_ <= 256 and ts[0].data_ptr() % 16 == 0 and ts[1].data_ptr() % 16 == 0:
                ldg = _pair_ld(F_)
                side = (dbuf, torch.empty(T * B, ldg, device=dbuf.device, dtype=torch.bfloat16),
                        torch.empty(int(lib.fhvae_elbo_colsum_rows(B)), 2 * F_, device=dbuf.device, dtype=torch.float32))
                bd.d_x_pair_lp, bd.ld_pair, bd.d_x_colsum = _p(side[1]), ldg, _p(side[2])
        else:
            d_xmu = torch.empty_like(ts[1]) if need_x else None
            d_xlv = torch.empty_like(ts[2]) if need_x else None
        dz = [torch.empty_like(t) for t in ts[3:8]]
        bd.d_x_mu, bd.d_x_lv = _p(d_xmu), _p(d_xlv)
        bd.d_z1_mu, bd.d_z1_lv, bd.d_z2_mu, bd.d_z2_lv, bd.d_mu2 = (_p(t) for t in dz)
        with _Timed("fhvae_elbo_bwd"):
            _check(lib.fhvae_elbo_bwd(C.byref(bd), _stream()), "fhvae_elbo_bwd")
        if side is not None:
            _PAIR_GRAD["latest"] = side + (dbuf._version,)
        return (None, d_xmu, d_xlv, *dz, None, None, None)


def elbo(x, x_mu, x_lv, z1_mu, z1_lv, z2_mu, z2_lv, mu2, num_segs, layout, reference_detach):
    if reference_detach:
        x_mu, x_lv = x_mu.detach(), x_lv.detach()
    return _Elbo.apply(x, x_mu, x_lv, z1_mu, z1_lv, z2_mu, z2_lv, mu2, num_segs, layout, bool(reference_detach))


class _FusedLoss(torch.autograd.Function):

    @staticmethod
    def forward(ctx, lower_bound, log_qy, alpha):
        _need_gpu(lower_bound, log_qy)
        lib = load_library()
        lb, qy = _f32c(lower_bound), _f32c(log_qy)
        out = torch.empty((), device=lb.device, dtype=torch.float32)
        with _Timed("fhvae_loss_fwd"):
            _check(lib.fhvae_loss_fwd(_p(lb), _p(qy), float(alpha), _p(out), lb.numel(), _device_words(lb.device)[1:].data_ptr(),
                                      _stream()), "fhvae_loss_fwd")
        ctx.alpha, ctx.B = float(alpha), lb.numel()
        return out

    @staticmethod
    def backward(ctx, g):
        lib = load_library()
        g = _f32c(g)
        d_lb = torch.empty(ctx.B, device=g.device, dtype=torch.float32)
        d_qy = torch.empty((), device=g.device, dtype=torch.float32) if ctx.needs_input_grad[1] else None
        with _Timed("fhvae_loss_bwd"):
            _check(lib.fhvae_loss_bwd(_p(g), ctx.alpha, _p(d_lb), _p(d_qy), ctx.B, _stream()), "fhvae_loss_bwd")
        return d_lb, d_qy, None


def fused_loss(lower_bound, log_qy, alpha):
    return _FusedLoss.apply(lower_bound, log_qy, float(alpha))


def raw_disc_fwd(q, table, idx, row0=0, want_ce=True, lp=False, out3=None, ce_scale=1.0):
    lib = load_library()
    B, D = q.shape
    S = table.shape[0]
    dev = q.device
    ws = torch.empty(max(int(lib.fhvae_disc_lse_ws_bytes(B, S)), 8), device=dev, dtype=torch.uint8)
    rmax, rsum, tgt = (out3[0], out3[1], out3[2]) if out3 is not None else (torch.empty(B, device=dev, dtype=torch.float32) for _ in range(3))
    ce = torch.empty((), device=dev, dtype=torch.float32) if want_ce else None
    with _Timed("fhvae_disc_lse_fwd"):
        _check(lib.fhvae_disc_lse_fwd(_p(q), _p(table), _p(idx), row0, INV_TWO_VAR, _p(rmax), _p(rsum), _p(tgt), _p(ce), float(ce_scale),
                                      _p(ws), B, S, D, BF16 if lp else F32, _stream()), "fhvae_disc_lse_fwd")
    return rmax, rsum, tgt, ce


DISC_BWD_WS = {"bytes": None}


def raw_disc_bwd(q, table, idx, rmax, rsum, g_scale, g_mul, row0=0, need_dq=True, need_dt=True, dt_sink=None, lp=False, ws_bytes=None):
    lib = load_library()
    B, D = q.shape
    S = table.shape[0]
    dq = torch.empty(B, D, device=q.device, dtype=torch.float32) if need_dq else None
    dt = dt_sink if dt_sink is not None else (torch.zeros(S, D, device=q.device, dtype=torch.float32) if need_dt else None)
    if ws_bytes is None:
        ws_bytes = DISC_BWD_WS["bytes"]
    nws = int(lib.fhvae_disc_lse_bwd_ws_bytes(B, S, D)) if ws_bytes is None else int(ws_bytes)
    ws = torch.empty(nws, device=q.device, dtype=torch.uint8) if (need_dq and dt is not None and nws > 0) else None
    with _Timed("fhvae_disc_lse_bwd"):
        _check(lib.fhvae_disc_lse_bwd(_p(q), _p(table), _p(idx), row0, INV_TWO_VAR, _p(rmax), _p(rsum), _p(g_scale), float(g_mul),
                                      _p(dq), _p(dt), _p(ws), nws if ws is not None else 0, B, S, D, BF16 if lp else F32, _stream()),
               "fhvae_disc_lse_bwd")
    return dq, (None if dt_sink is not None else dt)


def shard_pack(q, idx):
    lib = load_library()
    B, D = q.shape
    out = torch.empty(B, D + 1, device=q.device, dtype=torch.float32)
    _check(lib.fhvae_shard_pack(_p(q), _p(idx), _p(out), B, D, _stream()), "fhvae_shard_pack")
    return out


def shard_unpack(pk):
    lib = load_library()
    N, D = pk.shape[0], pk.shape[1] - 1
    q = torch.empty(N, D, device=pk.device, dtype=torch.float32)
    idx = torch.empty(N, device=pk.device, dtype=torch.int64)
    _check(lib.fhvae_shard_unpack(_p(pk), _p(q), _p(idx), N, D, _stream()), "fhvae_shard_unpack")
    return q, idx


def disc_merge_partials(parts):
    lib = load_library()
    W, _, N = parts.shape
    m, s, t = (torch.empty(N, device=parts.device, dtype=torch.float32) for _ in range(3))
    _check(lib.fhvae_disc_merge_partials(_p(parts), _p(m), _p(s), _p(t), W, N, _stream()), "fhvae_disc_merge_partials")
    return m, s, t


def shard_bwd_pack(dq_all, dq_scale, dmu2_local, own0, n_all, D):
    lib = load_library()
    ref = dq_all if dq_all is not None else dmu2_local
    out = torch.empty(n_all, 2 * D, device=ref.device, dtype=torch.float32)
    n_own = dmu2_local.shape[0] if dmu2_local is not None else 0
    _check(lib.fhvae_shard_bwd_pack(_p(dq_all), float(dq_scale), _p(dmu2_local), own0, n_own, _p(out), n_all, D, _stream()),
           "fhvae_shard_bwd_pack")
    return out


def shard_bwd_unpack(buf, own0, n_own, want_dq=True, want_dmu2=True):
    lib = load_library()
    N, D = buf.shape[0], buf.shape[1] // 2
    dq = torch.empty(n_own, D, device=buf.device, dtype=torch.float32) if want_dq else None
    dm = torch.empty(N, D, device=buf.device, dtype=torch.float32) if want_dmu2 else None
    _check(lib.fhvae_shard_bwd_unpack(_p(buf), own0, n_own, _p(dq), _p(dm), N, D, _stream()), "fhvae_shard_bwd_unpack")
    return dq, dm


def raw_disc_ce_mean(m, s, tgt, scale=1.0):
    lib = load_library()
    ce = torch.empty((), device=m.device, dtype=torch.float32)
    with _Timed("fhvae_disc_ce_mean"):
        _check(lib.fhvae_disc_ce_mean(_p(m), _p(s), _p(tgt), _p(ce), float(scale), m.numel(), _stream()), "fhvae_disc_ce_mean")
    return ce


class _DiscLse(torch.autograd.Function):

    @staticmethod
    def forward(ctx, q, table, idx, lp, sign):
        _need_gpu(q, table, idx)
        ctx.sink = _sink(table)
        ctx.lp = bool(lp)
        ctx.sign = float(sign)
        q, table = _f32c(q), _f32c(table)
        rmax, rsum, _, ce = raw_disc_fwd(q, table, idx, lp=ctx.lp, ce_scale=ctx.sign)
        ctx.save_for_backward(q, table, idx, rmax, rsum)
        return ce

    @staticmethod
    def backward(ctx, g):
        q, table, idx, rmax, rsum = ctx.saved_tensors
        g = _f32c(g).reshape(1)
        dq, dt = raw_disc_bwd(q, table, idx, rmax, rsum, g, ctx.sign / q.shape[0], need_dq=ctx.needs_input_grad[0],
                              need_dt=ctx.needs_input_grad[1], dt_sink=ctx.sink, lp=ctx.lp)
        return dq, dt, None, None, None


def disc_lse(q, table, idx, lp=False, sign=1.0):
    return _DiscLse.apply(q, table, idx, bool(lp), float(sign))


def wgrad_bf16_(c, a, b):
    lib = load_library()
    _need_gpu(c, a, b)
    assert a.dtype == torch.bfloat16 and b.dtype == torch.bfloat16 and c.dtype == torch.float32
    assert a.stride(1) == 1 and b.stride(1) == 1 and c.stride(1) == 1 and a.shape[0] == b.shape[0]
    K, M = a.shape
    N = b.shape[1]
    with _Timed("fhvae_wgrad_bf16"):
        _check(lib.fhvae_wgrad_bf16(_p(a), a.stride(0), _p(b), b.stride(0), _p(c), c.stride(0), M, N, K, _stream()), "fhvae_wgrad_bf16")
    return c


def wgrad_f32_(c, a, b):
    lib = load_library()
    _need_gpu(c, a, b)
    assert a.dtype == torch.float32 and b.dtype == torch.float32 and c.dtype == torch.float32
    assert a.stride(1) == 1 and b.stride(1) == 1 and c.stride(1) == 1 and a.shape[0] == b.shape[0]
    K, M = a.shape
    N = b.shape[1]
    with _Timed("fhvae_wgrad_f32"):
        _check(lib.fhvae_wgrad_f32(_p(a), a.stride(0), _p(b), b.stride(0), _p(c), c.stride(0), M, N, K, _stream()), "fhvae_wgrad_f32")
    return c


def proj_bf16(a, w, bias=None, out=None):
    lib = load_library()
    _need_gpu(a, w)
    assert a.dtype == torch.bfloat16 and w.dtype == torch.bfloat16 and a.stride(1) == 1 and w.stride(1) == 1 and a.shape[1] == w.shape[1]
    M, K = a.shape
    N = w.shape[0]
    if out is None:
        out = torch.empty(M, N, device=a.device, dtype=torch.float32)
    with _Timed("fhvae_proj_bf16"):
        _check(lib.fhvae_proj_bf16(_p(a), a.stride(0), _p(w), w.stride(0), _p(bias), _p(out), out.stride(0), M, N, K, _stream()), "fhvae_proj_bf16")
    return out


ADAM_ZERO_GRAD, ADAM_ADVANCE, ADAM_STEP_WORDS = 1, 2, 65 * 32
_ONES = {}


def backward(loss: torch.Tensor):
    key = (loss.device, loss.dtype, tuple(loss.shape))
    one = _ONES.get(key)
    if one is None:
        if loss.is_cuda and torch.cuda.is_current_stream_capturing():
            loss.backward()
            return
        one = _ONES[key] = torch.ones_like(loss)
    loss.backward(gradient=one)


def adam_step_(p, g, m, v, step_dev, lr, beta1, beta2, eps, grad_scale=1.0, p_lp=None, flags=0):
    lib = load_library()
    _need_gpu(p, g, m, v, step_dev)
    if (flags & ADAM_ADVANCE) and step_dev.numel() < ADAM_STEP_WORDS:
        raise RuntimeError("ADAM_ADVANCE needs an int32[%d] step buffer (step count + scratch words)" % ADAM_STEP_WORDS)
    n = p.numel()
    if n == 0:
        return
    with _Timed("fhvae_adam_step"):
        _check(lib.fhvae_adam_step(_p(p), _p(g), _p(m), _p(v), _p(p_lp), n, lr, beta1, beta2, eps, grad_scale, int(flags), _p(step_dev),
                                   _stream()), "fhvae_adam_step")



def segment_gather(pool, start, T, mean=None, inv_std=None, time_major=False):
    lib = load_library()
    _need_gpu(pool, start, mean, inv_std)
    pool = _f32c(pool)
    B, F_ = start.shape[0], pool.shape[1]
    out = torch.empty(B, T, F_, device=pool.device, dtype=torch.float32)
    out_tm = torch.empty(T, B, F_, device=pool.device, dtype=torch.float32) if time_major else None
    with _Timed("fhvae_segment_gather"):
        _check(lib.fhvae_segment_gather(_p(pool), pool.shape[0], _p(start), _p(mean), _p(inv_std), _p(out), _p(out_tm), B, T, F_,
                                        None, _stream()), "fhvae_segment_gather")
    return (out, out_tm) if time_major else out


class Mu2Estimator:

    def __init__(self, num_seqs: int, dim: int, device):
        self.S, self.D = int(num_seqs), int(dim)
        self.zsum = torch.zeros(self.S, self.D, device=device, dtype=torch.float32)
        self.count = torch.zeros(self.S, device=device, dtype=torch.float32)

    def add(self, z2_mu, idx):
        lib = load_library()
        _need_gpu(z2_mu, idx)
        z2_mu = _f32c(z2_mu.detach())
        with _Timed("fhvae_mu2_accumulate"):
            _check(lib.fhvae_mu2_accumulate(_p(z2_mu), _p(idx), _p(self.zsum), _p(self.count), z2_mu.shape[0], self.S, self.D,
                                            _stream()), "fhvae_mu2_accumulate")

    def result(self, ratio: float):
        lib = load_library()
        mu2 = torch.empty_like(self.zsum)
        with _Timed("fhvae_mu2_finalize"):
            _check(lib.fhvae_mu2_finalize(_p(self.zsum), _p(self.count), _p(mu2), self.S, self.D, float(ratio), _stream()),
                   "fhvae_mu2_finalize")
        return mu2, self.count


HS_BAD_SEQ, HS_CAP, HS_BAD_IDX, HS_UNSORTED = 1, 2, 4, 8


def hs_status_message(st: int) -> str:
    names = [n for b, n in ((HS_BAD_SEQ, "sequence id out of range"), (HS_CAP, "segment total above capacity"),
                            (HS_BAD_IDX, "local index out of range"), (HS_UNSORTED, "local indices not sorted")) if st & b]
    return ", ".join(names) or "ok"


def hs_select(seq_ptr, block_seqs, seg_ids, local_idx, n_out, status):
    _need_gpu(seq_ptr, block_seqs, seg_ids, local_idx, n_out, status)
    for t in (seq_ptr, block_seqs, seg_ids, local_idx, n_out):
        if t.dtype != torch.int64 or not t.is_contiguous():
            raise RuntimeError("hs_select takes contiguous int64 tensors")
    if status.dtype != torch.int32 or seg_ids.shape != local_idx.shape:
        raise RuntimeError("hs_select: status must be int32 and seg_ids / local_idx the same length")
    lib = load_library()
    with _Timed("fhvae_hs_select"):
        _check(lib.fhvae_hs_select(_p(seq_ptr), seq_ptr.shape[0] - 1, _p(block_seqs), block_seqs.shape[0], _p(seg_ids),
                                   _p(local_idx), _p(n_out), seg_ids.shape[0], _p(status), _stream()), "fhvae_hs_select")


FEATS_TYPES = {"fbank": 0, "spec": 1}
FEATS_BAD_PTR = 1


def feats_fwd(wave, wave_ptr, frame_ptr, dft_basis, mel_basis, n_fft, hop, n_mels, ftype, out, status):
    _need_gpu(wave, wave_ptr, frame_ptr, dft_basis, mel_basis, out, status)
    for t in (wave, dft_basis, out) + ((mel_basis,) if mel_basis is not None else ()):
        if t.dtype != torch.float32 or not t.is_contiguous():
            raise RuntimeError("feats_fwd takes contiguous f32 samples, bases and output")
    for t in (wave_ptr, frame_ptr):
        if t.dtype != torch.int64 or not t.is_contiguous():
            raise RuntimeError("feats_fwd takes contiguous int64 wave_ptr / frame_ptr")
    if status.dtype != torch.int32 or wave_ptr.shape != frame_ptr.shape or out.dim() != 2:
        raise RuntimeError("feats_fwd: status must be int32, wave_ptr / frame_ptr the same length and out 2-D")
    n_out = n_mels if ftype == "fbank" else n_fft // 2 + 1
    G = (n_fft // 2 + 16) // 16
    if tuple(dft_basis.shape) != (32 * G, (n_fft + 15) // 16 * 16):
        raise RuntimeError("feats_fwd: dft_basis must be (%d, %d) for n_fft %d" % (32 * G, (n_fft + 15) // 16 * 16, n_fft))
    if ftype == "fbank" and (mel_basis is None or tuple(mel_basis.shape) != ((n_mels + 15) // 16 * 16, 16 * G)):
        raise RuntimeError("feats_fwd: mel_basis must be (%d, %d)" % ((n_mels + 15) // 16 * 16, 16 * G))
    if out.shape[1] != n_out:
        raise RuntimeError("feats_fwd: out has %d columns, %s needs %d" % (out.shape[1], ftype, n_out))
    lib = load_library()
    with _Timed("fhvae_feats_fwd"):
        _check(lib.fhvae_feats_fwd(_p(wave), wave.numel(), _p(wave_ptr), _p(frame_ptr), wave_ptr.shape[0] - 1, out.shape[0],
                                   _p(dft_basis), _p(mel_basis), n_fft, hop, n_mels, FEATS_TYPES[ftype], _p(out), _p(status),
                                   _stream()), "fhvae_feats_fwd")


RESAMPLE_BAD_PTR = 1


def resample_fwd(wave_in, in_ptr, out_ptr, row_ptr, n_rows, bank, chunks, L, M, P, WL, ratio, exc, alt, alt_wl, wave_out, status):
    _need_gpu(wave_in, in_ptr, out_ptr, row_ptr, bank, chunks, exc, alt, wave_out, status)
    for t in (wave_in, bank, wave_out) + ((alt,) if alt is not None else ()):
        if t.dtype != torch.float32 or not t.is_contiguous():
            raise RuntimeError("resample_fwd takes contiguous f32 samples, bank and output")
    for t in (in_ptr, out_ptr, row_ptr):
        if t.dtype != torch.int64 or not t.is_contiguous() or t.dim() != 1 or t.shape != in_ptr.shape or t.shape[0] < 2:
            raise RuntimeError("resample_fwd takes contiguous int64 in_ptr / out_ptr / row_ptr of one length (U + 1)")
    if status.dtype != torch.int32 or status.numel() != 1 or wave_in.dim() != 1 or wave_out.dim() != 1:
        raise RuntimeError("resample_fwd: status must be one int32 word, wave_in and wave_out 1-D")
    NCP = (P * L + 15) // 16 * 16
    if bank.dim() != 2 or bank.shape[0] != NCP or bank.shape[1] % 16 != 0:
        raise RuntimeError("resample_fwd: bank must be (%d, KP) with KP a multiple of 16" % NCP)
    if chunks.dtype != torch.int32 or not chunks.is_contiguous() or tuple(chunks.shape) != (NCP // 16, 2):
        raise RuntimeError("resample_fwd: chunks must be contiguous int32 (%d, 2)" % (NCP // 16))
    if (exc is None) != (alt is None) or (exc is not None and (exc.dtype != torch.uint8 or not exc.is_contiguous() or exc.dim() != 1)):
        raise RuntimeError("resample_fwd: exc (uint8, 1-D) and alt come together")
    lib = load_library()
    with _Timed("fhvae_resample_fwd"):
        _check(lib.fhvae_resample_fwd(_p(wave_in), wave_in.numel(), _p(in_ptr), _p(out_ptr), _p(row_ptr), in_ptr.shape[0] - 1,
                                      n_rows, _p(bank), _p(chunks), L, M, P, bank.shape[1], WL, float(ratio), _p(exc),
                                      0 if exc is None else exc.numel(), _p(alt), 0 if alt is None else alt.numel(), alt_wl,
                                      _p(wave_out), wave_out.numel(), _p(status), _stream()), "fhvae_resample_fwd")


SYNTH_BAD_PTR = 1


def _synth_args(name, f32, ptrs, status):
    for t in f32:
        if t is not None and (t.dtype != torch.float32 or not t.is_contiguous()):
            raise RuntimeError("%s takes contiguous f32 tensors" % name)
    for t in ptrs:
        if t.dtype != torch.int64 or not t.is_contiguous() or t.dim() != 1 or t.shape != ptrs[0].shape or t.shape[0] < 2:
            raise RuntimeError("%s takes contiguous int64 wave_ptr / frame_ptr of one length (U + 1)" % name)
    if status.dtype != torch.int32 or status.numel() != 1:
        raise RuntimeError("%s: status must be one int32 word" % name)


def synth_istft(spec, wave_ptr, frame_ptr, synth_basis, win_sq, n_fft, hop, frames_ws, wave_out, status):
    _need_gpu(spec, wave_ptr, frame_ptr, synth_basis, win_sq, frames_ws, wave_out, status)
    _synth_args("synth_istft", (spec, synth_basis, win_sq, frames_ws, wave_out), (wave_ptr, frame_ptr), status)
    n_bins, KP = n_fft // 2 + 1, (n_fft + 15) // 16 * 16
    if spec.dim() != 3 or tuple(spec.shape[1:]) != (n_bins, 2):
        raise RuntimeError("synth_istft: spec must be (n_frames, %d, 2) for n_fft %d" % (n_bins, n_fft))
    if tuple(synth_basis.shape) != (KP, (2 * n_bins + 15) // 16 * 16) or tuple(win_sq.shape) != (n_fft,):
        raise RuntimeError("synth_istft: synth_basis must be (%d, %d) and win_sq (%d,)" % (KP, (2 * n_bins + 15) // 16 * 16, n_fft))
    if tuple(frames_ws.shape) != (spec.shape[0], KP) or wave_out.dim() != 1:
        raise RuntimeError("synth_istft: frames_ws must be (%d, %d) and wave_out 1-D" % (spec.shape[0], KP))
    lib = load_library()
    with _Timed("fhvae_synth_istft"):
        _check(lib.fhvae_synth_istft(_p(spec), spec.shape[0], _p(wave_ptr), _p(frame_ptr), wave_ptr.shape[0] - 1, wave_out.numel(),
                                     _p(synth_basis), _p(win_sq), n_fft, hop, _p(frames_ws), _p(wave_out), _p(status), _stream()),
               "fhvae_synth_istft")


def synth_project(wave, wave_ptr, frame_ptr, dft_basis, mag, tprev, coef, n_fft, hop, rebuilt, nxt, status):
    _need_gpu(wave, wave_ptr, frame_ptr, dft_basis, mag, tprev, rebuilt, nxt, status)
    _synth_args("synth_project", (wave, dft_basis, mag, tprev, rebuilt, nxt), (wave_ptr, frame_ptr), status)
    n_bins = n_fft // 2 + 1
    G = (n_bins + 15) // 16
    if tuple(dft_basis.shape) != (32 * G, (n_fft + 15) // 16 * 16):
        raise RuntimeError("synth_project: dft_basis must be (%d, %d) for n_fft %d" % (32 * G, (n_fft + 15) // 16 * 16, n_fft))
    if mag.dim() != 2 or mag.shape[1] != n_bins or wave.dim() != 1:
        raise RuntimeError("synth_project: mag must be (n_frames, %d) and wave 1-D" % n_bins)
    for t in (tprev, rebuilt, nxt):
        if t is not None and tuple(t.shape) != (mag.shape[0], n_bins, 2):
            raise RuntimeError("synth_project: complex arrays must be (%d, %d, 2)" % (mag.shape[0], n_bins))
    lib = load_library()
    with _Timed("fhvae_synth_project"):
        _check(lib.fhvae_synth_project(_p(wave), wave.numel(), _p(wave_ptr), _p(frame_ptr), wave_ptr.shape[0] - 1, mag.shape[0],
                                       _p(dft_basis), _p(mag), _p(tprev), float(coef), n_fft, hop, _p(rebuilt), _p(nxt), _p(status),
                                       _stream()), "fhvae_synth_project")


def synth_deemph(wave, wave_ptr, coef, out, status):
    _need_gpu(wave, wave_ptr, out, status)
    _synth_args("synth_deemph", (wave, out), (wave_ptr,), status)
    if wave.dim() != 1 or out.shape != wave.shape:
        raise RuntimeError("synth_deemph: wave and out must be 1-D of one length")
    lib = load_library()
    with _Timed("fhvae_synth_deemph"):
        _check(lib.fhvae_synth_deemph(_p(wave), _p(wave_ptr), wave_ptr.shape[0] - 1, wave.numel(), float(coef), _p(out), _p(status),
                                      _stream()), "fhvae_synth_deemph")


def mu2_accumulate_sorted(z2_mu, local_idx, zsum, count, status):
    _need_gpu(z2_mu, local_idx, zsum, count, status)
    z2_mu = _f32c(z2_mu.detach())
    if local_idx.dtype != torch.int64 or not local_idx.is_contiguous() or status.dtype != torch.int32:
        raise RuntimeError("mu2_accumulate_sorted takes contiguous int64 indices and an int32 status word")
    N, D = z2_mu.shape
    if local_idx.shape[0] != N or zsum.shape[1] != D or count.shape[0] != zsum.shape[0]:
        raise RuntimeError("mu2_accumulate_sorted: shapes do not agree")
    if N == 0:
        return
    lib = load_library()
    with _Timed("fhvae_mu2_accumulate_sorted"):
        _check(lib.fhvae_mu2_accumulate_sorted(_p(z2_mu), _p(local_idx), _p(zsum), _p(count), N, zsum.shape[0], D, _p(status),
                                               _stream()), "fhvae_mu2_accumulate_sorted")


def mu2_load_table(zsum, count, table, m_rows, v_rows, ratio):
    _need_gpu(zsum, count, table, m_rows, v_rows)
    K, D = table.shape
    for t in (zsum, table, m_rows, v_rows):
        if t.dtype != torch.float32 or not t.is_contiguous() or t.numel() != K * D:
            raise RuntimeError("mu2_load_table: every row buffer must be contiguous f32 of %d x %d" % (K, D))
    if count.shape != (K,) or count.dtype != torch.float32:
        raise RuntimeError("mu2_load_table: count must be (%d,) f32" % K)
    lib = load_library()
    with _Timed("fhvae_mu2_load_table"):
        _check(lib.fhvae_mu2_load_table(_p(zsum), _p(count), _p(table), _p(m_rows), _p(v_rows), K, D, float(ratio), _stream()),
               "fhvae_mu2_load_table")


def hs_pack_partials(zsum, count, out):
    _need_gpu(zsum, count, out)
    K, D = zsum.shape
    for t, shape in ((zsum, (K, D)), (count, (K,)), (out, (K, D + 1))):
        if t.dtype != torch.float32 or not t.is_contiguous() or tuple(t.shape) != shape:
            raise RuntimeError("hs_pack_partials: zsum (K, D), count (K,) and out (K, D+1) must be contiguous f32")
    lib = load_library()
    with _Timed("fhvae_hs_pack_partials"):
        _check(lib.fhvae_hs_pack_partials(_p(zsum), _p(count), _p(out), K, D, _stream()), "fhvae_hs_pack_partials")


def mu2_merge_load_shard(parts, row0, row1, shard, m_rows, v_rows, ratio):
    _need_gpu(parts)
    W, K, D1 = parts.shape
    D, n = D1 - 1, row1 - row0
    if parts.dtype != torch.float32 or not parts.is_contiguous() or not 0 <= row0 <= row1 <= K:
        raise RuntimeError("mu2_merge_load_shard: parts must be contiguous f32 (W, K, D+1) and 0 <= row0 <= row1 <= K")
    for t in (shard, m_rows, v_rows):
        if t.dtype != torch.float32 or not t.is_contiguous() or t.numel() != n * D:
            raise RuntimeError("mu2_merge_load_shard: shard / m_rows / v_rows must be contiguous f32 of %d x %d" % (n, D))
    if n == 0:
        return
    _need_gpu(shard, m_rows, v_rows)
    lib = load_library()
    with _Timed("fhvae_mu2_merge_load_shard"):
        _check(lib.fhvae_mu2_merge_load_shard(_p(parts), W, K, row0, row1, _p(shard), _p(m_rows), _p(v_rows), D, float(ratio),
                                              _stream()), "fhvae_mu2_merge_load_shard")


class SortedMu2Estimator:

    def __init__(self, num_seqs: int, dim: int, device, status=None):
        self.S, self.D = int(num_seqs), int(dim)
        self.zsum = torch.zeros(self.S, self.D, device=device, dtype=torch.float32)
        self.count = torch.zeros(self.S, device=device, dtype=torch.float32)
        self.status = status if status is not None else torch.zeros(1, device=device, dtype=torch.int32)

    def add(self, z2_mu, idx):
        mu2_accumulate_sorted(z2_mu, idx, self.zsum, self.count, self.status)

    def check(self):
        st = int(self.status.item())
        if st != 0:
            raise RuntimeError("sorted mu2 estimate: %s (status %d)" % (hs_status_message(st), st))

    def result(self, ratio: float):
        lib = load_library()
        mu2 = torch.empty_like(self.zsum)
        with _Timed("fhvae_mu2_finalize"):
            _check(lib.fhvae_mu2_finalize(_p(self.zsum), _p(self.count), _p(mu2), self.S, self.D, float(ratio), _stream()),
                   "fhvae_mu2_finalize")
        return mu2, self.count

    def load_into(self, table, m_rows, v_rows, ratio: float):
        mu2_load_table(self.zsum, self.count, table, m_rows, v_rows, ratio)
```

Measured before the change: 1.253 million segments/s.

## Fuse mu2 gather/scatter into ELBO kernels and merge disc bwd finish kernels

The mu2 row gather is folded into the ELBO forward kernel, and the matching scatter-add of mu2 gradients into the table is folded into the ELBO backward kernel, in place of separate gather and scatter passes. In the discriminator MFMA backward, the dq reduction, the own-row correction and the table-gradient finish are merged into one kernel launch, so the separate own-row kernel is skipped. This saves several launches and intermediate B×D buffers. In exchange it adds atomics on the table gradient and recomputes the own-row distance in the finish kernel.

```diff
diff --git a/include/fhvae_hip.h b/include/fhvae_hip.h
--- a/include/fhvae_hip.h
+++ b/include/fhvae_hip.h
@@ -163,6 +163,11 @@
 int fhvae_elbo_bwd(const fhvae_elbo_bwd_desc* d, void* stream);
 int64_t fhvae_elbo_colsum_rows(int64_t B);
 
+int fhvae_elbo_gather_fwd(const fhvae_elbo_desc* d, const float* table, const int64_t* idx, int64_t S, float* mu2_rows,
+                          void* stream);
+int fhvae_elbo_scatter_bwd(const fhvae_elbo_bwd_desc* d, const float* table, const int64_t* idx, int64_t S, float* dtable,
+                           void* stream);
+
 int64_t fhvae_disc_lse_ws_bytes(int64_t B, int64_t S);
 int fhvae_disc_lse_fwd(const float* q, const float* table, const int64_t* idx, int64_t row0,
                        float inv_two_var, float* row_max, float* row_sumexp, float* tgt_logit,
diff --git a/pytorch-scalablefhvae_amd/csrc/disc_mfma.h b/pytorch-scalablefhvae_amd/csrc/disc_mfma.h
--- a/pytorch-scalablefhvae_amd/csrc/disc_mfma.h
+++ b/pytorch-scalablefhvae_amd/csrc/disc_mfma.h
@@ -22,6 +22,18 @@
   int chunk;
 };
 
+template <int D>
+__device__ __forceinline__ float sqdist(const float (&q)[D], const float* __restrict__ trow) {
+  float a0 = 0.f, a1 = 0.f;
+#pragma unroll
+  for (int d = 0; d < D; d += 2) {
+    const float d0 = q[d] - trow[d], d1 = q[d + 1] - trow[d + 1];
+    a0 = fmaf(d0, d0, a0);
+    a1 = fmaf(d1, d1, a1);
+  }
+  return a0 + a1;
+}
+
 int mfma_chunk(int64_t nx, int64_t ny, int target = 1024);
 
 bool disc_mfma_supported(int64_t B, int64_t S, int64_t D);
@@ -32,7 +44,7 @@
 int64_t disc_onepass_ws_bytes(int64_t B, int64_t S, int64_t D);
 int disc_mfma_bwd(const float* q, const float* table, const int64_t* idx, int64_t row0, float c, const float* rmax,
                   const float* rsum, const float* gsc, float gmul, float* dq, float* dtable, float* ws, int64_t ws_bytes,
-                  int64_t B, int64_t S, int64_t D, int lp, hipStream_t st);
+                  int64_t B, int64_t S, int64_t D, int lp, hipStream_t st, bool* own_done = nullptr);
 void disc_lp_launch(const DiscMfmaArgs& a, int mode, dim3 grid, hipStream_t st);
 
 }
diff --git a/pytorch-scalablefhvae_amd/csrc/disc_mfma.hip b/pytorch-scalablefhvae_amd/csrc/disc_mfma.hip
--- a/pytorch-scalablefhvae_amd/csrc/disc_mfma.hip
+++ b/pytorch-scalablefhvae_amd/csrc/disc_mfma.hip
@@ -347,9 +347,41 @@
   }
 }
 
-__global__ void disc_dt_finish_kernel(float* __restrict__ dy, const float* __restrict__ y, const float* __restrict__ g2,
-                                      const float* __restrict__ wy, int nxt, float c2, int64_t NY, int D) {
-  const int64_t i = (int64_t)blockIdx.x * blockDim.x + threadIdx.x;
+template <int D>
+__global__ __launch_bounds__(256) void disc_bwd_finish_kernel(float* __restrict__ dx, const float* __restrict__ g, int nchunks, int NX,
+                                                              int qblocks, const float* __restrict__ x, const float* __restrict__ y,
+                                                              const int64_t* __restrict__ idx, int64_t row0, float c,
+                                                              const float* __restrict__ rmax, const float* __restrict__ rsum,
+                                                              const float* __restrict__ gsc, float gmul, float* __restrict__ dy,
+                                                              const float* __restrict__ g2, const float* __restrict__ wy, int nxt,
+                                                              int64_t NY) {
+  if ((int)blockIdx.x < qblocks) {
+    const int64_t n = (int64_t)NX * D;
+    const int64_t i = (int64_t)blockIdx.x * 256 + threadIdx.x;
+    if (i >= n) return;
+    float a0 = 0.f, a1 = 0.f, a2 = 0.f, a3 = 0.f;
+    int k = 0;
+    for (; k + 4 <= nchunks; k += 4) {
+      a0 += g[(int64_t)k * n + i], a1 += g[(int64_t)(k + 1) * n + i], a2 += g[(int64_t)(k + 2) * n + i], a3 += g[(int64_t)(k + 3) * n + i];
+    }
+    for (; k < nchunks; ++k) a0 += g[(int64_t)k * n + i];
+    float r = (a0 + a1) + (a2 + a3);
+    const int b = (int)(i / D), d = (int)(i % D);
+    const int64_t s = idx[b] - row0;
+    if (s >= 0 && s < NY) {
+      float qr[D];
+#pragma unroll
+      for (int j = 0; j < D; ++j) qr[j] = x[(int64_t)b * D + j];
+      const float t = -c * sqdist<D>(qr, y + s * D);
+      const float w = (*gsc) * gmul * (__expf(t - rmax[b]) / rsum[b] - 1.f);
+      const float diff = x[(int64_t)b * D + d] - y[s * D + d];
+      r = __fadd_rn(r, -2.f * c * w * diff);
+      atomicAdd(dy + s * D + d, 2.f * c * w * diff);
+    }
+    dx[i] = r;
+    return;
+  }
+  const int64_t i = (int64_t)(blockIdx.x - qblocks) * 256 + threadIdx.x;
   if (i >= NY * D) return;
   const int64_t row = i / D;
   float sg = 0.f, sw = 0.f;
@@ -357,18 +389,7 @@
     sg += g2[(int64_t)t * NY * D + i];
     sw += wy[(int64_t)t * NY + row];
   }
-  dy[i] += c2 * (sg - y[i] * sw);
-}
-__global__ void disc_dq_reduce_kernel(float* __restrict__ dx, const float* __restrict__ g, int nchunks, int64_t n) {
-  const int64_t i = (int64_t)blockIdx.x * blockDim.x + threadIdx.x;
-  if (i >= n) return;
-  float a0 = 0.f, a1 = 0.f, a2 = 0.f, a3 = 0.f;
-  int c = 0;
-  for (; c + 4 <= nchunks; c += 4) {
-    a0 += g[(int64_t)c * n + i], a1 += g[(int64_t)(c + 1) * n + i], a2 += g[(int64_t)(c + 2) * n + i], a3 += g[(int64_t)(c + 3) * n + i];
-  }
-  for (; c < nchunks; ++c) a0 += g[(int64_t)c * n + i];
-  dx[i] = (a0 + a1) + (a2 + a3);
+  atomicAdd(dy + i, 2.f * c * (sg - y[i] * sw));
 }
 
 int mfma_chunk(int64_t nx, int64_t ny, int target) {
@@ -432,7 +453,7 @@
 
 int disc_mfma_bwd(const float* q, const float* table, const int64_t* idx, int64_t row0, float c, const float* rmax,
                   const float* rsum, const float* gsc, float gmul, float* dq, float* dtable, float* ws, int64_t ws_bytes, int64_t B,
-                  int64_t S, int64_t D, int lp, hipStream_t st) {
+                  int64_t S, int64_t D, int lp, hipStream_t st, bool* own_done) {
   DiscMfmaArgs a = {};
   a.c = c;
   a.idx = idx;
@@ -467,12 +488,17 @@
         hipLaunchKernelGGL((disc_mfma_kernel<16, 2>), grid, dim3(256), 0, st, a);
       int e = fh_launch_status();
       if (e) return e;
-      hipLaunchKernelGGL(disc_dq_reduce_kernel, dim3((unsigned)fh_cdiv(nb * D, 256)), dim3(256), 0, st, dq + x0 * D, a.G, (int)nchunks, nb * D);
-      hipLaunchKernelGGL(disc_dt_finish_kernel, dim3((unsigned)fh_cdiv(S * D, 256)), dim3(256), 0, st, dtable, table, a.G2, a.WY, (int)nxt,
-                         2.f * c, S, (int)D);
+      const unsigned qblocks = (unsigned)fh_cdiv(nb * D, 256), yblocks = (unsigned)fh_cdiv(S * D, 256);
+      if (D == 32)
+        hipLaunchKernelGGL((disc_bwd_finish_kernel<32>), dim3(qblocks + yblocks), dim3(256), 0, st, dq + x0 * D, a.G, (int)nchunks, (int)nb,
+                           (int)qblocks, a.X, table, a.idx, row0, c, a.rmax, a.rsum, gsc, gmul, dtable, a.G2, a.WY, (int)nxt, S);
+      else
+        hipLaunchKernelGGL((disc_bwd_finish_kernel<16>), dim3(qblocks + yblocks), dim3(256), 0, st, dq + x0 * D, a.G, (int)nchunks, (int)nb,
+                           (int)qblocks, a.X, table, a.idx, row0, c, a.rmax, a.rsum, gsc, gmul, dtable, a.G2, a.WY, (int)nxt, S);
       e = fh_launch_status();
       if (e) return e;
     }
+    if (own_done) *own_done = true;
     return FHVAE_OK;
   }
   if (dq) {
diff --git a/pytorch-scalablefhvae_amd/csrc/loss.hip b/pytorch-scalablefhvae_amd/csrc/loss.hip
--- a/pytorch-scalablefhvae_amd/csrc/loss.hip
+++ b/pytorch-scalablefhvae_amd/csrc/loss.hip
@@ -76,7 +76,22 @@
   return lv + df * df / expf(lv);
 }
 
-__global__ __launch_bounds__(256) void elbo_fwd_kernel(fhvae_elbo_desc d) {
+struct ElboTable {
+  const float* table;
+  const int64_t* idx;
+  int64_t S;
+  float* rows;
+  float* dtable;
+};
+template <bool GATHER>
+__device__ __forceinline__ int64_t elbo_row(const ElboTable& tb, int64_t b) {
+  if constexpr (!GATHER) return 0;
+  const int64_t s = tb.idx[b];
+  return (s < 0 || s >= tb.S) ? -1 : s;
+}
+
+template <bool GATHER>
+__global__ __launch_bounds__(256) void elbo_fwd_kernel(fhvae_elbo_desc d, ElboTable tb) {
   const int lane = threadIdx.x & 63;
   const int64_t b = (int64_t)blockIdx.x * 4 + (threadIdx.x >> 6);
   if (b >= d.B) return;
@@ -112,8 +127,16 @@
     const float mu = d.z1_mu[b * d.D1 + j], lv = d.z1_lv[b * d.D1 + j];
     k1 += 1.f + lv - 0.f - (mu * mu + expf(lv)) / 1.f;
   }
+  const int64_t srow = elbo_row<GATHER>(tb, b);
   for (int j = lane; j < d.D2; j += 64) {
-    const float mu = d.z2_mu[b * d.D2 + j], lv = d.z2_lv[b * d.D2 + j], m2 = d.mu2[b * d.D2 + j];
+    const float mu = d.z2_mu[b * d.D2 + j], lv = d.z2_lv[b * d.D2 + j];
+    float m2;
+    if constexpr (GATHER) {
+      m2 = srow >= 0 ? tb.table[srow * d.D2 + j] : 0.f;
+      if (tb.rows) tb.rows[b * d.D2 + j] = m2;
+    } else {
+      m2 = d.mu2[b * d.D2 + j];
+    }
     const float df = mu - m2;
     k2 += 1.f + lv - kPz2Logvar - (df * df + expf(lv)) / v2;
     pm += kLog2Pi + m2 * m2;
@@ -158,8 +181,10 @@
   g.gpm = glb / ns + (bd.g_log_pmu2 ? bd.g_log_pmu2[b] : 0.f);
   return g;
 }
-__device__ __forceinline__ void elbo_dz(const fhvae_elbo_bwd_desc& bd, int64_t b, int lane, const ElboG& g) {
+template <bool GATHER>
+__device__ __forceinline__ void elbo_dz(const fhvae_elbo_bwd_desc& bd, int64_t b, int lane, const ElboG& g, const ElboTable& tb) {
   const fhvae_elbo_desc& d = bd.f;
+  const int64_t srow = elbo_row<GATHER>(tb, b);
   const float v2 = expf(kPz2Logvar);
   for (int j = lane; j < d.D1; j += 64) {
     const int64_t o = b * d.D1 + j;
@@ -169,15 +194,27 @@
   }
   for (int j = lane; j < d.D2; j += 64) {
     const int64_t o = b * d.D2 + j;
-    const float mu = d.z2_mu[o], lv = d.z2_lv[o], m2 = d.mu2[o];
+    const float mu = d.z2_mu[o], lv = d.z2_lv[o];
+    float m2;
+    if constexpr (GATHER)
+      m2 = srow >= 0 ? tb.table[srow * d.D2 + j] : 0.f;
+    else
+      m2 = d.mu2[o];
     const float df = (mu - m2) / v2;
     bd.d_z2_mu[o] = -df * g.gk2;
     bd.d_z2_lv[o] = 0.5f * (1.f - expf(lv) / v2) * g.gk2;
-    bd.d_mu2[o] = df * g.gk2 + (bd.reference_detach ? 0.f : -m2 * g.gpm);
-  }
-}
-
-__global__ __launch_bounds__(256) void elbo_bwd_kernel(fhvae_elbo_bwd_desc bd) {
+    const float dm2 = df * g.gk2 + (bd.reference_detach ? 0.f : -m2 * g.gpm);
+    if constexpr (GATHER) {
+      if (bd.d_mu2) bd.d_mu2[o] = dm2;
+      if (tb.dtable && srow >= 0) atomicAdd(tb.dtable + srow * d.D2 + j, dm2);
+    } else {
+      bd.d_mu2[o] = dm2;
+    }
+  }
+}
+
+template <bool GATHER>
+__global__ __launch_bounds__(256) void elbo_bwd_kernel(fhvae_elbo_bwd_desc bd, ElboTable tb) {
   const fhvae_elbo_desc& d = bd.f;
   const int lane = threadIdx.x & 63;
   const int64_t b = (int64_t)blockIdx.x * 4 + (threadIdx.x >> 6);
@@ -213,10 +250,11 @@
       }
     }
   }
-  elbo_dz(bd, b, lane, g);
-}
-
-__global__ __launch_bounds__(256) void elbo_bwd_pair_kernel(fhvae_elbo_bwd_desc bd) {
+  elbo_dz<GATHER>(bd, b, lane, g, tb);
+}
+
+template <bool GATHER>
+__global__ __launch_bounds__(256) void elbo_bwd_pair_kernel(fhvae_elbo_bwd_desc bd, ElboTable tb) {
   const fhvae_elbo_desc& d = bd.f;
   __shared__ float cs[4][512];
   const int lane = threadIdx.x & 63, wave = threadIdx.x >> 6;
@@ -269,7 +307,7 @@
       const int t = i / padc, c = i % padc;
       *(uint4*)(gp + ((int64_t)t * d.B + b) * bd.ld_pair + 2 * F + c * 8) = make_uint4(0u, 0u, 0u, 0u);
     }
-    if (half == 0) elbo_dz(bd, b, lane, g);
+    if (half == 0) elbo_dz<GATHER>(bd, b, lane, g, tb);
   }
   for (int j = lane; j < 2 * F; j += 64) cs[wave][j] = 0.f;
   __syncthreads();
@@ -298,18 +336,6 @@
   p.chunk = (int)chunk;
   p.nchunks = (int)fh_cdiv(S, chunk);
   return p;
-}
-
-template <int D>
-__device__ __forceinline__ float sqdist(const float (&q)[D], const float* __restrict__ trow) {
-  float a0 = 0.f, a1 = 0.f;
-#pragma unroll
-  for (int d = 0; d < D; d += 2) {
-    const float d0 = q[d] - trow[d], d1 = q[d + 1] - trow[d + 1];
-    a0 = fmaf(d0, d0, a0);
-    a1 = fmaf(d1, d1, a1);
-  }
-  return a0 + a1;
 }
 
 template <int D>
@@ -747,7 +773,7 @@
   return fh_launch_status();
 }
 
-static int check_elbo(const fhvae_elbo_desc* d) {
+static int check_elbo(const fhvae_elbo_desc* d, bool need_mu2 = true) {
   FH_CHECK_PTR(d);
   FH_CHECK_POS(d->B);
   FH_CHECK_POS(d->T);
@@ -762,32 +788,47 @@
   FH_CHECK_PTR(d->z1_lv);
   FH_CHECK_PTR(d->z2_mu);
   FH_CHECK_PTR(d->z2_lv);
-  FH_CHECK_PTR(d->mu2);
+  if (need_mu2) FH_CHECK_PTR(d->mu2);
   if (!d->num_segs && !(d->nsegs_scalar > 0)) return FHVAE_ERR_SHAPE;
   return FHVAE_OK;
 }
 
-extern "C" int fhvae_elbo_fwd(const fhvae_elbo_desc* d, void* stream) {
-  int e = check_elbo(d);
+static int elbo_fwd_launch(const fhvae_elbo_desc* d, const ElboTable* tb, void* stream) {
+  int e = check_elbo(d, tb == nullptr);
   if (e) return e;
   FH_CHECK_PTR(d->lower_bound);
   FH_CHECK_PTR(d->log_px_z);
   FH_CHECK_PTR(d->neg_kld_z1);
   FH_CHECK_PTR(d->neg_kld_z2);
   FH_CHECK_PTR(d->log_pmu2);
-  hipLaunchKernelGGL(elbo_fwd_kernel, dim3((unsigned)fh_cdiv(d->B, 4)), dim3(256), 0, (hipStream_t)stream, *d);
-  return fh_launch_status();
-}
-
-extern "C" int fhvae_elbo_bwd(const fhvae_elbo_bwd_desc* d, void* stream) {
+  const dim3 grid((unsigned)fh_cdiv(d->B, 4));
+  if (tb)
+    hipLaunchKernelGGL(elbo_fwd_kernel<true>, grid, dim3(256), 0, (hipStream_t)stream, *d, *tb);
+  else
+    hipLaunchKernelGGL(elbo_fwd_kernel<false>, grid, dim3(256), 0, (hipStream_t)stream, *d, ElboTable{});
+  return fh_launch_status();
+}
+
+extern "C" int fhvae_elbo_fwd(const fhvae_elbo_desc* d, void* stream) { return elbo_fwd_launch(d, nullptr, stream); }
+
+extern "C" int fhvae_elbo_gather_fwd(const fhvae_elbo_desc* d, const float* table, const int64_t* idx, int64_t S, float* mu2_rows,
+                                     void* stream) {
+  FH_CHECK_PTR(table);
+  FH_CHECK_PTR(idx);
+  FH_CHECK_POS(S);
+  const ElboTable tb = {table, idx, S, mu2_rows, nullptr};
+  return elbo_fwd_launch(d, &tb, stream);
+}
+
+static int elbo_bwd_launch(const fhvae_elbo_bwd_desc* d, const ElboTable* tb, void* stream) {
   FH_CHECK_PTR(d);
-  int e = check_elbo(&d->f);
+  int e = check_elbo(&d->f, tb == nullptr);
   if (e) return e;
   FH_CHECK_PTR(d->d_z1_mu);
   FH_CHECK_PTR(d->d_z1_lv);
   FH_CHECK_PTR(d->d_z2_mu);
   FH_CHECK_PTR(d->d_z2_lv);
-  FH_CHECK_PTR(d->d_mu2);
+  if (!tb) FH_CHECK_PTR(d->d_mu2);
   if (!d->reference_detach && (!d->d_x_mu || !d->d_x_lv)) return FHVAE_ERR_NULL;
   if (d->d_x_pair_lp) {
     const fhvae_elbo_desc& f = d->f;
@@ -798,11 +839,32 @@
     if ((((uintptr_t)f.x | (uintptr_t)f.x_mu | (uintptr_t)f.x_lv | (uintptr_t)d->d_x_mu | (uintptr_t)d->d_x_lv | (uintptr_t)d->d_x_pair_lp) & 15))
       return FHVAE_ERR_ALIGN;
   }
-  if (d->d_x_pair_lp)
-    hipLaunchKernelGGL(elbo_bwd_pair_kernel, dim3((unsigned)fh_cdiv(d->f.B, 2)), dim3(256), 0, (hipStream_t)stream, *d);
-  else
-    hipLaunchKernelGGL(elbo_bwd_kernel, dim3((unsigned)fh_cdiv(d->f.B, 4)), dim3(256), 0, (hipStream_t)stream, *d);
-  return fh_launch_status();
+  hipStream_t st = (hipStream_t)stream;
+  if (d->d_x_pair_lp) {
+    const dim3 grid((unsigned)fh_cdiv(d->f.B, 2));
+    if (tb)
+      hipLaunchKernelGGL(elbo_bwd_pair_kernel<true>, grid, dim3(256), 0, st, *d, *tb);
+    else
+      hipLaunchKernelGGL(elbo_bwd_pair_kernel<false>, grid, dim3(256), 0, st, *d, ElboTable{});
+  } else {
+    const dim3 grid((unsigned)fh_cdiv(d->f.B, 4));
+    if (tb)
+      hipLaunchKernelGGL(elbo_bwd_kernel<true>, grid, dim3(256), 0, st, *d, *tb);
+    else
+      hipLaunchKernelGGL(elbo_bwd_kernel<false>, grid, dim3(256), 0, st, *d, ElboTable{});
+  }
+  return fh_launch_status();
+}
+
+extern "C" int fhvae_elbo_bwd(const fhvae_elbo_bwd_desc* d, void* stream) { return elbo_bwd_launch(d, nullptr, stream); }
+
+extern "C" int fhvae_elbo_scatter_bwd(const fhvae_elbo_bwd_desc* d, const float* table, const int64_t* idx, int64_t S, float* dtable,
+                                      void* stream) {
+  FH_CHECK_PTR(table);
+  FH_CHECK_PTR(idx);
+  FH_CHECK_POS(S);
+  const ElboTable tb = {table, idx, S, nullptr, dtable};
+  return elbo_bwd_launch(d, &tb, stream);
 }
 
 
@@ -951,10 +1013,11 @@
   hipStream_t st = (hipStream_t)stream;
   if (disc_mfma_supported(B, S, D) && !getenv("FHVAE_DISC_VALU")) {
     if (ws && (((uintptr_t)ws) & 15)) return FHVAE_ERR_ALIGN;
+    bool own_done = false;
     int e = disc_mfma_bwd(q, table, idx, row0, inv_two_var, row_max, row_sumexp, g_scale, g_mul, dq, dtable, (float*)ws,
-                          ws ? ws_bytes : 0, B, S, D, dtype == FHVAE_BF16, st);
+                          ws ? ws_bytes : 0, B, S, D, dtype == FHVAE_BF16, st, &own_done);
     if (e) return e;
-    if (dq || dtable) {
+    if ((dq || dtable) && !own_done) {
       DISC_DISPATCH(D, hipLaunchKernelGGL((disc_own_bwd_kernel<DD>), dim3((unsigned)fh_cdiv(B * (DD / 4), 256)), dim3(256), 0, st, q,
                                           table, idx, row0, inv_two_var, row_max, row_sumexp, g_scale, g_mul, dq, dtable, (int)B,
                                           (int)S));
diff --git a/pytorch-scalablefhvae_amd/fhvae.py b/pytorch-scalablefhvae_amd/fhvae.py
--- a/pytorch-scalablefhvae_amd/fhvae.py
+++ b/pytorch-scalablefhvae_amd/fhvae.py
@@ -6,7 +6,7 @@
 import torch.nn as nn
 
 import hip_binding as hb
-from fhvae_core import FHVAEBase
+from fhvae_core import FHVAEBase, LocalTableOps
 from simple_fhvae import GaussianLayer
 
 
@@ -115,7 +115,11 @@
         B, T, F_ = x.shape
         if F_ != self.n_feat:
             raise ValueError("x has %d features per frame, model was built for %d" % (F_, self.n_feat))
-        mu2_table, mu2 = self.mu2_lookup(mu_idx, self.z2_dim, num_seqs, mu2_table=mu2_table)
+        fuse = type(self.table_ops) is LocalTableOps
+        if fuse:
+            mu2_table, mu2 = self.table_ops.lookup(mu_idx, num_seqs, mu2_table, defer=True)
+        else:
+            mu2_table, mu2 = self.mu2_lookup(mu_idx, self.z2_dim, num_seqs, mu2_table=mu2_table)
         e2, e1 = self._draw(eps, B, x.device)
 
         dt = hb.BF16 if self.compute_dtype == "bf16" else hb.F32
@@ -137,4 +141,4 @@
 
         layout = (B, T, F_, (F_, B * F_), (F_, B * F_))
         return self._tail(x_tm, layout, x_mu, x_logvar, (z1_mu, z1_logvar), (z2_mu, z2_logvar), mu2, mu2_table, mu_idx,
-                          num_segs)
+                          num_segs, gather_in_k3=fuse)
diff --git a/pytorch-scalablefhvae_amd/fhvae_core.py b/pytorch-scalablefhvae_amd/fhvae_core.py
--- a/pytorch-scalablefhvae_amd/fhvae_core.py
+++ b/pytorch-scalablefhvae_amd/fhvae_core.py
@@ -19,9 +19,9 @@
     def __init__(self, model):
         self.model = model
 
-    def lookup(self, mu_idx, num_seqs, mu2_table=None):
+    def lookup(self, mu_idx, num_seqs, mu2_table=None, defer=False):
         table = mu2_table if mu2_table is not None else self.model._table(num_seqs, mu_idx.device)
-        return table, hb.mu2_gather(table, mu_idx)
+        return table, (None if defer else hb.mu2_gather(table, mu_idx))
 
     def disc(self, z2_mu, table, mu_idx, sign=1.0):
         return hb.disc_lse(z2_mu, table, mu_idx, lp=getattr(self.model, "compute_dtype", "f32") == "bf16", sign=sign)
@@ -116,10 +116,15 @@
         e1 = torch.randn(B, self.z1_dim, device=device)
         return e2, e1
 
-    def _tail(self, x_like, layout, x_mu, x_lv, z1, z2, mu2, table, mu_idx, num_segs):
+    def _tail(self, x_like, layout, x_mu, x_lv, z1, z2, mu2, table, mu_idx, num_segs, gather_in_k3=False):
         rc = self.reference_compat
-        mu2, log_qy = self.table_ops.resolve(z2[0], table, mu_idx, mu2, 1.0 if rc else -1.0)
-        lb, lpx, nk1, nk2, lpm = hb.elbo(x_like, x_mu, x_lv, z1[0], z1[1], z2[0], z2[1], mu2, num_segs, layout, rc)
+        if gather_in_k3:
+            log_qy = self.table_ops.disc(z2[0], table, mu_idx, 1.0 if rc else -1.0)
+            lb, lpx, nk1, nk2, lpm, mu2 = hb.elbo(x_like, x_mu, x_lv, z1[0], z1[1], z2[0], z2[1], None, num_segs, layout, rc,
+                                                  table=table, idx=mu_idx)
+        else:
+            mu2, log_qy = self.table_ops.resolve(z2[0], table, mu_idx, mu2, 1.0 if rc else -1.0)
+            lb, lpx, nk1, nk2, lpm = hb.elbo(x_like, x_mu, x_lv, z1[0], z1[1], z2[0], z2[1], mu2, num_segs, layout, rc)
         self.qz2_x = [z2[0], z2[1]]
         self.pz2 = [mu2, PZ2_LOGVAR]
         return lb, log_qy, lpx, nk1, nk2, lpm
diff --git a/pytorch-scalablefhvae_amd/hip_binding.py b/pytorch-scalablefhvae_amd/hip_binding.py
--- a/pytorch-scalablefhvae_amd/hip_binding.py
+++ b/pytorch-scalablefhvae_amd/hip_binding.py
@@ -113,6 +113,8 @@
     "fhvae_disc_ce_mean": (C.c_int, [_vp, _vp, _vp, _vp, _f32, _i64, _vp]),
     "fhvae_elbo_fwd": (C.c_int, [C.POINTER(ElboDesc), _vp]),
     "fhvae_elbo_bwd": (C.c_int, [C.POINTER(ElboBwdDesc), _vp]),
+    "fhvae_elbo_gather_fwd": (C.c_int, [C.POINTER(ElboDesc), _vp, _vp, _i64, _vp, _vp]),
+    "fhvae_elbo_scatter_bwd": (C.c_int, [C.POINTER(ElboBwdDesc), _vp, _vp, _i64, _vp, _vp]),
     "fhvae_disc_lse_ws_bytes": (_i64, [_i64, _i64]),
     "fhvae_disc_lse_bwd_ws_bytes": (_i64, [_i64, _i64, _i64]),
     "fhvae_disc_lse_fwd": (C.c_int, [_vp, _vp, _vp, _i64, _f32, _vp, _vp, _vp, _vp, _f32, _vp, _i64, _i64, _i64, C.c_int, _vp]),
@@ -895,7 +897,13 @@
 class _Elbo(torch.autograd.Function):
 
     @staticmethod
-    def forward(ctx, x, x_mu, x_lv, z1_mu, z1_lv, z2_mu, z2_lv, mu2, num_segs, layout, reference_detach):
+    def forward(ctx, x, x_mu, x_lv, z1_mu, z1_lv, z2_mu, z2_lv, mu2, num_segs, layout, reference_detach, table=None, idx=None):
+        gather = table is not None
+        if gather:
+            _need_gpu(table, idx)
+            ctx.sink = _sink(table)
+            mu2 = table
+        ctx.gather = gather
         _need_gpu(x, x_mu, x_lv, z1_mu, z1_lv, z2_mu, z2_lv, mu2)
         ctx.set_materialize_grads(False)
         lib = load_library()
@@ -914,23 +922,32 @@
         d = ElboDesc()
         _fill_elbo_desc(d, ts[0], xs, ts[1], ts[2], xos, *ts[3:], num_segs, B, T, F_)
         d.lower_bound, d.log_px_z, d.neg_kld_z1, d.neg_kld_z2, d.log_pmu2 = (_p(o) for o in outs)
-        with _Timed("fhvae_elbo_fwd"):
-            _check(lib.fhvae_elbo_fwd(C.byref(d), _stream()), "fhvae_elbo_fwd")
+        if gather:
+            d.mu2 = None
+            rows = torch.empty(B, ts[7].shape[1], device=ts[0].device, dtype=torch.float32)
+            with _Timed("fhvae_elbo_gather_fwd"):
+                _check(lib.fhvae_elbo_gather_fwd(C.byref(d), _p(ts[7]), _p(idx), ts[7].shape[0], _p(rows), _stream()), "fhvae_elbo_gather_fwd")
+            outs.append(rows)
+        else:
+            with _Timed("fhvae_elbo_fwd"):
+                _check(lib.fhvae_elbo_fwd(C.byref(d), _stream()), "fhvae_elbo_fwd")
         ctx.layout, ctx.detach = layout, bool(reference_detach)
         ctx.nsegs = num_segs
-        ctx.save_for_backward(*ts)
-        if reference_detach:
-            ctx.mark_non_differentiable(outs[1], outs[4])
+        ctx.save_for_backward(*ts, *((idx,) if gather else ()))
+        nd = ([outs[1], outs[4]] if reference_detach else []) + outs[5:]
+        if nd:
+            ctx.mark_non_differentiable(*nd)
         return tuple(outs)
 
     @staticmethod
-    def backward(ctx, g_lb, g_px, g_k1, g_k2, g_pm):
+    def backward(ctx, g_lb, g_px, g_k1, g_k2, g_pm, *_g_rows):
         lib = load_library()
         ts = ctx.saved_tensors
+        gather = ctx.gather
         B, T, F_, xs, xos = ctx.layout
         _PAIR_GRAD.clear()
         bd = ElboBwdDesc()
-        _fill_elbo_desc(bd.f, ts[0], xs, ts[1], ts[2], xos, *ts[3:], ctx.nsegs, B, T, F_)
+        _fill_elbo_desc(bd.f, ts[0], xs, ts[1], ts[2], xos, *ts[3:8], ctx.nsegs, B, T, F_)
         gs = [_f32c(g) if g is not None else None for g in (g_lb, g_px, g_k1, g_k2, g_pm)]
         if ctx.detach:
             gs[1] = gs[4] = None
@@ -949,20 +966,37 @@
         else:
             d_xmu = torch.empty_like(ts[1]) if need_x else None
             d_xlv = torch.empty_like(ts[2]) if need_x else None
-        dz = [torch.empty_like(t) for t in ts[3:8]]
+        dz = [torch.empty_like(t) for t in ts[3:7]] + [None if gather else torch.empty_like(ts[7])]
         bd.d_x_mu, bd.d_x_lv = _p(d_xmu), _p(d_xlv)
         bd.d_z1_mu, bd.d_z1_lv, bd.d_z2_mu, bd.d_z2_lv, bd.d_mu2 = (_p(t) for t in dz)
-        with _Timed("fhvae_elbo_bwd"):
-            _check(lib.fhvae_elbo_bwd(C.byref(bd), _stream()), "fhvae_elbo_bwd")
+        dt = None
+        if gather:
+            bd.f.mu2 = None
+            table, idx = ts[7], ts[8]
+            want = ctx.needs_input_grad[11]
+            dt = ctx.sink if ctx.sink is not None else (torch.zeros_like(table) if want else None)
+            with _Timed("fhvae_elbo_scatter_bwd"):
+                _check(lib.fhvae_elbo_scatter_bwd(C.byref(bd), _p(table), _p(idx), table.shape[0], _p(dt) if want else None, _stream()),
+                       "fhvae_elbo_scatter_bwd")
+            if ctx.sink is not None:
+                dt = None
+        else:
+            with _Timed("fhvae_elbo_bwd"):
+                _check(lib.fhvae_elbo_bwd(C.byref(bd), _stream()), "fhvae_elbo_bwd")
         if side is not None:
             _PAIR_GRAD["latest"] = side + (dbuf._version,)
-        return (None, d_xmu, d_xlv, *dz, None, None, None)
-
-
-def elbo(x, x_mu, x_lv, z1_mu, z1_lv, z2_mu, z2_lv, mu2, num_segs, layout, reference_detach):
+        return (None, d_xmu, d_xlv, *dz, None, None, None, dt, None)
+
+
+def elbo(x, x_mu, x_lv, z1_mu, z1_lv, z2_mu, z2_lv, mu2, num_segs, layout, reference_detach, table=None, idx=None):
     if reference_detach:
         x_mu, x_lv = x_mu.detach(), x_lv.detach()
-    return _Elbo.apply(x, x_mu, x_lv, z1_mu, z1_lv, z2_mu, z2_lv, mu2, num_segs, layout, bool(reference_detach))
+    if table is None:
+        return _Elbo.apply(x, x_mu, x_lv, z1_mu, z1_lv, z2_mu, z2_lv, mu2, num_segs, layout, bool(reference_detach), None, None)
+    if mu2 is not None:
+        raise ValueError("elbo: pass either mu2 or (table, idx)")
+    idx = torch.as_tensor(idx).to(device=table.device, dtype=torch.int64).contiguous()
+    return _Elbo.apply(x, x_mu, x_lv, z1_mu, z1_lv, z2_mu, z2_lv, None, num_segs, layout, bool(reference_detach), table, idx)
 
 
 class _FusedLoss(torch.autograd.Function):
```

Result: no change. 1.265 million segments/s (median of 6 runs) (+1.0%).
